# DanEngelbrecht/longtail

Measured on AMD Instinct MI355X. Metric: ingest GB/s (chunk+hash+compress), higher is better.
Workload: dtype u8/u32

## Files before the change

### longtail_amd/csrc/k_blake3.hip

```cpp
#include "lthip_internal.h"

#include <stdlib.h>

namespace
{

enum
{
    F_CHUNK_START = 1,
    F_CHUNK_END = 2,
    F_PARENT = 4,
    F_ROOT = 8
};

#define B3_IV0 0x6A09E667u
#define B3_IV1 0xBB67AE85u
#define B3_IV2 0x3C6EF372u
#define B3_IV3 0xA54FF53Au
#define B3_IV4 0x510E527Fu
#define B3_IV5 0x9B05688Cu
#define B3_IV6 0x1F83D9ABu
#define B3_IV7 0x5BE0CD19u

__device__ __forceinline__ uint32_t rotr32(uint32_t x, uint32_t r) { return __builtin_amdgcn_alignbit(x, x, r); }

__device__ __forceinline__ void b3_g(uint32_t& a, uint32_t& b, uint32_t& c, uint32_t& d, uint32_t mx, uint32_t my)
{
    a = a + b + mx;
    d = rotr32(d ^ a, 16);
    c = c + d;
    b = rotr32(b ^ c, 12);
    a = a + b + my;
    d = rotr32(d ^ a, 8);
    c = c + d;
    b = rotr32(b ^ c, 7);
}

#define B3_ROUND(m0, m1, m2, m3, m4, m5, m6, m7, m8, m9, m10, m11, m12, m13, m14, m15) \
    b3_g(s0, s4, s8, s12, m0, m1);                                                      \
    b3_g(s1, s5, s9, s13, m2, m3);                                                      \
    b3_g(s2, s6, s10, s14, m4, m5);                                                     \
    b3_g(s3, s7, s11, s15, m6, m7);                                                     \
    b3_g(s0, s5, s10, s15, m8, m9);                                                     \
    b3_g(s1, s6, s11, s12, m10, m11);                                                   \
    b3_g(s2, s7, s8, s13, m12, m13);                                                    \
    b3_g(s3, s4, s9, s14, m14, m15);

__device__ __forceinline__ void b3_compress(uint32_t (&cv)[8], const uint32_t (&m)[16], uint32_t counter_lo,
                                            uint32_t block_len, uint32_t flags)
{
    uint32_t s0 = cv[0], s1 = cv[1], s2 = cv[2], s3 = cv[3], s4 = cv[4], s5 = cv[5], s6 = cv[6], s7 = cv[7];
    uint32_t s8 = B3_IV0, s9 = B3_IV1, s10 = B3_IV2, s11 = B3_IV3;
    uint32_t s12 = counter_lo, s13 = 0u, s14 = block_len, s15 = flags;
    B3_ROUND(m[0], m[1], m[2], m[3], m[4], m[5], m[6], m[7], m[8], m[9], m[10], m[11], m[12], m[13], m[14], m[15])
    B3_ROUND(m[2], m[6], m[3], m[10], m[7], m[0], m[4], m[13], m[1], m[11], m[12], m[5], m[9], m[14], m[15], m[8])
    B3_ROUND(m[3], m[4], m[10], m[12], m[13], m[2], m[7], m[14], m[6], m[5], m[9], m[0], m[11], m[15], m[8], m[1])
    B3_ROUND(m[10], m[7], m[12], m[9], m[14], m[3], m[13], m[15], m[4], m[0], m[11], m[2], m[5], m[8], m[1], m[6])
    B3_ROUND(m[12], m[13], m[9], m[11], m[15], m[10], m[14], m[8], m[7], m[2], m[5], m[3], m[0], m[1], m[6], m[4])
    B3_ROUND(m[9], m[14], m[11], m[5], m[8], m[12], m[15], m[1], m[13], m[3], m[0], m[10], m[2], m[6], m[4], m[7])
    B3_ROUND(m[11], m[15], m[5], m[0], m[1], m[9], m[8], m[6], m[14], m[10], m[2], m[12], m[3], m[4], m[7], m[13])
    cv[0] = s0 ^ s8;
    cv[1] = s1 ^ s9;
    cv[2] = s2 ^ s10;
    cv[3] = s3 ^ s11;
    cv[4] = s4 ^ s12;
    cv[5] = s5 ^ s13;
    cv[6] = s6 ^ s14;
    cv[7] = s7 ^ s15;
}

typedef uint32_t u32x4_a4 __attribute__((ext_vector_type(4), aligned(4)));

__device__ __forceinline__ uint32_t leaves_of(uint32_t len) { return len ? (len + 1023u) >> 10 : 1u; }

__global__ void k_leaf_counts(const uint32_t* __restrict__ lens, uint64_t bound, const uint32_t* __restrict__ n_dev,
                              uint32_t* __restrict__ counts)
{
    uint64_t i = (uint64_t)blockIdx.x * blockDim.x + threadIdx.x;
    uint64_t n = n_dev ? (*n_dev < bound ? *n_dev : bound) : bound;
    if (i < n)
        counts[i] = leaves_of(lens[i]);
}

constexpr uint32_t b3s_blocks(uint32_t n, uint32_t B) { return (n + B - 1u) / B; }
constexpr uint32_t b3s_block_leaves(uint32_t n, uint32_t b, uint32_t B) { return n - b * B < B ? n - b * B : B; }
constexpr bool b3s_reg_merge(uint32_t m, uint32_t k, uint32_t st) { return k + st < m; }
constexpr bool b3s_root(uint32_t n, uint32_t K, uint32_t st) { return K == 0u && 2u * st >= n; }
constexpr bool b3s_to_lds(uint32_t n, uint32_t B) { return b3s_blocks(n, B) > 1u; }
constexpr bool b3s_lds_merge(uint32_t nb, uint32_t k, uint32_t st) { return (k & (2u * st - 1u)) == 0u && k + st < nb; }
constexpr bool b3s_lds_root(uint32_t nb, uint32_t st) { return 2u * st >= nb; }
constexpr uint32_t b3s_max_nodes(uint32_t S, uint32_t B) { return 2u * S / (B + 1u); }
constexpr uint32_t b3s_range_bytes(uint32_t n, uint32_t B) { return 6u + (b3s_to_lds(n, B) ? 32u * b3s_blocks(n, B) : 0u); }
constexpr uint32_t b3s_max_bytes(uint32_t S, uint32_t B) { return (6u * (B + 1u) > 70u ? 6u * (B + 1u) : 70u) * S / (B + 1u) + 6u + 16u; }

constexpr uint32_t PJ = 2;
constexpr uint32_t PB = 1u << PJ;
constexpr int PW = 2048;
constexpr int PW_MAXN = 256;
constexpr int PW_THREADS = 512;
constexpr int PW_WAVES = 8;
constexpr uint32_t PW_NODES = b3s_max_nodes(PW + PW_MAXN - 1, PB) + 1u;
constexpr uint32_t PW_MEM16 = (b3s_max_bytes(PW + PW_MAXN - 1, PB) + 15u) / 16u;
constexpr uint32_t PW_LEVELS = 8u - PJ;
static_assert(PW <= 4096 && (PW & (PW - 1)) == 0 && PW_THREADS % 64 == 0 && PW_MAXN >> PJ <= 255, "window tables are 16 bits, list entries 16 + 8 + 8");


__device__ __forceinline__ void b3_load_interior(uint32_t (&w)[17], const uint32_t* __restrict__ src)
{
    const u32x4_a4 v0 = *reinterpret_cast<const u32x4_a4*>(src);
    const u32x4_a4 v1 = *reinterpret_cast<const u32x4_a4*>(src + 4);
    const u32x4_a4 v2 = *reinterpret_cast<const u32x4_a4*>(src + 8);
    const u32x4_a4 v3 = *reinterpret_cast<const u32x4_a4*>(src + 12);
    w[0] = v0.x; w[1] = v0.y; w[2] = v0.z; w[3] = v0.w;
    w[4] = v1.x; w[5] = v1.y; w[6] = v1.z; w[7] = v1.w;
    w[8] = v2.x; w[9] = v2.y; w[10] = v2.z; w[11] = v2.w;
    w[12] = v3.x; w[13] = v3.y; w[14] = v3.z; w[15] = v3.w;
    w[16] = src[16];
}

__device__ __forceinline__ void b3_load_last(uint32_t (&w)[17], const uint32_t* __restrict__ src, uint32_t nd)
{
#pragma unroll
    for (int i = 0; i < 17; ++i)
        w[i] = (uint32_t)i < nd ? src[i] : 0u;
}

__device__ __forceinline__ void b3_interior_block(uint32_t (&cv)[8], uint32_t (&w)[17], uint32_t sh, uint32_t k, uint32_t flags)
{
#pragma unroll
    for (int i = 0; i < 16; ++i)
        asm("v_alignbit_b32 %0, %1, %0, %2" : "+v"(w[i]) : "v"(w[i + 1]), "v"(sh));
    uint32_t m[16];
#pragma unroll
    for (int i = 0; i < 16; ++i)
        m[i] = w[i];
    b3_compress(cv, m, k, 64u, flags);
}

__device__ __forceinline__ void b3_last_block(uint32_t (&cv)[8], const uint32_t (&w)[17], uint32_t sh, uint32_t k, uint32_t bl, uint32_t flags)
{
    uint32_t m[16];
#pragma unroll
    for (int i = 0; i < 16; ++i)
    {
        uint32_t v = __builtin_amdgcn_alignbit(w[i + 1], w[i], sh);
        const int rem = (int)bl - 4 * i;
        if (rem <= 0)
            v = 0u;
        else if (rem < 4)
            v &= (1u << (8 * rem)) - 1u;
        m[i] = v;
    }
    b3_compress(cv, m, k, bl, flags);
}

__device__ __forceinline__ void b3_pin(uint32_t (&cv)[8])
{
    asm volatile("" : "+v"(cv[0]), "+v"(cv[1]), "+v"(cv[2]), "+v"(cv[3]), "+v"(cv[4]), "+v"(cv[5]), "+v"(cv[6]), "+v"(cv[7])::"memory");
}

template <bool PIPE>
__global__ __launch_bounds__(256, 8) void k_blake3_leaves(const uint8_t* __restrict__ data,
                                                       const uint64_t* __restrict__ offsets,
                                                       const uint32_t* __restrict__ lens,
                                                       const uint32_t* __restrict__ leaf_prefix,
                                                       uint64_t count_bound, const uint32_t* __restrict__ n_dev,
                                                       uint32_t* __restrict__ cvs, uint32_t* __restrict__ win_first)
{
    const uint32_t count = (uint32_t)(n_dev ? (*n_dev < count_bound ? *n_dev : count_bound) : count_bound);
    const uint32_t total = leaf_prefix[count];
    const uint64_t g64 = (uint64_t)blockIdx.x * blockDim.x + threadIdx.x;
    if (g64 >= total)
        return;
    const uint32_t g = (uint32_t)g64;
    uint32_t lo = 0, hi = count;
    while (hi - lo > 1)
    {
        const uint32_t mid = lo + ((hi - lo) >> 1);
        if (leaf_prefix[mid] <= g)
            lo = mid;
        else
            hi = mid;
    }
    const uint32_t c = lo;
    const uint32_t first = leaf_prefix[c];
    const uint32_t k = g - first;
    if (win_first && (g & (uint32_t)(PW - 1)) == 0u)
        win_first[g / (uint32_t)PW] = k == 0u ? c : c + 1u;
    const uint32_t rlen = lens[c];
    const uint32_t nleaf = leaves_of(rlen);
    const uint32_t llen = rlen - (k << 10) < 1024u ? rlen - (k << 10) : 1024u;
    const uint8_t* p = data + offsets[c] + ((uint64_t)k << 10);
    const uint32_t root = nleaf == 1u ? (uint32_t)F_ROOT : 0u;

    const uint32_t mis = (uint32_t)((uintptr_t)p & 3u);
    const uint32_t sh = mis * 8u;
    const uint32_t* q = reinterpret_cast<const uint32_t*>(p - mis);

    uint32_t cv[8] = {B3_IV0, B3_IV1, B3_IV2, B3_IV3, B3_IV4, B3_IV5, B3_IV6, B3_IV7};
    const uint32_t nblocks = llen ? (llen + 63u) >> 6 : 1u;

    if constexpr (PIPE)
    {
        const uint32_t last = nblocks - 1u;
        const uint32_t bl = llen - last * 64u;
        const uint32_t nd = bl ? (mis + bl + 3u) >> 2 : 0u;
        uint32_t wa[17], wb[17];
        uint32_t b = 0;
        bool first_half = last > 1u && ((last - 1u) & 1u) == 0u;
        if (last > 1u && !first_half)
            b3_load_interior(wb, q);
        else if (last)
            b3_load_interior(wa, q);
        if (last > 1u)
        {
#pragma unroll 1
            for (;;)
            {
                if (first_half)
                {
                    b3_load_interior(wb, q + (b + 1u) * 16u);
                    b3_pin(cv);
                    b3_interior_block(cv, wa, sh, k, b == 0 ? (uint32_t)F_CHUNK_START : 0u);
                    b3_pin(cv);
                    ++b;
                }
                first_half = true;
                b3_load_interior(wa, q + (b + 1u) * 16u);
                b3_pin(cv);
                b3_interior_block(cv, wb, sh, k, b == 0 ? (uint32_t)F_CHUNK_START : 0u);
                b3_pin(cv);
                ++b;
                if (b + 1u >= last)
                    break;
            }
        }
        if (last)
        {
            b3_load_last(wb, q + last * 16u, nd);
            b3_pin(cv);
            b3_interior_block(cv, wa, sh, k, b == 0 ? (uint32_t)F_CHUNK_START : 0u);
            b3_pin(cv);
        }
        else
            b3_load_last(wb, q, nd);
        b3_last_block(cv, wb, sh, k, bl, (uint32_t)F_CHUNK_END | root | (last == 0 ? (uint32_t)F_CHUNK_START : 0u));
    }
    else
    {
        for (uint32_t b = 0; b + 1 < nblocks; ++b)
        {
            const uint32_t* src = q + b * 16u;
            uint32_t w[17];
            const u32x4_a4 v0 = *reinterpret_cast<const u32x4_a4*>(src);
            const u32x4_a4 v1 = *reinterpret_cast<const u32x4_a4*>(src + 4);
            const u32x4_a4 v2 = *reinterpret_cast<const u32x4_a4*>(src + 8);
            const u32x4_a4 v3 = *reinterpret_cast<const u32x4_a4*>(src + 12);
            w[0] = v0.x; w[1] = v0.y; w[2] = v0.z; w[3] = v0.w;
            w[4] = v1.x; w[5] = v1.y; w[6] = v1.z; w[7] = v1.w;
            w[8] = v2.x; w[9] = v2.y; w[10] = v2.z; w[11] = v2.w;
            w[12] = v3.x; w[13] = v3.y; w[14] = v3.z; w[15] = v3.w;
            w[16] = mis ? src[16] : 0u;
            uint32_t m[16];
#pragma unroll
            for (int i = 0; i < 16; ++i)
                m[i] = __builtin_amdgcn_alignbit(w[i + 1], w[i], sh);
            b3_compress(cv, m, k, 64u, b == 0 ? (uint32_t)F_CHUNK_START : 0u);
        }
        const uint32_t b = nblocks - 1u;
        const uint32_t bl = llen - b * 64u;
        uint32_t w[17];
        b3_load_last(w, q + b * 16u, bl ? (mis + bl + 3u) >> 2 : 0u);
        b3_last_block(cv, w, sh, k, bl, (uint32_t)F_CHUNK_END | root | (b == 0 ? (uint32_t)F_CHUNK_START : 0u));
    }
    uint4* out = reinterpret_cast<uint4*>(cvs + (uint64_t)g * 8u);
    out[0] = make_uint4(cv[0], cv[1], cv[2], cv[3]);
    out[1] = make_uint4(cv[4], cv[5], cv[6], cv[7]);
}

__device__ __forceinline__ void b3_parent(uint32_t* __restrict__ left, const uint32_t* __restrict__ right, uint32_t flags)
{
    uint32_t m[16];
    const uint4 a0 = reinterpret_cast<const uint4*>(left)[0], a1 = reinterpret_cast<const uint4*>(left)[1];
    const uint4 b0 = reinterpret_cast<const uint4*>(right)[0], b1 = reinterpret_cast<const uint4*>(right)[1];
    m[0] = a0.x; m[1] = a0.y; m[2] = a0.z; m[3] = a0.w; m[4] = a1.x; m[5] = a1.y; m[6] = a1.z; m[7] = a1.w;
    m[8] = b0.x; m[9] = b0.y; m[10] = b0.z; m[11] = b0.w; m[12] = b1.x; m[13] = b1.y; m[14] = b1.z; m[15] = b1.w;
    uint32_t cv[8] = {B3_IV0, B3_IV1, B3_IV2, B3_IV3, B3_IV4, B3_IV5, B3_IV6, B3_IV7};
    b3_compress(cv, m, 0u, 64u, flags);
    reinterpret_cast<uint4*>(left)[0] = make_uint4(cv[0], cv[1], cv[2], cv[3]);
    reinterpret_cast<uint4*>(left)[1] = make_uint4(cv[4], cv[5], cv[6], cv[7]);
}

#ifdef LTHIP_ABLATIONS
#include "ablations/k_blake3_parents_small.inc"
#endif

constexpr uint32_t B3_ONE_PITCH = 1024u + 4u;
__global__ __launch_bounds__(64) void k_blake3_one(const uint8_t* __restrict__ in, uint32_t len, uint64_t* __restrict__ out)
{
    extern __shared__ __attribute__((aligned(16))) uint32_t s_one[];
    uint32_t* s_cv = s_one;
    uint32_t* s_in = s_one + 64 * 8;
    const uint32_t lane = threadIdx.x;
    const uint32_t nleaf = leaves_of(len);
    {
        const uint32_t nvec = (((uintptr_t)in & 15u) == 0u) ? len >> 4 : 0u;
        const uint4* in4 = reinterpret_cast<const uint4*>(in);
        for (uint32_t v0 = 0; v0 < nvec; v0 += 64u * 8u)
        {
            uint4 q[8];
#pragma unroll
            for (int u = 0; u < 8; ++u)
            {
                const uint32_t v = v0 + (uint32_t)u * 64u + lane;
                q[u] = v < nvec ? in4[v] : make_uint4(0, 0, 0, 0);
            }
#pragma unroll
            for (int u = 0; u < 8; ++u)
            {
                const uint32_t v = v0 + (uint32_t)u * 64u + lane;
                if (v < nvec)
                {
                    uint32_t* d = s_in + (v >> 6) * (B3_ONE_PITCH / 4u) + (v & 63u) * 4u;
                    d[0] = q[u].x;
                    d[1] = q[u].y;
                    d[2] = q[u].z;
                    d[3] = q[u].w;
                }
            }
        }
        for (uint32_t j = (nvec << 4) + lane; j < len; j += 64u)
            reinterpret_cast<uint8_t*>(s_in)[(j >> 10) * B3_ONE_PITCH + (j & 1023u)] = in[j];
    }
    __syncthreads();
    if (lane < nleaf)
    {
        const uint32_t llen = len - (lane << 10) < 1024u ? len - (lane << 10) : 1024u;
        const uint32_t* pw = s_in + lane * (B3_ONE_PITCH / 4u);
        const uint8_t* p = reinterpret_cast<const uint8_t*>(pw);
        const uint32_t nblocks = llen ? (llen + 63u) >> 6 : 1u;
        uint32_t cv[8] = {B3_IV0, B3_IV1, B3_IV2, B3_IV3, B3_IV4, B3_IV5, B3_IV6, B3_IV7};
        for (uint32_t b = 0; b < nblocks; ++b)
        {
            const uint32_t bl = llen - b * 64u < 64u ? llen - b * 64u : 64u;
            uint32_t m[16];
            if (bl == 64u)
            {
#pragma unroll
                for (int i = 0; i < 16; ++i)
                    m[i] = pw[b * 16u + (uint32_t)i];
            }
            else
            {
#pragma unroll
                for (int i = 0; i < 16; ++i)
                    m[i] = 0u;
                for (uint32_t j = 0; j < bl; ++j)
                    m[j >> 2] |= (uint32_t)p[b * 64u + j] << (8u * (j & 3u));
            }
            uint32_t fl = b == 0 ? (uint32_t)F_CHUNK_START : 0u;
            if (b + 1 == nblocks)
                fl |= (uint32_t)F_CHUNK_END | (nleaf == 1u ? (uint32_t)F_ROOT : 0u);
            b3_compress(cv, m, lane, bl, fl);
        }
#pragma unroll
        for (int i = 0; i < 8; ++i)
            s_cv[lane * 8 + i] = cv[i];
    }
    __syncthreads();
    for (uint32_t stride = 1; stride < nleaf; stride <<= 1)
    {
        const uint32_t last = (stride << 1) >= nleaf;
        const uint32_t k = lane * (stride << 1);
        if (k + stride < nleaf)
            b3_parent(s_cv + k * 8u, s_cv + (k + stride) * 8u, (uint32_t)F_PARENT | (last ? (uint32_t)F_ROOT : 0u));
        __syncthreads();
    }
    if (lane == 0)
        *out = (uint64_t)s_cv[0] | ((uint64_t)s_cv[1] << 32);
}

constexpr int B3S_LEAVES = 1024;

__global__ __launch_bounds__(B3S_LEAVES) void k_blake3_stream_batch(const uint8_t* __restrict__ data, uint32_t leaf0,
                                                                      uint32_t* __restrict__ stack, uint32_t depth_in, uint32_t merges)
{
    __shared__ uint32_t s_cv[B3S_LEAVES * 8];
    const uint32_t t = threadIdx.x;
    {
        const uint32_t* p = reinterpret_cast<const uint32_t*>(data) + (size_t)t * 256u;
        uint32_t cv[8] = {B3_IV0, B3_IV1, B3_IV2, B3_IV3, B3_IV4, B3_IV5, B3_IV6, B3_IV7};
        for (uint32_t b = 0; b < 16u; ++b)
        {
            uint32_t m[16];
            const uint4* q = reinterpret_cast<const uint4*>(p + b * 16u);
            const uint4 v0 = q[0], v1 = q[1], v2 = q[2], v3 = q[3];
            m[0] = v0.x; m[1] = v0.y; m[2] = v0.z; m[3] = v0.w; m[4] = v1.x; m[5] = v1.y; m[6] = v1.z; m[7] = v1.w;
            m[8] = v2.x; m[9] = v2.y; m[10] = v2.z; m[11] = v2.w; m[12] = v3.x; m[13] = v3.y; m[14] = v3.z; m[15] = v3.w;
            b3_compress(cv, m, leaf0 + t, 64u, (b == 0 ? (uint32_t)F_CHUNK_START : 0u) | (b == 15u ? (uint32_t)F_CHUNK_END : 0u));
        }
#pragma unroll
        for (int i = 0; i < 8; ++i)
            s_cv[t * 8 + i] = cv[i];
    }
    __syncthreads();
    for (uint32_t stride = 1; stride < (uint32_t)B3S_LEAVES; stride <<= 1)
    {
        if ((t & (2u * stride - 1u)) == 0u)
            b3_parent(s_cv + t * 8u, s_cv + (t + stride) * 8u, (uint32_t)F_PARENT);
        __syncthreads();
    }
    if (t == 0)
    {
        uint32_t depth = depth_in;
        for (int i = 0; i < 8; ++i)
            stack[depth * 8u + i] = s_cv[i];
        ++depth;
        for (uint32_t m = 0; m < merges; ++m)
        {
            b3_parent(stack + (depth - 2u) * 8u, stack + (depth - 1u) * 8u, (uint32_t)F_PARENT);
            --depth;
        }
    }
}

__global__ __launch_bounds__(B3S_LEAVES) void k_blake3_stream_final(const uint8_t* __restrict__ tail, uint32_t tail_len, uint32_t leaf0,
                                                                      const uint32_t* __restrict__ stack, uint32_t depth_in,
                                                                      uint64_t* __restrict__ out)
{
    __shared__ uint32_t s_cv[B3S_LEAVES * 8];
    __shared__ uint32_t s_stack[64 * 8];
    const uint32_t t = threadIdx.x;
    const uint32_t nleaf = tail_len ? (tail_len + 1023u) >> 10 : (leaf0 == 0u ? 1u : 0u);
    const bool single = leaf0 == 0u && nleaf == 1u;
    if (t < nleaf)
    {
        const uint32_t llen = tail_len - (t << 10) < 1024u ? tail_len - (t << 10) : 1024u;
        const uint8_t* p = tail + ((size_t)t << 10);
        const uint32_t nblocks = llen ? (llen + 63u) >> 6 : 1u;
        uint32_t cv[8] = {B3_IV0, B3_IV1, B3_IV2, B3_IV3, B3_IV4, B3_IV5, B3_IV6, B3_IV7};
        for (uint32_t b = 0; b < nblocks; ++b)
        {
            const uint32_t bl = llen - b * 64u < 64u ? llen - b * 64u : 64u;
            uint32_t m[16];
#pragma unroll
            for (int i = 0; i < 16; ++i)
                m[i] = 0u;
            for (uint32_t j = 0; j < bl; ++j)
                m[j >> 2] |= (uint32_t)p[b * 64u + j] << (8u * (j & 3u));
            uint32_t fl = b == 0 ? (uint32_t)F_CHUNK_START : 0u;
            if (b + 1 == nblocks)
                fl |= (uint32_t)F_CHUNK_END | (single ? (uint32_t)F_ROOT : 0u);
            b3_compress(cv, m, leaf0 + t, bl, fl);
        }
#pragma unroll
        for (int i = 0; i < 8; ++i)
            s_cv[t * 8 + i] = cv[i];
    }
    for (uint32_t i = t; i < depth_in * 8u; i += (uint32_t)B3S_LEAVES)
        s_stack[i] = stack[i];
    __syncthreads();
    if (t != 0)
        return;
    if (single)
    {
        *out = (uint64_t)s_cv[0] | ((uint64_t)s_cv[1] << 32);
        return;
    }
    uint32_t depth = depth_in;
    for (uint32_t j = 0; j + 1 < nleaf; ++j)
    {
        for (int i = 0; i < 8; ++i)
            s_stack[depth * 8u + i] = s_cv[j * 8u + i];
        ++depth;
        uint32_t cnt = leaf0 + j + 1u;
        while ((cnt & 1u) == 0u)
        {
            b3_parent(s_stack + (depth - 2u) * 8u, s_stack + (depth - 1u) * 8u, (uint32_t)F_PARENT);
            --depth;
            cnt >>= 1;
        }
    }
    uint32_t* cur = s_cv + (nleaf - 1u) * 8u;
    while (depth > 0u)
    {
        uint32_t* left = s_stack + (depth - 1u) * 8u;
        b3_parent(left, cur, (uint32_t)F_PARENT | (depth == 1u ? (uint32_t)F_ROOT : 0u));
        cur = left;
        --depth;
    }
    *out = (uint64_t)cur[0] | ((uint64_t)cur[1] << 32);
}

__device__ __forceinline__ void b3_merge_regs(uint32_t (&left)[8], const uint32_t (&right)[8], uint32_t flags)
{
    const uint32_t m[16] = {left[0], left[1], left[2], left[3], left[4], left[5], left[6], left[7],
                            right[0], right[1], right[2], right[3], right[4], right[5], right[6], right[7]};
    uint32_t cv[8] = {B3_IV0, B3_IV1, B3_IV2, B3_IV3, B3_IV4, B3_IV5, B3_IV6, B3_IV7};
    b3_compress(cv, m, 0u, 64u, flags);
#pragma unroll
    for (int i = 0; i < 8; ++i)
        left[i] = cv[i];
}

__device__ __forceinline__ void pw_append(bool is, uint32_t entry, uint32_t* list, uint32_t* cnt, int lane)
{
    const uint64_t mask = __builtin_amdgcn_ballot_w64(is);
    if (mask == 0)
        return;
    uint32_t base = 0;
    if (lane == 0)
        base = atomicAdd(cnt, (uint32_t)__builtin_popcountll(mask));
    base = __builtin_amdgcn_readfirstlane(base);
    if (is)
        list[base + (uint32_t)__builtin_popcountll(mask & ((1ull << lane) - 1ull))] = entry;
}

__global__ __launch_bounds__(PW_THREADS, PW_WAVES) void k_blake3_parents_window(const uint32_t* __restrict__ leaf_prefix, uint64_t count_bound,
                                                                         const uint32_t* __restrict__ n_dev, const uint32_t* __restrict__ cvs,
                                                                         const uint32_t* __restrict__ win_first, uint64_t* __restrict__ hashes)
{
    __shared__ uint4 s_mem[PW_MEM16];
    __shared__ uint32_t s_list[2][PW_NODES / 2 + 1];
    __shared__ uint32_t s_cnt[PW_LEVELS + 1];
    __shared__ uint32_t s_wsum[PW_THREADS / 64];
    const uint32_t count = (uint32_t)(n_dev ? (*n_dev < count_bound ? *n_dev : count_bound) : count_bound);
    const uint32_t total = leaf_prefix[count];
    const uint64_t w0 = (uint64_t)blockIdx.x * PW;
    if (w0 >= total)
        return;
    const uint32_t tid = threadIdx.x;
    const int lane = (int)(tid & 63u);
    const uint32_t c_lo = win_first[blockIdx.x];
    const uint32_t c_hi = w0 + PW >= total ? count : win_first[blockIdx.x + 1u];
    const uint32_t nch = c_hi - c_lo;
    if (nch == 0)
        return;
    const uint32_t wbase = leaf_prefix[c_lo];
    if (nch > (uint32_t)PW || leaf_prefix[c_hi] - wbase > (uint32_t)(PW + PW_MAXN - 1))
        return;
    if (tid <= PW_LEVELS)
        s_cnt[tid] = 0;
    uint16_t* s_leaf = reinterpret_cast<uint16_t*>(s_mem);
    uint16_t* s_blk = s_leaf + (nch + 1u);
    uint16_t* s_node = s_blk + (nch + 1u);
    uint4* s_cv = s_mem + (6u * (nch + 1u) + 15u) / 16u;

    constexpr uint32_t R = (PW + PW_THREADS - 1) / PW_THREADS;
    {
        const uint32_t j0 = tid * R;
        uint32_t lp[R + 1], sum = 0;
#pragma unroll
        for (uint32_t i = 0; i <= R; ++i)
            lp[i] = leaf_prefix[c_lo + (j0 + i < nch ? j0 + i : nch)] - wbase;
#pragma unroll
        for (uint32_t i = 0; i < R; ++i)
        {
            const uint32_t n = lp[i + 1] - lp[i], nb = b3s_blocks(n, PB);
            sum += nb | (b3s_to_lds(n, PB) ? nb << 16 : 0u);
        }
        uint32_t incl = sum;
#pragma unroll
        for (int d = 1; d < 64; d <<= 1)
        {
            const uint32_t up = __shfl_up(incl, d, 64);
            if (lane >= d)
                incl += up;
        }
        if (lane == 63)
            s_wsum[tid >> 6] = incl;
        __syncthreads();
        uint32_t run = incl - sum;
        for (uint32_t w = 0; w < (tid >> 6); ++w)
            run += s_wsum[w];
#pragma unroll
        for (uint32_t i = 0; i <= R; ++i)
        {
            const uint32_t j = j0 + i;
            if (j <= nch && (i < R || j == nch))
            {
                s_leaf[j] = (uint16_t)lp[i];
                s_blk[j] = (uint16_t)(run & 0xFFFFu);
                s_node[j] = (uint16_t)(run >> 16);
            }
            if (i < R)
            {
                const uint32_t n = lp[i + 1] - lp[i], nb = b3s_blocks(n, PB);
                run += nb | (b3s_to_lds(n, PB) ? nb << 16 : 0u);
            }
        }
    }
    __syncthreads();

    if ((6u * (nch + 1u) + 15u) / 16u + 2u * s_node[nch] > PW_MEM16)
        return;

    const uint32_t nblk = s_blk[nch];
    const uint4* cvs4 = reinterpret_cast<const uint4*>(cvs) + (uint64_t)wbase * 2u;
    for (uint32_t b0 = 0; b0 < nblk; b0 += PW_THREADS)
    {
        const uint32_t blk = b0 + tid;
        bool left = false;
        uint32_t entry = 0;
        if (blk < nblk)
        {
            uint32_t lo = 0, hi = nch;
            while (hi - lo > 1)
            {
                const uint32_t mid = lo + ((hi - lo) >> 1);
                if (s_blk[mid] <= blk)
                    lo = mid;
                else
                    hi = mid;
            }
            const uint32_t j = lo, b = blk - s_blk[j];
            const uint32_t p = s_leaf[j], n = s_leaf[j + 1] - p, nb = b3s_blocks(n, PB);
            const uint32_t m = b3s_block_leaves(n, b, PB);
            const uint4* g = cvs4 + (p + b * PB) * 2u;
            uint32_t cv[PB][8];
#pragma unroll
            for (uint32_t i = 0; i < PB; ++i)
            {
                const uint32_t ii = i < m ? i : m - 1u;
                const uint4 x = g[2u * ii], y = g[2u * ii + 1u];
                cv[i][0] = x.x; cv[i][1] = x.y; cv[i][2] = x.z; cv[i][3] = x.w;
                cv[i][4] = y.x; cv[i][5] = y.y; cv[i][6] = y.z; cv[i][7] = y.w;
            }
#pragma unroll
            for (uint32_t st = 1; st < PB; st <<= 1)
            {
#pragma unroll
                for (uint32_t k = 0; k + st < PB; k += 2u * st)
                    if (b3s_reg_merge(m, k, st))
                        b3_merge_regs(cv[k], cv[k + st], (uint32_t)F_PARENT | (b3s_root(n, b * PB + k, st) ? (uint32_t)F_ROOT : 0u));
            }
            if (!b3s_to_lds(n, PB))
                hashes[c_lo + j] = (uint64_t)cv[0][0] | ((uint64_t)cv[0][1] << 32);
            else
            {
                const uint32_t node = (uint32_t)s_node[j] + b;
                s_cv[2u * node] = make_uint4(cv[0][0], cv[0][1], cv[0][2], cv[0][3]);
                s_cv[2u * node + 1u] = make_uint4(cv[0][4], cv[0][5], cv[0][6], cv[0][7]);
                left = b3s_lds_merge(nb, b, 1u);
                entry = node | (b << 16) | (nb << 24);
            }
        }
        pw_append(left, entry, s_list[0], &s_cnt[0], lane);
    }

    uint32_t rot = blockIdx.x;
    for (uint32_t lvl = 0, st = 1;; ++lvl, st <<= 1, ++rot)
    {
        __syncthreads();
        const uint32_t nm = lvl < PW_LEVELS ? s_cnt[lvl] : 0u;
        if (nm == 0)
            break;
        const uint32_t* cur = s_list[lvl & 1u];
        uint32_t* nxt = s_list[(lvl + 1u) & 1u];
        for (uint32_t m0 = 0; m0 < nm; m0 += PW_THREADS)
        {
            const uint32_t mi = m0 + (tid + 64u * rot) % (uint32_t)PW_THREADS;
            bool keep = false;
            uint32_t entry = 0;
            if (mi < nm)
            {
                entry = cur[mi];
                const uint32_t node = entry & 0xFFFFu, k = (entry >> 16) & 0xFFu, nb = entry >> 24;
                const uint4 a0 = s_cv[2u * node], a1 = s_cv[2u * node + 1u];
                const uint4 b0 = s_cv[2u * (node + st)], b1 = s_cv[2u * (node + st) + 1u];
                uint32_t m[16] = {a0.x, a0.y, a0.z, a0.w, a1.x, a1.y, a1.z, a1.w, b0.x, b0.y, b0.z, b0.w, b1.x, b1.y, b1.z, b1.w};
                uint32_t cv[8] = {B3_IV0, B3_IV1, B3_IV2, B3_IV3, B3_IV4, B3_IV5, B3_IV6, B3_IV7};
                b3_compress(cv, m, 0u, 64u, (uint32_t)F_PARENT | (b3s_lds_root(nb, st) ? (uint32_t)F_ROOT : 0u));
                s_cv[2u * node] = make_uint4(cv[0], cv[1], cv[2], cv[3]);
                s_cv[2u * node + 1u] = make_uint4(cv[4], cv[5], cv[6], cv[7]);
                keep = b3s_lds_merge(nb, k, 2u * st);
            }
            pw_append(keep, entry, nxt, &s_cnt[lvl + 1u], lane);
        }
    }
    for (uint32_t j = tid; j < nch; j += PW_THREADS)
        if (b3s_to_lds((uint32_t)s_leaf[j + 1] - s_leaf[j], PB))
        {
            const uint4 r = s_cv[2u * s_node[j]];
            hashes[c_lo + j] = (uint64_t)r.x | ((uint64_t)r.y << 32);
        }
}

__global__ __launch_bounds__(256) void k_blake3_parents_level(const uint32_t* __restrict__ leaf_prefix, uint32_t count,
                                                              uint32_t stride, uint32_t* __restrict__ cvs)
{
    const uint32_t total = leaf_prefix[count];
    const uint64_t g64 = (uint64_t)blockIdx.x * blockDim.x + threadIdx.x;
    if (g64 >= total)
        return;
    const uint32_t g = (uint32_t)g64;
    uint32_t lo = 0, hi = count;
    while (hi - lo > 1)
    {
        const uint32_t mid = lo + ((hi - lo) >> 1);
        if (leaf_prefix[mid] <= g)
            lo = mid;
        else
            hi = mid;
    }
    const uint32_t slot0 = leaf_prefix[lo];
    const uint32_t n = leaf_prefix[lo + 1] - slot0;
    const uint32_t k = g - slot0;
    if ((k & ((stride << 1) - 1u)) != 0u || k + stride >= n)
        return;
    const uint32_t last = (stride << 1) >= n;
    b3_parent(cvs + (uint64_t)g * 8u, cvs + (uint64_t)(g + stride) * 8u, (uint32_t)F_PARENT | (last ? (uint32_t)F_ROOT : 0u));
}

__global__ void k_blake3_emit(const uint32_t* __restrict__ leaf_prefix, uint32_t count, const uint32_t* __restrict__ cvs,
                              uint64_t* __restrict__ hashes)
{
    const uint64_t c = (uint64_t)blockIdx.x * blockDim.x + threadIdx.x;
    if (c >= count)
        return;
    const uint32_t* base = cvs + (uint64_t)leaf_prefix[c] * 8u;
    hashes[c] = (uint64_t)base[0] | ((uint64_t)base[1] << 32);
}

}

int lthip_launch_blake3(lthip_ctx* ctx, const uint8_t* d_data, const uint64_t* d_offsets, const uint32_t* d_lens,
                        const uint32_t* d_count, uint64_t count_bound, uint64_t leaf_bound, uint64_t max_len,
                        uint64_t* d_hashes)
{
    if (count_bound == 0)
        return 0;
    void *lc, *lp, *cv;
    int err;
    if ((err = lthip_scratch(ctx, S_LEAF_COUNT, (count_bound + 1) * 4, &lc)))
        return err;
    if ((err = lthip_scratch(ctx, S_LEAF_PREFIX, (count_bound + 1) * 4, &lp)))
        return err;
    {
        LaunchTimer t(ctx, LTHIP_K_COMPACT);
        hipLaunchKernelGGL(k_leaf_counts, dim3((uint32_t)div_up_u64(count_bound, 256)), dim3(256), 0, ctx->stream, d_lens,
                           count_bound, d_count, (uint32_t*)lc);
        LTHIP_LAUNCH_CHECK(ctx);
    }
    if ((err = lthip_exclusive_scan_u32(ctx, (const uint32_t*)lc, (uint32_t*)lp, count_bound, d_count, LTHIP_K_COMPACT)))
        return err;

    const bool small_trees = max_len != 0 && max_len <= 256u * 1024u;
    uint32_t host_count = 0;
    if (leaf_bound == 0 || !small_trees)
    {
        if (d_count)
        {
            LTHIP_CHECK(ctx, hipMemcpyAsync(&host_count, d_count, 4, hipMemcpyDeviceToHost, ctx->stream));
            LTHIP_CHECK(ctx, lthip_stream_wait(ctx));
            if (host_count > count_bound)
                host_count = (uint32_t)count_bound;
        }
        else
            host_count = (uint32_t)count_bound;
        uint32_t total = 0;
        LTHIP_CHECK(ctx, hipMemcpyAsync(&total, (const uint32_t*)lp + host_count, 4, hipMemcpyDeviceToHost, ctx->stream));
        LTHIP_CHECK(ctx, lthip_stream_wait(ctx));
        leaf_bound = total;
        if (host_count == 0)
            return 0;
    }
    if (leaf_bound == 0)
        return 0;
    if (leaf_bound > 0xFFFFFFF0ull)
        return lthip_fail(ctx, EINVAL, "blake3", "too many leaves in one batch");
    if ((err = lthip_scratch(ctx, S_CV, leaf_bound * 32, &cv)))
        return err;
    void* wf = nullptr;
    if (small_trees && (err = lthip_scratch(ctx, S_B3_WINDOWS, (leaf_bound / PW + 2) * 4, &wf)))
        return err;
    {
        LaunchTimer t(ctx, LTHIP_K_B3_LEAF);
        LTHIP_ABLATION_ENV(env_pad, "LTHIP_B3_PAD_LDS");
        const int pad_lds = env_pad.get() > 0 ? env_pad.get() : 0;
#ifdef LTHIP_ABLATIONS
        LTHIP_ABLATION_ENV(env_pf, "LTHIP_B3_PREFETCH");
        if (env_pf.get() == 0)
            hipLaunchKernelGGL(k_blake3_leaves<false>, dim3((uint32_t)div_up_u64(leaf_bound, 256)), dim3(256), (size_t)pad_lds, ctx->stream,
                               d_data, d_offsets, d_lens, (const uint32_t*)lp, count_bound, d_count, (uint32_t*)cv, (uint32_t*)wf);
        else
#endif
            hipLaunchKernelGGL(k_blake3_leaves<true>, dim3((uint32_t)div_up_u64(leaf_bound, 256)), dim3(256), (size_t)pad_lds, ctx->stream,
                               d_data, d_offsets, d_lens, (const uint32_t*)lp, count_bound, d_count, (uint32_t*)cv, (uint32_t*)wf);
        LTHIP_LAUNCH_CHECK(ctx);
    }
    if (small_trees)
    {
        LaunchTimer t(ctx, LTHIP_K_B3_PARENT);
#ifdef LTHIP_ABLATIONS
        LTHIP_ABLATION_ENV(env_serial, "LTHIP_B3_SERIAL_PARENTS");
        if (env_serial.get() >= 0)
            hipLaunchKernelGGL(k_blake3_parents_small, dim3((uint32_t)div_up_u64(count_bound, 256)), dim3(256), 0, ctx->stream,
                               d_lens, (const uint32_t*)lp, count_bound, d_count, (uint32_t*)cv, d_hashes);
        else
#endif
            hipLaunchKernelGGL(k_blake3_parents_window, dim3((uint32_t)div_up_u64(leaf_bound, PW)), dim3(PW_THREADS), 0, ctx->stream,
                               (const uint32_t*)lp, count_bound, d_count, (const uint32_t*)cv, (const uint32_t*)wf, d_hashes);
        LTHIP_LAUNCH_CHECK(ctx);
    }
    else
    {
        LaunchTimer t(ctx, LTHIP_K_B3_PARENT);
        uint64_t max_leaves = max_len ? div_up_u64(max_len, 1024) : (1ull << 22);
        for (uint64_t stride = 1; stride < max_leaves; stride <<= 1)
            hipLaunchKernelGGL(k_blake3_parents_level, dim3((uint32_t)div_up_u64(leaf_bound, 256)), dim3(256), 0,
                               ctx->stream, (const uint32_t*)lp, host_count, (uint32_t)stride, (uint32_t*)cv);
        hipLaunchKernelGGL(k_blake3_emit, dim3((uint32_t)div_up_u64(host_count, 256)), dim3(256), 0, ctx->stream,
                           (const uint32_t*)lp, host_count, (const uint32_t*)cv, d_hashes);
        LTHIP_LAUNCH_CHECK(ctx);
    }
    return 0;
}

int lthip_launch_blake3_one(lthip_ctx* ctx, const void* in, uint32_t len, uint64_t* out)
{
    if (len > 65536u)
        return lthip_fail(ctx, EINVAL, "blake3_one", "input above 64 KiB");
    LaunchTimer t(ctx, LTHIP_K_B3_LEAF);
    const size_t lds = 64 * 8 * 4 + (size_t)(len ? (len + 1023u) >> 10 : 1u) * B3_ONE_PITCH;
    if (lds > 64u * 1024u)
    {
        static bool granted[64] = {};
        if (ctx->device < 0 || ctx->device >= 64 || !granted[ctx->device])
        {
            LTHIP_CHECK(ctx, hipFuncSetAttribute(reinterpret_cast<const void*>(&k_blake3_one), hipFuncAttributeMaxDynamicSharedMemorySize, 80 * 1024));
            if (ctx->device >= 0 && ctx->device < 64)
                granted[ctx->device] = true;
        }
    }
    hipLaunchKernelGGL(k_blake3_one, dim3(1), dim3(64), lds, ctx->stream, (const uint8_t*)in, len, out);
    LTHIP_LAUNCH_CHECK(ctx);
    return 0;
}

int lthip_launch_blake3_stream_batch(lthip_ctx* ctx, const void* d_data, uint32_t leaf0, uint32_t* d_stack, uint32_t depth_in, uint32_t merges)
{
    LaunchTimer t(ctx, LTHIP_K_B3_LEAF);
    hipLaunchKernelGGL(k_blake3_stream_batch, dim3(1), dim3(B3S_LEAVES), 0, ctx->stream, (const uint8_t*)d_data, leaf0, d_stack, depth_in, merges);
    LTHIP_LAUNCH_CHECK(ctx);
    return 0;
}

int lthip_launch_blake3_stream_final(lthip_ctx* ctx, const void* d_tail, uint32_t tail_len, uint32_t leaf0, const uint32_t* d_stack,
                                     uint32_t depth, uint64_t* d_out)
{
    LaunchTimer t(ctx, LTHIP_K_B3_PARENT);
    hipLaunchKernelGGL(k_blake3_stream_final, dim3(1), dim3(B3S_LEAVES), 0, ctx->stream, (const uint8_t*)d_tail, tail_len, leaf0, d_stack, depth,
                       d_out);
    LTHIP_LAUNCH_CHECK(ctx);
    return 0;
}
```

### longtail_amd/csrc/k_buzhash.hip

```cpp
#include "lthip_internal.h"

#include <stdlib.h>
#include <type_traits>

namespace
{

__constant__ uint32_t c_buztab[256] = {
#include "buzhash_table.inc"
};

constexpr int RUN = 64;
constexpr int TILE = 256 * RUN;
constexpr int ROW_DW = 17;
constexpr int TAB_REP = 64;

__device__ __forceinline__ uint32_t lds_load_u32(uint32_t byte_addr)
{
#if defined(__HIP_DEVICE_COMPILE__)
    return *(const __attribute__((address_space(3))) uint32_t*)byte_addr;
#else
    (void)byte_addr;
    return 0u;
#endif
}

__device__ __forceinline__ uint32_t lds_load_u8(uint32_t byte_addr)
{
#if defined(__HIP_DEVICE_COMPILE__)
    return *(const __attribute__((address_space(3))) uint8_t*)byte_addr;
#else
    (void)byte_addr;
    return 0u;
#endif
}

__device__ __forceinline__ uint4 lds_load_u128(uint32_t byte_addr)
{
#if defined(__HIP_DEVICE_COMPILE__)
    typedef uint32_t v4 __attribute__((ext_vector_type(4)));
    const v4 q = *(const __attribute__((address_space(3))) v4*)byte_addr;
    return make_uint4(q.x, q.y, q.z, q.w);
#else
    (void)byte_addr;
    return make_uint4(0, 0, 0, 0);
#endif
}

__device__ __forceinline__ uint32_t rotl32(uint32_t x, uint32_t r) { return __builtin_amdgcn_alignbit(x, x, (32u - r) & 31u); }
__device__ __forceinline__ uint32_t rotr32(uint32_t x, uint32_t r) { return __builtin_amdgcn_alignbit(x, x, r & 31u); }

__global__ void k_tile_table(const PartDev* __restrict__ parts, uint32_t nparts, uint32_t* __restrict__ tile_part,
                             uint64_t ntiles)
{
    uint64_t t = (uint64_t)blockIdx.x * blockDim.x + threadIdx.x;
    if (t >= ntiles)
        return;
    uint32_t lo = 0, hi = nparts;
    while (hi - lo > 1)
    {
        uint32_t mid = lo + (hi - lo) / 2;
        if ((uint64_t)parts[mid].tile_base <= t)
            lo = mid;
        else
            hi = mid;
    }
    tile_part[t] = lo;
}

constexpr int WROWS = 64 + 1;
constexpr int WTILE = 64 * RUN;

#ifdef LTHIP_ABLATIONS
#include "ablations/k_buzhash_roll.inc"
#endif

#ifndef K1_MAD64
#define K1_MAD64 0
#endif
constexpr int HALO_DW = 64;

struct PrefixConsts
{
    uint32_t lane4;
    uint32_t hj;
    uint32_t halo_byte;
    uint32_t thr;
    uint32_t exact_add;
};

template <int MODE>
__device__ __forceinline__ uint64_t prefix_tile(const uint32_t (&win)[16], uint32_t hb, const PrefixConsts& pc, const DivTest& dv,
                                                int lane, uint32_t* __restrict__ halo)
{
    {
        uint32_t x = lds_load_u32((hb << 8) | pc.lane4);
        x = rotr32(x, pc.hj);
        if (lane >= 47)
            x = 0u;
        x ^= (uint32_t)__builtin_amdgcn_update_dpp(0, (int)x, 0x111, 0xf, 0xf, false);
        x ^= (uint32_t)__builtin_amdgcn_update_dpp(0, (int)x, 0x112, 0xf, 0xf, false);
        x ^= (uint32_t)__builtin_amdgcn_update_dpp(0, (int)x, 0x114, 0xf, 0xf, false);
        x ^= (uint32_t)__builtin_amdgcn_update_dpp(0, (int)x, 0x118, 0xf, 0xf, false);
        x ^= (uint32_t)__builtin_amdgcn_update_dpp(0, (int)x, 0x142, 0xa, 0xf, false);
        x ^= (uint32_t)__builtin_amdgcn_update_dpp(0, (int)x, 0x143, 0xc, 0xf, false);
        halo[pc.hj] = x;
    }

    uint32_t S[65];
#define LT_LOOKUP(j) S[j] = lds_load_u32(__builtin_amdgcn_perm(win[(j) >> 2], pc.lane4, 0x0c0c0400u | ((uint32_t)((j) & 3) << 8)))
#pragma unroll
    for (int j = 63; j >= 0; --j)
        LT_LOOKUP(j);
#undef LT_LOOKUP
    __builtin_amdgcn_sched_barrier(0);
    S[64] = 0u;
#pragma unroll
    for (int j = 63; j >= 0; --j)
        S[j] = S[j + 1] ^ ((j & 31) ? rotr32(S[j], (uint32_t)(j & 31)) : S[j]);
    __builtin_amdgcn_wave_barrier();

    uint32_t mlo = 0, mhi = 0;
    uint32_t inv_v;
    asm volatile("v_mov_b32 %0, %1" : "=v"(inv_v) : "s"(dv.inv));
#if K1_MAD64
    const uint64_t inv64 = (uint64_t)inv_v;
#endif
    typedef uint32_t u32x4 __attribute__((ext_vector_type(4)));
    u32x4 Q[16];
    auto halo_quad = [&](auto QI) __attribute__((always_inline))
    {
        constexpr int q = decltype(QI)::value;
        if constexpr (q >= 4 && q <= 15)
        {
            u32x4 v = {S[4 * q], S[4 * q + 1], S[4 * q + 2], S[4 * q + 3]};
            uint64_t save;
            asm volatile("s_mov_b64 %[sv], exec\n\ts_mov_b64 exec, %[msk]\n\t"
                         "ds_read_b128 %[r], %[ad] offset:%[o]\n\t"
                         "s_mov_b64 exec, %[sv]"
                         : [sv] "=&s"(save), [r] "+v"(v)
                         : [ad] "v"(pc.halo_byte), [msk] "s"(0x8000000000000000ull), [o] "i"(16 * q)
                         : "memory");
            Q[q] = v;
        }
    };
    auto halo_wait = [&](auto QI) __attribute__((always_inline))
    {
        constexpr int q = decltype(QI)::value;
        if constexpr (q >= 4 && q <= 15)
        {
            u32x4 v = Q[q];
            if constexpr (q >= 6)
                asm volatile("s_waitcnt lgkmcnt(2)" : "+v"(v));
            else if constexpr (q == 5)
                asm volatile("s_waitcnt lgkmcnt(1)" : "+v"(v));
            else
                asm volatile("s_waitcnt lgkmcnt(0)" : "+v"(v));
            S[4 * q] = v.x;
            S[4 * q + 1] = v.y;
            S[4 * q + 2] = v.z;
            S[4 * q + 3] = v.w;
        }
    };
    auto group = [&](auto G) __attribute__((always_inline))
    {
        constexpr int g = decltype(G)::value;
        uint32_t y[8];
#pragma unroll
        for (int half = 1; half >= 0; --half)
        {
            if (half == 1)
                halo_wait(std::integral_constant<int, 2 * g + 1 + 4>{});
            else
                halo_wait(std::integral_constant<int, 2 * g + 4>{});
#pragma unroll
            for (int ii = 3; ii >= 0; --ii)
            {
                const int i = 4 * half + ii;
                const int k = 8 * g + i;
                uint32_t w;
                if (k >= 47)
                    w = S[k - 47] ^ S[k + 1];
                else
                    w = (S[0] ^ S[k + 1]) ^ (uint32_t)__builtin_amdgcn_update_dpp(0, (int)S[(k + 17) & 63], 0x13C, 0xf, 0xf, false);
                const uint32_t h = (k & 31) ? rotl32(w, (uint32_t)(k & 31)) : w;
                if (MODE == 1)
                    y[i] = ~h & (dv.d - 1u);
                else
                {
#if K1_MAD64
                    uint64_t t, carry;
                    asm("v_mad_u64_u32 %0, %1, %2, %3, %4" : "=v"(t), "=s"(carry) : "v"(h), "s"(dv.inv), "v"(inv64));
                    y[i] = (uint32_t)t;
#else
                    y[i] = h * dv.inv + inv_v;
#endif
                }
            }
            if (half == 1)
                halo_quad(std::integral_constant<int, 2 * g + 2>{});
            else
                halo_quad(std::integral_constant<int, 2 * g + 1>{});
        }
        const uint32_t m = min(min(min(y[0], y[1]), y[2]), min(min(min(y[3], y[4]), y[5]), min(y[6], y[7])));
        if (__builtin_amdgcn_ballot_w64(m <= pc.thr) != 0ull)
        {
            asm volatile("");
#pragma unroll
            for (int i = 0; i < 8; ++i)
            {
                const int k = 8 * g + i;
                if (__builtin_amdgcn_ballot_w64(y[i] <= pc.thr) != 0ull)
                {
                    asm volatile("");
                    const bool hit = MODE == 1 ? y[i] == 0u : rotr32(y[i] + pc.exact_add, dv.k2) <= dv.qlim;
                    uint32_t hbit;
                    asm volatile("v_cndmask_b32_e64 %0, 0, 1, %1" : "=v"(hbit) : "s"(__builtin_amdgcn_ballot_w64(hit)));
                    if (k < 32)
                        mlo |= hbit << k;
                    else
                        mhi |= hbit << (k - 32);
                }
            }
        }
    };
    group(std::integral_constant<int, 7>{});
    group(std::integral_constant<int, 6>{});
    group(std::integral_constant<int, 5>{});
    group(std::integral_constant<int, 4>{});
    group(std::integral_constant<int, 3>{});
    group(std::integral_constant<int, 2>{});
    group(std::integral_constant<int, 1>{});
    group(std::integral_constant<int, 0>{});
    return ((uint64_t)mhi << 32) | mlo;
}

__device__ __forceinline__ uint64_t prefix_legal(uint64_t m, uint64_t q0, uint64_t size)
{
    if (q0 >= size)
        return 0ull;
    if (q0 < 47)
        m &= ~0ull << (47 - q0);
    const uint64_t remain = size - q0;
    if (remain < 64)
        m &= (1ull << remain) - 1ull;
    return m;
}

__device__ __forceinline__ void prefix_table_init(uint32_t* tab, int tid, int nthreads)
{
    for (int v = tid; v < 256; v += nthreads)
    {
        const uint32_t tv = c_buztab[v];
        uint4 q = make_uint4(tv, tv, tv, tv);
        uint4* dst = reinterpret_cast<uint4*>(tab + v * TAB_REP);
#pragma unroll
        for (int j = 0; j < TAB_REP / 4; ++j)
            dst[j] = q;
    }
    __syncthreads();
    if ((uint32_t)(uintptr_t)(const __attribute__((address_space(3))) uint32_t*)tab != 0u)
        __builtin_trap();
}

#ifdef LTHIP_ABLATIONS
#include "ablations/k_buzhash_prefix_regs.inc"
#endif

constexpr int DMA_BUF_B = WROWS * 64;

struct TileDma
{
    const uint8_t* data;
    uint32_t* buf;
    int lane;
    uint32_t buf_byte;
    uint32_t buf_mid;
    uint32_t src_off;
    uint32_t own_row;
    uint32_t own_f;

    __device__ __forceinline__ TileDma(const uint8_t* d, uint32_t* b, int ln) : data(d), buf(b), lane(ln)
    {
        buf_byte = __builtin_amdgcn_readfirstlane((uint32_t)(uintptr_t)(const __attribute__((address_space(3))) uint32_t*)buf);
        buf_mid = buf_byte + 2048u;
        const uint32_t src_vec = 4u * ((uint32_t)lane >> 2) + (((uint32_t)lane & 3u) ^ (((uint32_t)lane >> 4) & 3u));
        src_off = 16u * src_vec;
        own_f = (((uint32_t)lane + 1u) >> 2) & 3u;
        own_row = buf_byte + 64u * ((uint32_t)lane + 1u);
    }

    template <int MODE>
    __device__ __forceinline__ PrefixConsts consts(const DivTest& dv) const
    {
        PrefixConsts pc;
        pc.lane4 = (uint32_t)lane * 4u;
        pc.hj = 63u - (uint32_t)lane;
        pc.halo_byte = buf_byte + DMA_BUF_B;
        pc.thr = MODE == 1 ? 0u : 0xFFFFFFFFu / (dv.d >> dv.k2);
        pc.exact_add = dv.addc - dv.inv;
        return pc;
    }

    template <int u>
    __device__ __forceinline__ void piece(const uint8_t* mid_src) const
    {
        asm volatile("s_mov_b32 m0, %[l]\n\ts_nop 0\n\t"
                     "global_load_lds_dwordx4 %[v], %[b] offset:%[o]"
                     :
                     : [v] "v"(src_off), [l] "s"(buf_mid), [b] "s"(mid_src), [o] "i"(1024 * u - 2048)
                     : "memory");
    }

    template <int u>
    __device__ __forceinline__ void edge(const PartDev& p, uint64_t sp, const uint8_t* mid_src) const
    {
        const int64_t base = (int64_t)sp - 64 + 1024 * u;
        const int64_t left = (int64_t)p.size - base;
        const int32_t left_hi = (int32_t)(left >> 32);
        const uint32_t before = base < 0 ? (uint32_t)-base : 0u;
        const uint32_t room = left_hi < 0 ? 0u : left_hi > 0 || (uint32_t)left > 1024u ? 1024u : (uint32_t)left;
        const uint32_t room16 = room & ~15u;
        const bool lane_on = (u < 4 || lane < 4) && src_off >= before;
        const bool whole = lane_on && src_off < room16;
        const bool part = lane_on && src_off == room16 && room != room16;
        if (whole)
            piece<u>(mid_src);
        if (part)
        {
            const uint8_t* src = mid_src + (1024 * u - 2048);
            uint32_t w[4] = {0, 0, 0, 0};
            const uint32_t n = room - src_off;
            for (uint32_t bb = 0; bb < n; ++bb)
                w[bb >> 2] |= (uint32_t)src[src_off + bb] << (8 * (bb & 3));
            uint32_t* d = buf + 256 * u + 4 * lane;
            d[0] = w[0];
            d[1] = w[1];
            d[2] = w[2];
            d[3] = w[3];
        }
    }

    __device__ __forceinline__ void issue(const PartDev& p, uint64_t sp) const
    {
        const uint8_t* mid_src = data + p.off + sp - 64 + 2048;
        if (sp >= 64 && sp + (uint64_t)WTILE <= p.size)
        {
            asm volatile("s_mov_b32 m0, %[l]\n\ts_nop 0\n\t"
                         "global_load_lds_dwordx4 %[v], %[b] offset:-2048\n\t"
                         "global_load_lds_dwordx4 %[v], %[b] offset:-1024\n\t"
                         "global_load_lds_dwordx4 %[v], %[b] offset:0\n\t"
                         "global_load_lds_dwordx4 %[v], %[b] offset:1024"
                         :
                         : [v] "v"(src_off), [l] "s"(buf_mid), [b] "s"(mid_src)
                         : "memory");
            if (lane < 4)
                piece<4>(mid_src);
        }
        else
        {
            edge<0>(p, sp, mid_src);
            edge<1>(p, sp, mid_src);
            edge<2>(p, sp, mid_src);
            edge<3>(p, sp, mid_src);
            edge<4>(p, sp, mid_src);
        }
    }

    __device__ __forceinline__ void take(uint32_t (&win)[16], uint32_t& hb, const PrefixConsts& pc) const
    {
        asm volatile("s_waitcnt vmcnt(0)" ::: "memory");
#pragma unroll
        for (int c = 0; c < 4; ++c)
        {
            const uint4 q = lds_load_u128(own_row + 16u * ((uint32_t)c ^ own_f));
            win[4 * c + 0] = q.x;
            win[4 * c + 1] = q.y;
            win[4 * c + 2] = q.z;
            win[4 * c + 3] = q.w;
        }
        hb = lds_load_u8(buf_byte + pc.hj);
        asm volatile("s_waitcnt lgkmcnt(0)" ::: "memory");
    }
};

__device__ __forceinline__ uint64_t* run_words(uint64_t* __restrict__ bm0, uint64_t first)
{
    uint64_t* w = bm0 + first;
    asm("" : "+s"(w));
    return w;
}

template <int MODE, int WAVES>
__global__ __launch_bounds__(64 * WAVES, 1) void k_buzhash_prefix_dma(const uint8_t* __restrict__ data,
                                                                       const PartDev* __restrict__ parts,
                                                                       const uint32_t* __restrict__ tile_part,
                                                                       uint32_t ntiles, DivTest dv,
                                                                       uint64_t* __restrict__ bm0,
                                                                       uint64_t* __restrict__ bm1)
{
    extern __shared__ __attribute__((aligned(16))) uint32_t smem[];
    const int tid = threadIdx.x;
    const int lane = tid & 63;
    const int wave = __builtin_amdgcn_readfirstlane(tid >> 6);
    uint32_t* buf = smem + 256 * TAB_REP + wave * ((DMA_BUF_B >> 2) + HALO_DW);
    uint32_t* halo = buf + (DMA_BUF_B >> 2);
    prefix_table_init(smem, tid, 64 * WAVES);

    const TileDma dma(data, buf, lane);
    const PrefixConsts pc = dma.consts<MODE>(dv);

    const uint64_t nwt = (uint64_t)ntiles * 4u;
    const uint64_t wstride = (uint64_t)gridDim.x * (uint64_t)WAVES;
    uint64_t wt = (uint64_t)blockIdx.x * (uint64_t)WAVES + (uint64_t)wave;
    if (wt >= nwt)
        return;

    PartDev pd = parts[tile_part[wt >> 2]];
    uint64_t span = ((wt >> 2) - pd.tile_base) * (uint64_t)TILE + (wt & 3u) * (uint64_t)WTILE;
    dma.issue(pd, span);

    uint64_t pend_m = 0, pend_summary = 0, pend_i0 = 0, pend_i1 = 0;
    bool pend = false;
    for (;;)
    {
        uint32_t win[16], hb;
        dma.take(win, hb, pc);

        if (pend)
        {
            if (pend_m != 0ull)
                run_words(bm0, pend_i0)[(uint32_t)lane] = pend_m;
            if (lane == 0)
                bm1[pend_i1] = pend_summary;
        }

        const uint64_t next = wt + wstride;
        PartDev npd = pd;
        uint64_t next_span = 0;
        const bool more = (int64_t)(next - nwt) < 0;
        if (more)
        {
            npd = parts[tile_part[next >> 2]];
            next_span = ((next >> 2) - npd.tile_base) * (uint64_t)TILE + (next & 3u) * (uint64_t)WTILE;
            dma.issue(npd, next_span);
        }

        pend_m = prefix_legal(prefix_tile<MODE>(win, hb, pc, dv, lane, halo), span + (uint64_t)lane * RUN, pd.size);
        pend_summary = __builtin_amdgcn_ballot_w64(pend_m != 0ull);
        pend_i0 = pd.bm0_base + (span >> 6);
        pend_i1 = pd.bm1_base + (span >> 12);
        pend = true;

        if (!more)
            break;
        wt = next;
        pd = npd;
        span = next_span;
    }
    if (pend_m != 0ull)
        run_words(bm0, pend_i0)[(uint32_t)lane] = pend_m;
    if (lane == 0)
        bm1[pend_i1] = pend_summary;
}

__device__ __forceinline__ uint64_t bcast64(uint64_t v, int src_lane)
{
    uint32_t lo = __builtin_amdgcn_readlane((uint32_t)v, src_lane);
    uint32_t hi = __builtin_amdgcn_readlane((uint32_t)(v >> 32), src_lane);
    return ((uint64_t)hi << 32) | lo;
}

__global__ __launch_bounds__(64) void k_select_cuts(const PartDev* __restrict__ parts, uint32_t nparts,
                                                    const uint64_t* __restrict__ bm0, const uint64_t* __restrict__ bm1,
                                                    uint32_t min_chunk, uint32_t max_chunk, uint2* __restrict__ region,
                                                    uint32_t* __restrict__ part_count)
{
    const uint32_t p = blockIdx.x;
    if (p >= nparts)
        return;
    const int lane = threadIdx.x;
    const PartDev pd = parts[p];
    const uint64_t size = pd.size;
    const uint64_t* b0 = bm0 + pd.bm0_base;
    const uint64_t* b1 = bm1 + pd.bm1_base;
    uint2* out = region + pd.region_base;

    uint64_t s = 0;
    uint32_t n = 0;
    while (s < size)
    {
        const uint64_t left = size - s;
        uint64_t len;
        if (left <= min_chunk)
            len = left;
        else
        {
            const uint64_t end = left > max_chunk ? max_chunk : left;
            len = end;
            const uint64_t qlo = s + min_chunk;
            const uint64_t qhi = s + end - 1;
            if (qlo <= qhi)
            {
                const uint64_t rlo = qlo >> 6, rhi = qhi >> 6;
                const uint64_t wlo = rlo >> 6, whi = rhi >> 6;
                bool found = false;
                for (uint64_t w0 = wlo; w0 <= whi && !found; w0 += 64)
                {
                    const uint64_t w = w0 + (uint64_t)lane;
                    uint64_t word = 0;
                    if (w <= whi)
                    {
                        word = b1[w];
                        if (w == wlo)
                            word &= ~0ull << (rlo & 63);
                        if (w == whi && (rhi & 63) != 63)
                            word &= (1ull << ((rhi & 63) + 1)) - 1ull;
                    }
                    for (;;)
                    {
                        const uint64_t any = __builtin_amdgcn_ballot_w64(word != 0ull);
                        if (any == 0ull)
                            break;
                        const int f = __builtin_ctzll(any);
                        const uint64_t fw = bcast64(word, f);
                        const int bit = __builtin_ctzll(fw);
                        const uint64_t r = ((w0 + (uint64_t)f) << 6) + (uint64_t)bit;
                        uint64_t m = b0[r];
                        if (r == rlo)
                            m &= ~0ull << (qlo & 63);
                        if (r == rhi && (qhi & 63) != 63)
                            m &= (1ull << ((qhi & 63) + 1)) - 1ull;
                        if (m != 0ull)
                        {
                            const uint64_t q = (r << 6) + (uint64_t)__builtin_ctzll(m);
                            len = q - s + 1;
                            found = true;
                            break;
                        }
                        if (lane == f)
                            word &= word - 1ull;
                    }
                }
            }
        }
        if (lane == 0)
            out[n] = make_uint2((uint32_t)s, (uint32_t)len);
        ++n;
        s += len;
    }
    if (lane == 0)
        part_count[p] = n;
}

#ifdef LTHIP_ABLATIONS
__device__ unsigned long long g_walk_tiles;
#endif

template <int MODE, int WAVES, bool GUESS>
__global__ __launch_bounds__(64 * WAVES, 1) void k_buzhash_walk(const uint8_t* __restrict__ data, const PartDev* __restrict__ parts,
                                                                 uint32_t nparts, DivTest dv, uint32_t min_chunk, uint32_t max_chunk,
                                                                 uint2* __restrict__ region, uint32_t* __restrict__ part_count,
                                                                 uint32_t* __restrict__ ticket)
{
    extern __shared__ __attribute__((aligned(16))) uint32_t smem[];
    const int tid = threadIdx.x;
    const int lane = tid & 63;
    const int wave = __builtin_amdgcn_readfirstlane(tid >> 6);
    uint32_t* buf = smem + 256 * TAB_REP + wave * ((DMA_BUF_B >> 2) + HALO_DW);
    uint32_t* halo = buf + (DMA_BUF_B >> 2);
    prefix_table_init(smem, tid, 64 * WAVES);

    const TileDma dma(data, buf, lane);
    const PrefixConsts pc = dma.consts<MODE>(dv);
    const int lane_base = lane * RUN;

    auto jump = [](uint64_t q) __attribute__((always_inline)) { return q >= 64 ? ((q - 64) & ~(uint64_t)15) + 64 : (uint64_t)0; };

    bool inflight = false;
    uint64_t inflight_tb = 0;
#ifdef LTHIP_ABLATIONS
    uint32_t tiles = 0;
#endif
    for (;;)
    {
        __builtin_amdgcn_wave_barrier();
        uint32_t t = atomicAdd(ticket, lane == 0 ? 1u : 0u);
        t = __builtin_amdgcn_readfirstlane(t);
        if (t >= nparts)
            break;
        const PartDev pd = parts[t];
        const uint64_t size = pd.size;
        uint2* out = region + pd.region_base;
        uint64_t s = 0, qlo = 0, qhi = 0;
        uint32_t n = 0, end = 0;

        auto next_chunk = [&]() __attribute__((always_inline)) -> bool
        {
            for (;;)
            {
                if (s >= size)
                    return false;
                const uint64_t left = size - s;
                const uint32_t len = left <= min_chunk ? (uint32_t)left : left > max_chunk ? max_chunk : (uint32_t)left;
                if (left > min_chunk && len > min_chunk)
                {
                    end = len;
                    qlo = s + min_chunk;
                    qhi = s + end - 1;
                    return true;
                }
                if (lane == 0)
                    out[n] = make_uint2((uint32_t)s, len);
                ++n;
                s += len;
            }
        };

        if (next_chunk())
        {
            uint64_t tb = jump(qlo);
            auto ends_here = [&]() __attribute__((always_inline)) { return (uint32_t)(qhi - tb) < (uint32_t)WTILE; };
            for (bool walking = true; walking;)
            {
                if (!(inflight && inflight_tb == tb))
                {
                    if (inflight)
                        asm volatile("s_waitcnt vmcnt(0)" ::: "memory");
                    dma.issue(pd, tb);
                }
                inflight = false;
                uint32_t win[16], hb;
                dma.take(win, hb, pc);
                if (GUESS)
                {
                    uint64_t g = tb + (uint64_t)WTILE;
                    bool aim = true;
                    if (ends_here())
                    {
                        const uint64_t s2 = s + end;
                        aim = size - s2 > min_chunk && max_chunk > min_chunk;
                        g = jump(s2 + min_chunk);
                    }
                    if (aim)
                    {
                        dma.issue(pd, g);
                        inflight = true;
                        inflight_tb = g;
                    }
                }
                const uint64_t raw = prefix_tile<MODE>(win, hb, pc, dv, lane, halo);
#ifdef LTHIP_ABLATIONS
                ++tiles;
#endif
                for (;;)
                {
                    const int lo = (int)(qlo > tb ? qlo - tb : 0) - lane_base;
                    const int hi = (int)(ends_here() ? (uint32_t)(qhi - tb) : (uint32_t)WTILE - 1u) - lane_base;
                    uint64_t m = raw;
                    if (lo > 0)
                        m = lo > 63 ? 0ull : m & (~0ull << lo);
                    if (hi < 63)
                        m = hi < 0 ? 0ull : m & ((2ull << hi) - 1ull);
                    const uint64_t any = __builtin_amdgcn_ballot_w64(m != 0ull);
                    uint32_t len;
                    if (any != 0ull)
                    {
                        const int f = __builtin_ctzll(any);
                        const uint64_t q = tb + (uint64_t)(f * RUN + __builtin_ctzll(bcast64(m, f)));
                        len = (uint32_t)(q - s) + 1u;
                    }
                    else if (ends_here())
                        len = end;
                    else
                    {
                        tb += (uint64_t)WTILE;
                        break;
                    }
                    if (lane == 0)
                        out[n] = make_uint2((uint32_t)s, len);
                    ++n;
                    s += len;
                    if (!next_chunk())
                    {
                        walking = false;
                        break;
                    }
                    if ((uint32_t)(qlo - tb) < (uint32_t)WTILE)
                        continue;
                    tb = jump(qlo);
                    break;
                }
            }
        }
        if (inflight)
        {
            asm volatile("s_waitcnt vmcnt(0)" ::: "memory");
            inflight = false;
        }
        if (lane == 0)
            part_count[t] = n;
    }
#ifdef LTHIP_ABLATIONS
    if (lane == 0 && tiles)
        atomicAdd(&g_walk_tiles, (unsigned long long)tiles);
#endif
}

constexpr int SCAN_THREADS = 256;
constexpr int SCAN_ITEMS = 8;
constexpr int SCAN_BLOCK = SCAN_THREADS * SCAN_ITEMS;

__device__ __forceinline__ uint32_t block_exclusive_scan(uint32_t v, uint32_t* total, uint32_t* sh )
{
    const int lane = threadIdx.x & 63, wave = threadIdx.x >> 6;
    uint32_t x = v;
#pragma unroll
    for (int o = 1; o < 64; o <<= 1)
    {
        uint32_t y = __shfl_up(x, o, 64);
        if (lane >= o)
            x += y;
    }
    if (lane == 63)
        sh[wave] = x;
    __syncthreads();
    uint32_t base = 0, tot = 0;
#pragma unroll
    for (int w = 0; w < SCAN_THREADS / 64; ++w)
    {
        uint32_t t = sh[w];
        if (w < wave)
            base += t;
        tot += t;
    }
    __syncthreads();
    *total = tot;
    return base + x - v;
}

__global__ __launch_bounds__(SCAN_THREADS) void k_scan_sums(const uint32_t* __restrict__ in, uint64_t n,
                                                            const uint32_t* __restrict__ n_dev,
                                                            uint32_t* __restrict__ sums)
{
    __shared__ uint32_t sh[8];
    if (n_dev)
        n = *n_dev < n ? *n_dev : n;
    const uint64_t base = (uint64_t)blockIdx.x * SCAN_BLOCK;
    uint32_t acc = 0;
#pragma unroll
    for (int i = 0; i < SCAN_ITEMS; ++i)
    {
        uint64_t idx = base + (uint64_t)i * SCAN_THREADS + threadIdx.x;
        if (idx < n)
            acc += in[idx];
    }
    uint32_t tot;
    block_exclusive_scan(acc, &tot, sh);
    if (threadIdx.x == 0)
        sums[blockIdx.x] = tot;
}

__global__ __launch_bounds__(SCAN_THREADS) void k_scan_spine(uint32_t* __restrict__ sums, uint32_t nblocks)
{
    __shared__ uint32_t sh[8];
    uint32_t carry = 0;
    for (uint32_t b0 = 0; b0 < nblocks; b0 += SCAN_THREADS)
    {
        uint32_t i = b0 + threadIdx.x;
        uint32_t v = i < nblocks ? sums[i] : 0;
        uint32_t tot;
        uint32_t ex = block_exclusive_scan(v, &tot, sh);
        if (i < nblocks)
            sums[i] = carry + ex;
        carry += tot;
    }
    if (threadIdx.x == 0)
        sums[nblocks] = carry;
}

__global__ __launch_bounds__(SCAN_THREADS) void k_scan_apply(const uint32_t* __restrict__ in, uint64_t n,
                                                             const uint32_t* __restrict__ n_dev,
                                                             const uint32_t* __restrict__ sums, uint32_t nblocks,
                                                             uint32_t* __restrict__ out)
{
    __shared__ uint32_t sh[8];
    if (n_dev)
        n = *n_dev < n ? *n_dev : n;
    const uint64_t base = (uint64_t)blockIdx.x * SCAN_BLOCK + (uint64_t)threadIdx.x * SCAN_ITEMS;
    uint32_t v[SCAN_ITEMS];
    uint32_t acc = 0;
#pragma unroll
    for (int i = 0; i < SCAN_ITEMS; ++i)
    {
        uint64_t idx = base + i;
        v[i] = idx < n ? in[idx] : 0;
        acc += v[i];
    }
    uint32_t tot;
    uint32_t ex = block_exclusive_scan(acc, &tot, sh) + sums[blockIdx.x];
#pragma unroll
    for (int i = 0; i < SCAN_ITEMS; ++i)
    {
        uint64_t idx = base + i;
        if (idx < n)
            out[idx] = ex;
        ex += v[i];
    }
    if (blockIdx.x == 0 && threadIdx.x == 0)
        out[n] = sums[nblocks];
}

__global__ __launch_bounds__(64) void k_compact_chunks(const PartDev* __restrict__ parts, uint32_t nparts,
                                                       const uint2* __restrict__ region,
                                                       const uint32_t* __restrict__ part_first,
                                                       uint64_t* __restrict__ chunk_offsets,
                                                       uint32_t* __restrict__ chunk_lens)
{
    const uint32_t p = blockIdx.x;
    if (p >= nparts)
        return;
    const PartDev pd = parts[p];
    const uint32_t first = part_first[p];
    const uint32_t n = part_first[p + 1] - first;
    const uint2* in = region + pd.region_base;
    for (uint32_t i = threadIdx.x; i < n; i += 64)
    {
        uint2 e = in[i];
        chunk_offsets[first + i] = pd.off + (uint64_t)e.x;
        chunk_lens[first + i] = e.y;
    }
}

__global__ __launch_bounds__(64) void k_chunk_from_buffer(const uint8_t* __restrict__ buf, uint32_t n, uint32_t min_chunk,
                                                          DivTest dv, uint64_t* __restrict__ out_len)
{
    const int lane = threadIdx.x;
    uint32_t h0 = 0;
    for (uint32_t i = 0; i < 48; ++i)
        h0 ^= rotl32(c_buztab[buf[i]], (47u - i) & 31u);
    uint32_t result = n;
    const uint32_t kmax = n - min_chunk;
    for (uint32_t k0 = 1; k0 <= kmax; k0 += 64)
    {
        const uint32_t k = k0 + (uint32_t)lane;
        bool hit = false;
        if (k <= kmax)
        {
            uint32_t h;
            if (k < 48)
            {
                h = rotl32(h0, k & 31u);
                for (uint32_t i = 1; i <= k; ++i)
                    h ^= rotl32(rotl32(c_buztab[buf[i - 1]], 16) ^ c_buztab[buf[min_chunk + i - 1]], (k - i) & 31u);
            }
            else
            {
                const uint32_t p = min_chunk + k;
                h = 0;
                for (uint32_t j = 0; j < 48; ++j)
                    h ^= rotl32(c_buztab[buf[p - 1 - j]], j & 31u);
            }
            hit = dv.pow2 ? (h & (dv.d - 1u)) == dv.d - 1u : rotr32(h * dv.inv + dv.addc, dv.k2) <= dv.qlim;
        }
        const uint64_t any = __builtin_amdgcn_ballot_w64(hit);
        if (any)
        {
            result = min_chunk + k0 + (uint32_t)__builtin_ctzll(any);
            break;
        }
    }
    if (lane == 0)
        *out_len = result;
}

}

int lthip_launch_from_buffer(lthip_ctx* ctx, const uint8_t* d_data, uint32_t n, uint32_t min_chunk, const DivTest& dv,
                             uint64_t* d_out)
{
    LaunchTimer t(ctx, LTHIP_K_OTHER);
    hipLaunchKernelGGL(k_chunk_from_buffer, dim3(1), dim3(64), 0, ctx->stream, d_data, n, min_chunk, dv, d_out);
    LTHIP_LAUNCH_CHECK(ctx);
    return 0;
}

int lthip_launch_tile_table(lthip_ctx* ctx, lthip_plan* plan)
{
    if (plan->ntiles == 0)
        return 0;
    LaunchTimer t(ctx, LTHIP_K_OTHER);
    const uint32_t blocks = (uint32_t)div_up_u64(plan->ntiles, 256);
    hipLaunchKernelGGL(k_tile_table, dim3(blocks), dim3(256), 0, ctx->stream, plan->d_parts, plan->nparts,
                       plan->d_tile_part, plan->ntiles);
    LTHIP_LAUNCH_CHECK(ctx);
    return 0;
}

#ifdef LTHIP_ABLATIONS
constexpr bool K1_HAS_REG_FLAVOUR = true;
#else
constexpr bool K1_HAS_REG_FLAVOUR = false;
#endif

template <int WAVES, bool DMA>
static int launch_buzhash_prefix(lthip_ctx* ctx, const lthip_plan* plan, const uint8_t* d_data, uint64_t* bm0, uint64_t* bm1)
{
    static_assert(DMA || K1_HAS_REG_FLAVOUR, "the register-staged flavour is compiled by the ablation build only");
    constexpr size_t per_wave = DMA ? (DMA_BUF_B >> 2) + HALO_DW : WROWS * ROW_DW + HALO_DW;
    static_assert(sizeof(uint32_t) * (256 * TAB_REP + WAVES * per_wave) <= 160 * 1024, "LDS budget: one workgroup per CU");
    const size_t lds = sizeof(uint32_t) * (256 * TAB_REP + WAVES * per_wave);
#ifdef LTHIP_ABLATIONS
    auto k0 = DMA ? &k_buzhash_prefix_dma<0, WAVES> : &k_buzhash_prefix<0, WAVES>;
    auto k1 = DMA ? &k_buzhash_prefix_dma<1, WAVES> : &k_buzhash_prefix<1, WAVES>;
#else
    auto k0 = &k_buzhash_prefix_dma<0, WAVES>;
    auto k1 = &k_buzhash_prefix_dma<1, WAVES>;
#endif
    static bool granted[64] = {};
    if (ctx->device < 0 || ctx->device >= 64 || !granted[ctx->device])
    {
        LTHIP_CHECK(ctx, hipFuncSetAttribute(reinterpret_cast<const void*>(k0), hipFuncAttributeMaxDynamicSharedMemorySize, (int)lds));
        LTHIP_CHECK(ctx, hipFuncSetAttribute(reinterpret_cast<const void*>(k1), hipFuncAttributeMaxDynamicSharedMemorySize, (int)lds));
        if (ctx->device >= 0 && ctx->device < 64)
            granted[ctx->device] = true;
    }
    int ncu = 256;
    (void)hipDeviceGetAttribute(&ncu, hipDeviceAttributeMultiprocessorCount, ctx->device);
    uint32_t grid = (uint32_t)ncu;
    if ((uint64_t)grid * WAVES > plan->ntiles * 4u)
        grid = (uint32_t)div_up_u64(plan->ntiles * 4u, WAVES);
    LaunchTimer t(ctx, LTHIP_K_BUZHASH);
    hipLaunchKernelGGL(plan->div.pow2 ? k1 : k0, dim3(grid), dim3(64 * WAVES), lds, ctx->stream, d_data, plan->d_parts,
                       plan->d_tile_part, (uint32_t)plan->ntiles, plan->div, bm0, bm1);
    LTHIP_LAUNCH_CHECK(ctx);
    return 0;
}

#ifdef LTHIP_ABLATIONS
static int k1_flavour()
{
    static std::atomic<int> f{-1};
    static std::atomic<uint32_t> seen{0};
    const uint32_t gen = g_lthip_env_gen;
    if (seen.load(std::memory_order_acquire) != gen)
    {
        const char* e = getenv("LTHIP_K1");
        f.store(!e ? 0 : !strcmp(e, "roll") ? 4 : !strcmp(e, "prefix12") ? 3 : !strcmp(e, "prefix16") ? 2 : !strcmp(e, "dma12") ? 1 : 0,
                std::memory_order_relaxed);
        seen.store(gen, std::memory_order_release);
    }
    return f.load(std::memory_order_relaxed);
}

static int launch_buzhash_roll(lthip_ctx* ctx, const lthip_plan* plan, const uint8_t* d_data, uint64_t* bm0, uint64_t* bm1)
{
    static_assert(sizeof(uint32_t) * (256 * TAB_REP + K1_WAVES * WROWS * ROW_DW) <= 160 * 1024, "LDS budget: one workgroup per CU");
    const size_t lds = sizeof(uint32_t) * (256 * TAB_REP + K1_WAVES * WROWS * ROW_DW);
    if (!ctx->k1_lds_enabled)
    {
        LTHIP_CHECK(ctx, hipFuncSetAttribute(reinterpret_cast<const void*>(&k_buzhash_candidates<0>), hipFuncAttributeMaxDynamicSharedMemorySize, (int)lds));
        LTHIP_CHECK(ctx, hipFuncSetAttribute(reinterpret_cast<const void*>(&k_buzhash_candidates<1>), hipFuncAttributeMaxDynamicSharedMemorySize, (int)lds));
        ctx->k1_lds_enabled = true;
    }
    int ncu = 256;
    (void)hipDeviceGetAttribute(&ncu, hipDeviceAttributeMultiprocessorCount, ctx->device);
    uint32_t grid = (uint32_t)ncu;
    if ((uint64_t)grid * K1_WAVES > plan->ntiles * 4u)
        grid = (uint32_t)div_up_u64(plan->ntiles * 4u, K1_WAVES);
    LaunchTimer t(ctx, LTHIP_K_BUZHASH);
    if (plan->div.pow2)
        hipLaunchKernelGGL(k_buzhash_candidates<1>, dim3(grid), dim3(K1_THREADS), lds, ctx->stream, d_data, plan->d_parts,
                           plan->d_tile_part, (uint32_t)plan->ntiles, plan->div, bm0, bm1);
    else
        hipLaunchKernelGGL(k_buzhash_candidates<0>, dim3(grid), dim3(K1_THREADS), lds, ctx->stream, d_data, plan->d_parts,
                           plan->d_tile_part, (uint32_t)plan->ntiles, plan->div, bm0, bm1);
    LTHIP_LAUNCH_CHECK(ctx);
    return 0;
}
#endif

int lthip_launch_buzhash(lthip_ctx* ctx, const lthip_plan* plan, const uint8_t* d_data, uint64_t* bm0, uint64_t* bm1)
{
    if (plan->ntiles == 0)
        return 0;
#ifdef LTHIP_ABLATIONS
    const int flavour = k1_flavour();
    if (flavour == 1)
        return launch_buzhash_prefix<12, true>(ctx, plan, d_data, bm0, bm1);
    if (flavour == 2)
        return launch_buzhash_prefix<16, false>(ctx, plan, d_data, bm0, bm1);
    if (flavour == 3)
        return launch_buzhash_prefix<12, false>(ctx, plan, d_data, bm0, bm1);
    if (flavour == 4)
        return launch_buzhash_roll(ctx, plan, d_data, bm0, bm1);
#endif
    return launch_buzhash_prefix<16, true>(ctx, plan, d_data, bm0, bm1);
}

uint32_t lthip_k1_resident_waves(int device)
{
    static std::atomic<uint32_t> cached[64] = {};
    if (device >= 0 && device < 64 && cached[device].load(std::memory_order_relaxed))
        return cached[device].load(std::memory_order_relaxed);
    int ncu = 256;
    (void)hipDeviceGetAttribute(&ncu, hipDeviceAttributeMultiprocessorCount, device);
    const uint32_t w = (uint32_t)(ncu > 0 ? ncu : 256) * 16u;
    if (device >= 0 && device < 64)
        cached[device].store(w, std::memory_order_relaxed);
    return w;
}

#ifndef K1_WALK_GUESS
#define K1_WALK_GUESS 1
#endif

template <bool GUESS>
static int launch_buzhash_walk(lthip_ctx* ctx, const lthip_plan* plan, const uint8_t* d_data, uint2* region, uint32_t* part_count)
{
    constexpr int WAVES = 16;
    const size_t lds = sizeof(uint32_t) * (256 * TAB_REP + WAVES * ((DMA_BUF_B >> 2) + HALO_DW));
    auto k0 = &k_buzhash_walk<0, WAVES, GUESS>;
    auto k1 = &k_buzhash_walk<1, WAVES, GUESS>;
    static bool granted[64] = {};
    if (ctx->device < 0 || ctx->device >= 64 || !granted[ctx->device])
    {
        LTHIP_CHECK(ctx, hipFuncSetAttribute(reinterpret_cast<const void*>(k0), hipFuncAttributeMaxDynamicSharedMemorySize, (int)lds));
        LTHIP_CHECK(ctx, hipFuncSetAttribute(reinterpret_cast<const void*>(k1), hipFuncAttributeMaxDynamicSharedMemorySize, (int)lds));
        if (ctx->device >= 0 && ctx->device < 64)
            granted[ctx->device] = true;
    }
    void* ticket;
    int err = lthip_scratch(ctx, S_WALK_TICKET, 64, &ticket);
    if (err)
        return err;
    uint32_t grid = lthip_k1_resident_waves(ctx->device) / WAVES;
    if ((uint64_t)grid * WAVES > plan->nparts)
        grid = (uint32_t)div_up_u64(plan->nparts, WAVES);
    LaunchTimer t(ctx, LTHIP_K_BUZHASH);
    LTHIP_CHECK(ctx, hipMemsetAsync(ticket, 0, 4, ctx->stream));
    hipLaunchKernelGGL(plan->div.pow2 ? k1 : k0, dim3(grid), dim3(64 * WAVES), lds, ctx->stream, d_data, plan->d_parts, plan->nparts,
                       plan->div, plan->min_chunk, plan->max_chunk, region, part_count, (uint32_t*)ticket);
    LTHIP_LAUNCH_CHECK(ctx);
    return 0;
}

int lthip_launch_buzhash_walk(lthip_ctx* ctx, const lthip_plan* plan, const uint8_t* d_data, uint2* region, uint32_t* part_count)
{
    if (plan->nparts == 0)
        return 0;
#ifdef LTHIP_ABLATIONS
    LTHIP_ABLATION_ENV(env_guess, "LTHIP_K1_WALK_GUESS");
    if (env_guess.get() >= 0 && (env_guess.get() != 0) != (K1_WALK_GUESS != 0))
        return launch_buzhash_walk<!K1_WALK_GUESS>(ctx, plan, d_data, region, part_count);
#endif
    return launch_buzhash_walk<K1_WALK_GUESS != 0>(ctx, plan, d_data, region, part_count);
}

extern "C" int lthip_debug_walk_tiles(uint64_t* out_tiles)
{
#ifdef LTHIP_ABLATIONS
    if (!out_tiles)
        return EINVAL;
    unsigned long long v = 0, zero = 0;
    if (hipDeviceSynchronize() != hipSuccess || hipMemcpyFromSymbol(&v, HIP_SYMBOL(g_walk_tiles), sizeof v) != hipSuccess ||
        hipMemcpyToSymbol(HIP_SYMBOL(g_walk_tiles), &zero, sizeof zero) != hipSuccess)
        return EIO;
    *out_tiles = v;
    return 0;
#else
    (void)out_tiles;
    return ENOTSUP;
#endif
}

int lthip_launch_select(lthip_ctx* ctx, const lthip_plan* plan, const uint64_t* bm0, const uint64_t* bm1, uint2* region,
                        uint32_t* part_count)
{
    LaunchTimer t(ctx, LTHIP_K_SELECT);
    hipLaunchKernelGGL(k_select_cuts, dim3(plan->nparts), dim3(64), 0, ctx->stream, plan->d_parts, plan->nparts, bm0, bm1,
                       plan->min_chunk, plan->max_chunk, region, part_count);
    LTHIP_LAUNCH_CHECK(ctx);
    return 0;
}

int lthip_exclusive_scan_u32(lthip_ctx* ctx, const uint32_t* d_in, uint32_t* d_out, uint64_t n_bound,
                             const uint32_t* d_n, int kid)
{
    const uint64_t nblocks64 = n_bound ? div_up_u64(n_bound, SCAN_BLOCK) : 1;
    if (nblocks64 > 0x7FFFFFFFull)
        return lthip_fail(ctx, EINVAL, "scan", "too many elements");
    const uint32_t nblocks = (uint32_t)nblocks64;
    void* tmp;
    int err = lthip_scratch(ctx, S_SCAN_TMP, ((size_t)nblocks + 1) * 4, &tmp);
    if (err)
        return err;
    uint32_t* sums = (uint32_t*)tmp;
    LaunchTimer t(ctx, kid);
    hipLaunchKernelGGL(k_scan_sums, dim3(nblocks), dim3(SCAN_THREADS), 0, ctx->stream, d_in, n_bound, d_n, sums);
    hipLaunchKernelGGL(k_scan_spine, dim3(1), dim3(SCAN_THREADS), 0, ctx->stream, sums, nblocks);
    hipLaunchKernelGGL(k_scan_apply, dim3(nblocks), dim3(SCAN_THREADS), 0, ctx->stream, d_in, n_bound, d_n, sums, nblocks,
                       d_out);
    LTHIP_LAUNCH_CHECK(ctx);
    return 0;
}

int lthip_launch_compact(lthip_ctx* ctx, const lthip_plan* plan, const uint2* region, const uint32_t* part_count,
                         uint32_t* d_part_first, uint64_t* d_chunk_offsets, uint32_t* d_chunk_lens)
{
    int err = lthip_exclusive_scan_u32(ctx, part_count, d_part_first, plan->nparts, nullptr, LTHIP_K_COMPACT);
    if (err || plan->nparts == 0)
        return err;
    LaunchTimer t(ctx, LTHIP_K_COMPACT);
    hipLaunchKernelGGL(k_compact_chunks, dim3(plan->nparts), dim3(64), 0, ctx->stream, plan->d_parts, plan->nparts, region,
                       (const uint32_t*)d_part_first, d_chunk_offsets, d_chunk_lens);
    LTHIP_LAUNCH_CHECK(ctx);
    return 0;
}
```

### longtail_amd/csrc/lthip_ctx.hip

```cpp
#include "lthip_internal.h"
#include "store_index_ops.h"

#include <stdlib.h>

#include <new>

int lthip_fail(lthip_ctx* ctx, int code, const char* what, const char* detail)
{
    if (ctx)
        snprintf(ctx->err, sizeof ctx->err, "%s: %s", what ? what : "?", detail ? detail : "");
    return code;
}

int lthip_scratch(lthip_ctx* ctx, int slot, size_t bytes, void** out)
{
    if (bytes == 0)
        bytes = 256;
    if (ctx->scratch_cap[slot] < bytes)
    {
        if (ctx->scratch[slot])
        {
            LTHIP_CHECK(ctx, lthip_stream_wait(ctx));
            LTHIP_CHECK(ctx, hipFree(ctx->scratch[slot]));
            ctx->scratch[slot] = nullptr;
            ctx->scratch_cap[slot] = 0;
        }
        size_t cap = bytes + bytes / 8 + 4096;
        LTHIP_CHECK(ctx, lthip_hip_malloc(&ctx->scratch[slot], cap));
        ctx->scratch_cap[slot] = cap;
    }
    *out = ctx->scratch[slot];
    return 0;
}

volatile uint32_t g_lthip_env_gen = 1;
extern "C" void lthip_debug_reload_env(void) { g_lthip_env_gen = g_lthip_env_gen + 1u; }

#ifdef LTHIP_ABLATIONS
namespace
{
std::atomic<int64_t> g_alloc_calls{0};
std::atomic<int64_t> g_fail_first{INT64_MAX};
std::atomic<int64_t> g_fail_last{INT64_MAX};
std::atomic<int64_t> g_alloc_failed{0};
bool inject_failure()
{
    const int64_t n = g_alloc_calls.fetch_add(1, std::memory_order_relaxed) + 1;
    if (n < g_fail_first.load(std::memory_order_relaxed) || n > g_fail_last.load(std::memory_order_relaxed))
        return false;
    g_alloc_failed.fetch_add(1, std::memory_order_relaxed);
    return true;
}
}
hipError_t lthip_hip_malloc(void** p, size_t bytes)
{
    if (inject_failure())
    {
        *p = nullptr;
        return hipErrorOutOfMemory;
    }
    return hipMalloc(p, bytes);
}
hipError_t lthip_hip_host_malloc(void** p, size_t bytes, unsigned flags)
{
    if (inject_failure())
    {
        *p = nullptr;
        return hipErrorOutOfMemory;
    }
    return hipHostMalloc(p, bytes, flags);
}
extern "C" int lthip_debug_fail_alloc(int64_t after, int64_t count)
{
    if (after < 0 || count <= 0)
    {
        g_fail_first = INT64_MAX;
        g_fail_last = INT64_MAX;
        return 0;
    }
    const int64_t now = g_alloc_calls.load();
    g_fail_last = INT64_MAX;
    g_fail_first = now + after + 1;
    g_fail_last = count > INT64_MAX - (now + after) ? INT64_MAX : now + after + count;
    return 0;
}
extern "C" int64_t lthip_debug_alloc_calls(int64_t* out_failed)
{
    if (out_failed)
        *out_failed = g_alloc_failed.load();
    return g_alloc_calls.load();
}
#else
extern "C" int lthip_debug_fail_alloc(int64_t, int64_t) { return ENOTSUP; }
extern "C" int64_t lthip_debug_alloc_calls(int64_t* out_failed)
{
    if (out_failed)
        *out_failed = 0;
    return -1;
}
#endif

extern "C" int lthip_device_count(void)
{
    int n = 0;
    if (hipGetDeviceCount(&n) != hipSuccess)
        return 0;
    return n;
}

extern "C" int lthip_ctx_create(int device, void* hip_stream, lthip_ctx** out_ctx)
{
    if (!out_ctx)
        return EINVAL;
    *out_ctx = nullptr;
    int n = 0;
    if (hipGetDeviceCount(&n) != hipSuccess || n <= 0)
        return ENODEV;
    if (device < 0 || device >= n)
        return EINVAL;
    if (hipSetDevice(device) != hipSuccess)
        return EIO;
    lthip_ctx* ctx = new (std::nothrow) lthip_ctx();
    if (!ctx)
        return ENOMEM;
    ctx->device = device;
    ctx->slice_ctx = nullptr;
    ctx->err[0] = 0;
    ctx->timing = false;
    memset(ctx->scratch, 0, sizeof ctx->scratch);
    memset(ctx->stage, 0, sizeof ctx->stage);
    memset(ctx->stage_small, 0, sizeof ctx->stage_small);
    ctx->stage_next = ctx->stage_small_next = 0;
    ctx->k1_lds_enabled = false;
    ctx->z_last_retry = nullptr;
    ctx->z_last_payloads = 0;
    ctx->z_last_foreign_blocks = 0;
    memset(ctx->k5_lds_enabled, 0, sizeof ctx->k5_lds_enabled);
    memset(ctx->scratch_cap, 0, sizeof ctx->scratch_cap);
    memset(ctx->total_ms, 0, sizeof ctx->total_ms);
    memset(ctx->launches, 0, sizeof ctx->launches);
    if (hip_stream != LTHIP_STREAM_PRIVATE)
    {
        ctx->stream = (hipStream_t)hip_stream;
        ctx->own_stream = false;
    }
    else
    {
        if (hipStreamCreateWithFlags(&ctx->stream, hipStreamNonBlocking) != hipSuccess)
        {
            delete ctx;
            return EIO;
        }
        ctx->own_stream = true;
    }
    *out_ctx = ctx;
    return 0;
}

hipError_t lthip_stream_wait(lthip_ctx* ctx) { return hipStreamSynchronize(ctx->stream); }

extern "C" int lthip_set_blocking_waits(int device, int on)
{
    int n = 0;
    if (hipGetDeviceCount(&n) != hipSuccess || device < 0 || device >= n)
        return ENODEV;
    int prev = 0;
    (void)hipGetDevice(&prev);
    if (hipSetDevice(device) != hipSuccess)
        return EIO;
    const hipError_t e = hipSetDeviceFlags(on ? hipDeviceScheduleBlockingSync : hipDeviceScheduleAuto);
    (void)hipSetDevice(prev);
    return e == hipSuccess ? 0 : EIO;
}

extern "C" void lthip_ctx_destroy(lthip_ctx* ctx)
{
    if (!ctx)
        return;
    (void)hipSetDevice(ctx->device);
    (void)hipStreamSynchronize(ctx->stream);
    if (ctx->slice_ctx)
        lthip_ctx_destroy(ctx->slice_ctx);
    for (auto& r : ctx->pending)
    {
        (void)hipEventDestroy(r.a);
        (void)hipEventDestroy(r.b);
    }
    for (auto e : ctx->free_events)
        (void)hipEventDestroy(e);
    for (auto e : ctx->sync_events)
        (void)hipEventDestroy(e);
    if (ctx->stream2)
    {
        (void)hipStreamSynchronize(ctx->stream2);
        (void)hipStreamDestroy(ctx->stream2);
    }
    for (int i = 0; i < S_COUNT; ++i)
        if (ctx->scratch[i])
            (void)hipFree(ctx->scratch[i]);
    for (auto& st : ctx->stage)
    {
        if (st.done)
            (void)hipEventDestroy(st.done);
        if (st.p)
            (void)hipHostFree(st.p);
    }
    for (auto& st : ctx->stage_small)
    {
        if (st.done)
            (void)hipEventDestroy(st.done);
        if (st.p)
            (void)hipHostFree(st.p);
    }
    if (ctx->own_stream)
        (void)hipStreamDestroy(ctx->stream);
    delete ctx;
}

extern "C" int lthip_ctx_sync(lthip_ctx* ctx)
{
    if (!ctx)
        return EINVAL;
    LTHIP_CHECK(ctx, lthip_stream_wait(ctx));
    return 0;
}

extern "C" const char* lthip_ctx_error(const lthip_ctx* ctx) { return ctx ? ctx->err : "no context"; }

extern "C" int lthip_malloc_device(lthip_ctx* ctx, size_t bytes, void** out)
{
    if (!ctx || !out)
        return EINVAL;
    LTHIP_CHECK(ctx, hipSetDevice(ctx->device));
    LTHIP_CHECK(ctx, lthip_hip_malloc(out, bytes ? bytes : 16));
    return 0;
}

extern "C" void lthip_free_device(lthip_ctx* ctx, void* p)
{
    if (!p)
        return;
    if (ctx)
    {
        (void)hipSetDevice(ctx->device);
        (void)lthip_stream_wait(ctx);
    }
    (void)hipFree(p);
}

extern "C" int lthip_malloc_pinned(lthip_ctx* ctx, size_t bytes, void** out)
{
    if (!ctx || !out)
        return EINVAL;
    LTHIP_CHECK(ctx, hipSetDevice(ctx->device));
    LTHIP_CHECK(ctx, lthip_hip_host_malloc(out, bytes ? bytes : 16, hipHostMallocDefault));
    return 0;
}

extern "C" void lthip_free_pinned(lthip_ctx* ctx, void* p)
{
    if (!p)
        return;
    if (ctx)
    {
        (void)hipSetDevice(ctx->device);
        (void)lthip_stream_wait(ctx);
    }
    (void)hipHostFree(p);
}

extern "C" int lthip_copy_h2d(lthip_ctx* ctx, void* d_dst, const void* h_src, size_t bytes)
{
    if (!ctx || (bytes && (!d_dst || !h_src)))
        return EINVAL;
    if (bytes == 0)
        return 0;
    LTHIP_CHECK(ctx, hipSetDevice(ctx->device));
    LTHIP_CHECK(ctx, hipMemcpyAsync(d_dst, h_src, bytes, hipMemcpyHostToDevice, ctx->stream));
    return 0;
}

extern "C" int lthip_copy_d2h(lthip_ctx* ctx, void* h_dst, const void* d_src, size_t bytes)
{
    if (!ctx || (bytes && (!h_dst || !d_src)))
        return EINVAL;
    if (bytes == 0)
        return 0;
    LTHIP_CHECK(ctx, hipSetDevice(ctx->device));
    LTHIP_CHECK(ctx, hipMemcpyAsync(h_dst, d_src, bytes, hipMemcpyDeviceToHost, ctx->stream));
    return 0;
}

static hipEvent_t take_event(lthip_ctx* ctx)
{
    if (!ctx->free_events.empty())
    {
        hipEvent_t e = ctx->free_events.back();
        ctx->free_events.pop_back();
        return e;
    }
    hipEvent_t e = nullptr;
    (void)hipEventCreate(&e);
    return e;
}

LaunchTimer::LaunchTimer(lthip_ctx* c, int kid, hipStream_t s) : ctx(c), on(c->timing), stream(s ? s : c->stream)
{
    if (on)
    {
        rec.kid = kid;
        rec.a = take_event(ctx);
        rec.b = take_event(ctx);
        (void)hipEventRecord(rec.a, stream);
    }
}

int lthip_second_stream(lthip_ctx* ctx, hipStream_t* out)
{
    if (!ctx->stream2)
        LTHIP_CHECK(ctx, hipStreamCreateWithFlags(&ctx->stream2, hipStreamNonBlocking));
    *out = ctx->stream2;
    return 0;
}

int lthip_stage_upload(lthip_ctx* ctx, void* d_dst, const void* h_src, size_t bytes, hipStream_t stream)
{
    if (bytes == 0)
        return 0;
    const bool small = bytes <= LTHIP_STAGE_SMALL;
    LTHIP_ABLATION_ENV(env_slots, "LTHIP_STAGE_SLOTS");
    const size_t nsmall = env_slots.get() > 0 && env_slots.get() < 64 ? (size_t)env_slots.get() : sizeof(ctx->stage_small) / sizeof(ctx->stage_small[0]);
    lthip_ctx::Stage& st = small ? ctx->stage_small[ctx->stage_small_next++ % nsmall]
                                 : ctx->stage[ctx->stage_next++ % (sizeof(ctx->stage) / sizeof(ctx->stage[0]))];
    if (st.used)
        LTHIP_CHECK(ctx, hipEventSynchronize(st.done));
    if (st.cap < bytes)
    {
        if (st.p)
            LTHIP_CHECK(ctx, hipHostFree(st.p));
        st.p = nullptr;
        st.cap = 0;
        const size_t want = small ? LTHIP_STAGE_SMALL : bytes + bytes / 2 + 4096;
        LTHIP_CHECK(ctx, lthip_hip_host_malloc(&st.p, want, hipHostMallocDefault));
        st.cap = want;
    }
    if (!st.done)
        LTHIP_CHECK(ctx, hipEventCreateWithFlags(&st.done, hipEventDisableTiming));
    memcpy(st.p, h_src, bytes);
    LTHIP_CHECK(ctx, hipMemcpyAsync(d_dst, st.p, bytes, hipMemcpyHostToDevice, stream));
    LTHIP_CHECK(ctx, hipEventRecord(st.done, stream));
    st.used = true;
    return 0;
}

hipEvent_t lthip_sync_event(lthip_ctx* ctx)
{
    if (ctx->sync_events.size() < 16)
    {
        hipEvent_t e = nullptr;
        (void)hipEventCreateWithFlags(&e, hipEventDisableTiming);
        ctx->sync_events.push_back(e);
        return e;
    }
    return ctx->sync_events[ctx->sync_next++ % ctx->sync_events.size()];
}

LaunchTimer::~LaunchTimer()
{
    if (on)
    {
        (void)hipEventRecord(rec.b, stream);
        ctx->pending.push_back(rec);
    }
}

static int timing_collect(lthip_ctx* ctx)
{
    if (ctx->pending.empty())
        return 0;
    LTHIP_CHECK(ctx, lthip_stream_wait(ctx));
    for (auto& r : ctx->pending)
    {
        float ms = 0.f;
        if (hipEventElapsedTime(&ms, r.a, r.b) == hipSuccess)
        {
            ctx->total_ms[r.kid] += (double)ms;
            ctx->launches[r.kid] += 1;
        }
        ctx->free_events.push_back(r.a);
        ctx->free_events.push_back(r.b);
    }
    ctx->pending.clear();
    return 0;
}

extern "C" int lthip_timing_enable(lthip_ctx* ctx, int on)
{
    if (!ctx)
        return EINVAL;
    int err = timing_collect(ctx);
    ctx->timing = on != 0;
    if (ctx->slice_ctx)
        (void)lthip_timing_enable(ctx->slice_ctx, on);
    return err;
}

extern "C" int lthip_timing_reset(lthip_ctx* ctx)
{
    if (!ctx)
        return EINVAL;
    int err = timing_collect(ctx);
    memset(ctx->total_ms, 0, sizeof ctx->total_ms);
    memset(ctx->launches, 0, sizeof ctx->launches);
    if (ctx->slice_ctx)
        (void)lthip_timing_reset(ctx->slice_ctx);
    return err;
}

extern "C" int lthip_timing_get(lthip_ctx* ctx, int kernel_id, double* out_total_ms, uint64_t* out_launches)
{
    if (!ctx || kernel_id < 0 || kernel_id >= LTHIP_K_COUNT)
        return EINVAL;
    int err = timing_collect(ctx);
    double ms = ctx->total_ms[kernel_id];
    uint64_t n = ctx->launches[kernel_id];
    if (ctx->slice_ctx)
    {
        double ms2 = 0;
        uint64_t n2 = 0;
        if (lthip_timing_get(ctx->slice_ctx, kernel_id, &ms2, &n2) == 0)
        {
            ms += ms2;
            n += n2;
        }
    }
    if (out_total_ms)
        *out_total_ms = ms;
    if (out_launches)
        *out_launches = n;
    return err;
}

static uint32_t discriminator_from_avg(uint32_t avg)
{
    double a = (double)avg;
    return (uint32_t)(a / (-1.42888852e-7 * a + 1.33237515));
}

static DivTest make_div_test(uint32_t d)
{
    DivTest t;
    memset(&t, 0, sizeof t);
    t.d = d;
    if (d == 0)
        return t;
    uint32_t k2 = 0, dodd = d;
    while ((dodd & 1u) == 0)
    {
        dodd >>= 1;
        ++k2;
    }
    uint32_t inv = dodd;
    for (int i = 0; i < 5; ++i)
        inv *= 2u - dodd * inv;
    t.inv = inv;
    t.k2 = k2;
    t.addc = inv - (1u << k2);
    t.qlim = (uint32_t)(0xFFFFFFFFull / d) - 1u;
    t.pow2 = dodd == 1u;
    return t;
}

extern "C" int lthip_pack_blocks(uint64_t chunk_count, const uint32_t* chunk_lens, uint32_t max_block_size,
                                 uint32_t max_chunks_per_block, uint64_t* block_starts, uint64_t capacity, uint64_t* out_block_count)
{
    if (!out_block_count || (chunk_count && (!chunk_lens || !block_starts)) || max_block_size == 0 || max_chunks_per_block == 0)
        return EINVAL;
    const uint64_t limit = (uint64_t)max_block_size + max_block_size / 10;
    uint64_t i = 0, nb = 0;
    while (i < chunk_count)
    {
        if (nb + 1 >= capacity)
            return ENOMEM;
        block_starts[nb++] = i;
        uint64_t size = chunk_lens[i];
        uint32_t n = 1;
        while (i + 1 < chunk_count && n < max_chunks_per_block && size + chunk_lens[i + 1] <= limit)
        {
            size += chunk_lens[i + 1];
            ++n;
            ++i;
        }
        ++i;
    }
    if (capacity == 0)
        return ENOMEM;
    block_starts[nb] = chunk_count;
    *out_block_count = nb;
    return 0;
}

extern "C" int lthip_pack_blocks_batch(uint64_t chunk_count, const uint32_t* chunk_lens, uint64_t first_chunk,
                                       uint32_t max_block_size, uint32_t max_chunks_per_block, uint64_t max_batch_bytes,
                                       uint64_t arena_bytes, uint32_t bound_div, uint32_t bound_add, uint64_t* block_starts,
                                       uint64_t* block_sizes, uint64_t capacity, uint64_t* out_block_count,
                                       uint64_t* out_next_chunk)
{
    if (!out_block_count || !out_next_chunk || !block_starts || !block_sizes || (chunk_count && !chunk_lens) ||
        max_block_size == 0 || max_chunks_per_block == 0 || bound_div == 0 || capacity < 2 || first_chunk > chunk_count)
        return EINVAL;
    const uint64_t limit = (uint64_t)max_block_size + max_block_size / 10;
    uint64_t i = first_chunk, nb = 0, bytes = 0, arena = 0;
    while (i < chunk_count && nb + 1 < capacity)
    {
        const uint64_t start = i;
        uint64_t size = chunk_lens[i];
        uint32_t n = 1;
        while (i + 1 < chunk_count && n < max_chunks_per_block && size + chunk_lens[i + 1] <= limit)
        {
            size += chunk_lens[i + 1];
            ++n;
            ++i;
        }
        ++i;
        const uint64_t bound = (size + size / bound_div + bound_add + 63u) & ~(uint64_t)63u;
        if (nb && (bytes + size > max_batch_bytes || arena + bound > arena_bytes))
        {
            i = start;
            break;
        }
        block_starts[nb] = start;
        block_sizes[nb] = size;
        ++nb;
        bytes += size;
        arena += bound;
    }
    block_starts[nb] = i;
    *out_block_count = nb;
    *out_next_chunk = i;
    return 0;
}

extern "C" int lthip_store_index_prune(const void* store_index, size_t size, uint32_t keep_count, const uint64_t* keep_block_hashes, void* out,
                                       size_t out_capacity, size_t* out_size)
{
    return lthip_guarded(nullptr, nullptr, [&] { return store_index_ops::prune(store_index, size, keep_count, keep_block_hashes, out, out_capacity, out_size); });
}

extern "C" int lthip_store_index_merge(const void* local, size_t local_size, const void* remote, size_t remote_size, void* out, size_t out_capacity,
                                       size_t* out_size)
{
    return lthip_guarded(nullptr, nullptr, [&] { return store_index_ops::merge(local, local_size, remote, remote_size, out, out_capacity, out_size); });
}

extern "C" int lthip_version_chunk_hashes(const void* version_index, size_t size, uint64_t* out, uint64_t capacity, uint64_t* count)
{
    return store_index_ops::version_chunk_hashes(version_index, size, out, capacity, count);
}

extern "C" int lthip_divtest_eval(uint32_t discriminator, uint32_t hash)
{
    if (discriminator == 0)
        return 0;
    const DivTest t = make_div_test(discriminator);
    if (t.pow2)
        return (hash & (t.d - 1u)) == t.d - 1u;
    const uint32_t m = hash * t.inv + t.addc;
    const uint32_t r = t.k2 ? ((m >> t.k2) | (m << (32u - t.k2))) : m;
    return r <= t.qlim;
}

static uint32_t plan_slice_points(uint32_t part_count, const uint64_t* part_sizes, uint32_t want, uint32_t* first)
{
    if (part_count < 2 || want < 2)
        return 0;
    uint64_t total = 0;
    for (uint32_t p = 0; p < part_count; ++p)
        total += part_sizes[p];
    if (total < LTHIP_SLICE_MIN_BYTES)
        return 0;
    uint32_t S = want > part_count ? part_count : want;
    while (S > 2 && total / S < LTHIP_SLICE_MIN_BYTES / 2)
        --S;
    uint64_t acc = 0;
    uint32_t p = 0;
    first[0] = 0;
    for (uint32_t k = 1; k < S; ++k)
    {
        const uint64_t goal = total / S * k;
        while (p < part_count - (S - k) && acc + part_sizes[p] / 2 < goal)
            acc += part_sizes[p++];
        if (p <= first[k - 1])
        {
            acc += part_sizes[p];
            ++p;
        }
        first[k] = p;
    }
    first[S] = part_count;
    return S;
}

static int plan_layout(lthip_ctx* ctx, const char* what, uint32_t min_chunk, uint32_t part_count, const uint64_t* part_offsets,
                       const uint64_t* part_sizes, PartDev* parts, PlanExtents& x)
{
    memset(&x, 0, sizeof x);
    x.nparts = part_count;
    for (uint32_t p = 0; p < part_count; ++p)
    {
        const uint64_t sz = part_sizes[p];
        if ((part_offsets[p] & 15u) != 0 || sz > 0xFFFFFFFFull)
            return lthip_fail(ctx, EINVAL, what, "part offsets must be 16-byte aligned, sizes < 4 GiB");
        PartDev& pd = parts[p];
        memset(&pd, 0, sizeof pd);
        pd.off = part_offsets[p];
        pd.size = sz;
        pd.bm0_base = x.bm0_words;
        pd.bm1_base = x.bm1_words;
        pd.region_base = x.chunk_cap;
        pd.tile_base = (uint32_t)x.ntiles;
        const uint64_t cap = sz ? sz / min_chunk + 1 : 0;
        pd.region_cap = (uint32_t)cap;
        const uint64_t t = div_up_u64(sz, 16384);
        x.ntiles += t;
        x.bm0_words += t * 256;
        x.bm1_words += t * 4;
        x.chunk_cap += cap;
        x.total_bytes += sz;
        x.leaf_cap += div_up_u64(sz, 1024) + cap;
        x.nonempty_parts += sz != 0;
        x.max_part_bytes = sz > x.max_part_bytes ? sz : x.max_part_bytes;
    }
    return 0;
}

static bool plan_walk_rule(const lthip_plan* plan)
{
    const uint64_t waves = lthip_k1_resident_waves(plan->device);
    return plan->nonempty_parts >= LTHIP_WALK_MIN_PARTS_PER_WAVE * waves &&
           plan->max_part_bytes * LTHIP_WALK_MAX_PART_DIV <= plan->total_bytes / waves;
}

static int plan_create_impl(lthip_ctx* ctx, uint32_t part_count, const uint64_t* part_offsets, const uint64_t* part_sizes,
                            uint32_t min_chunk, uint32_t avg_chunk, uint32_t max_chunk, lthip_plan** out_plan)
{
    if (!ctx || !out_plan || (part_count && (!part_offsets || !part_sizes)))
        return EINVAL;
    *out_plan = nullptr;
    if (min_chunk < 48 || min_chunk > avg_chunk || avg_chunk > max_chunk)
        return lthip_fail(ctx, EINVAL, "lthip_plan_create", "need 48 <= min <= avg <= max");
    uint32_t d = discriminator_from_avg(avg_chunk);
    if (d == 0)
        return lthip_fail(ctx, EINVAL, "lthip_plan_create", "discriminator is zero");
    LTHIP_CHECK(ctx, hipSetDevice(ctx->device));
    std::vector<PartDev> parts(part_count);
    PlanExtents x;
    int err = plan_layout(ctx, "lthip_plan_create", min_chunk, part_count, part_offsets, part_sizes, parts.data(), x);
    if (err)
        return err;
    if (x.ntiles > 0xFFFFFFF0ull)
        return lthip_fail(ctx, EINVAL, "lthip_plan_create", "batch too large");

    lthip_plan* plan = new (std::nothrow) lthip_plan();
    if (!plan)
        return ENOMEM;
    memset(plan, 0, sizeof *plan);
    static_cast<PlanExtents&>(*plan) = x;
    plan->device = ctx->device;
    plan->min_chunk = min_chunk;
    plan->avg_chunk = avg_chunk;
    plan->max_chunk = max_chunk;
    plan->div = make_div_test(d);
    plan->capacity_bytes = x.total_bytes;
    plan->cap_parts = part_count ? part_count : 1;
    plan->cap_tiles = x.ntiles ? x.ntiles : 1;
    plan->walked = plan_walk_rule(plan);

    hipError_t e = lthip_hip_malloc((void**)&plan->d_parts, sizeof(PartDev) * plan->cap_parts);
    if (e == hipSuccess)
        e = lthip_hip_malloc((void**)&plan->d_tile_part, sizeof(uint32_t) * plan->cap_tiles);
    if (e == hipSuccess && part_count)
        e = hipMemcpyAsync(plan->d_parts, parts.data(), sizeof(PartDev) * part_count, hipMemcpyHostToDevice, ctx->stream);
    if (e == hipSuccess)
        e = lthip_stream_wait(ctx);
    if (e != hipSuccess)
    {
        lthip_plan_destroy(ctx, plan);
        return lthip_fail(ctx, e == hipErrorOutOfMemory ? ENOMEM : EIO, "lthip_plan_create", hipGetErrorString(e));
    }
    if ((err = lthip_launch_tile_table(ctx, plan)))
    {
        lthip_plan_destroy(ctx, plan);
        return err;
    }
    *out_plan = plan;
    return 0;
}

static int plan_aim(lthip_ctx* ctx, lthip_plan* plan, const PlanExtents& x, const PartDev* parts)
{
    static_cast<PlanExtents&>(*plan) = x;
    plan->walked = plan_walk_rule(plan);
    const int err = lthip_stage_upload(ctx, plan->d_parts, parts, sizeof(PartDev) * x.nparts, ctx->stream);
    return err ? err : lthip_launch_tile_table(ctx, plan);
}

static bool plan_walks(const lthip_plan* plan);
static void plan_aim_slices(lthip_ctx* ctx, lthip_plan* plan, uint32_t want, const uint64_t* part_offsets, const uint64_t* part_sizes)
{
    plan->sliced = false;
    LTHIP_ABLATION_ENV(env_slices, "LTHIP_SLICES");
    const bool as_one = plan_walks(plan) && env_slices.get() <= 0;
    if (as_one && plan->nslices)
        return;
    uint32_t first[9];
    const uint32_t S = plan_slice_points(plan->nparts, part_sizes, want, first);
    if (S == 0 || (plan->nslices && S != plan->nslices))
        return;
    bool ok = true;
    if (!plan->nslices)
        for (uint32_t k = 0; k < S && ok; ++k)
            ok = plan_create_impl(ctx, first[k + 1] - first[k], part_offsets + first[k], part_sizes + first[k], plan->min_chunk,
                                  plan->avg_chunk, plan->max_chunk, &plan->slice[k]) == 0;
    else
    {
        std::vector<PartDev> parts(plan->nparts);
        PlanExtents x[8];
        for (uint32_t k = 0; k < S && ok; ++k)
        {
            const uint32_t n = first[k + 1] - first[k];
            ok = plan_layout(ctx, "lthip_plan_reaim", plan->min_chunk, n, part_offsets + first[k], part_sizes + first[k], &parts[first[k]],
                             x[k]) == 0 &&
                 n <= plan->slice[k]->cap_parts && x[k].ntiles <= plan->slice[k]->cap_tiles;
        }
        for (uint32_t k = 0; k < S && ok; ++k)
            ok = plan_aim(ctx, plan->slice[k], x[k], &parts[first[k]]) == 0;
    }
    if (!ok)
    {
        if (!plan->nslices)
            for (uint32_t k = 0; k < S; ++k)
            {
                lthip_plan_destroy(ctx, plan->slice[k]);
                plan->slice[k] = nullptr;
            }
        ctx->err[0] = 0;
        return;
    }
    memcpy(plan->slice_first, first, sizeof(uint32_t) * (S + 1));
    plan->nslices = S;
    plan->sliced = !as_one;
}

extern "C" int lthip_plan_create(lthip_ctx* ctx, uint32_t part_count, const uint64_t* part_offsets,
                                 const uint64_t* part_sizes, uint32_t min_chunk, uint32_t avg_chunk, uint32_t max_chunk,
                                 lthip_plan** out_plan)
{
    int err = plan_create_impl(ctx, part_count, part_offsets, part_sizes, min_chunk, avg_chunk, max_chunk, out_plan);
    if (err)
        return err;
    int want = LTHIP_SLICES;
    LTHIP_ABLATION_ENV(env_slices, "LTHIP_SLICES");
    if (env_slices.get() > 0)
        want = env_slices.get() > 8 ? 8 : env_slices.get();
    plan_aim_slices(ctx, *out_plan, (uint32_t)want, part_offsets, part_sizes);
    return 0;
}

extern "C" int lthip_plan_resize_single(lthip_ctx* ctx, lthip_plan* plan, uint64_t size)
{
    if (!ctx || !plan || plan->nparts != 1)
        return EINVAL;
    if (size > plan->capacity_bytes)
        return lthip_fail(ctx, EINVAL, "lthip_plan_resize_single", "size above the capacity the plan was created with");
    LTHIP_CHECK(ctx, hipSetDevice(ctx->device));
    const uint64_t off = 0;
    PartDev pd;
    PlanExtents x;
    const int err = plan_layout(ctx, "lthip_plan_resize_single", plan->min_chunk, 1, &off, &size, &pd, x);
    if (err)
        return err;
    static_cast<PlanExtents&>(*plan) = x;
    return lthip_stage_upload(ctx, plan->d_parts, &pd, sizeof pd, ctx->stream);
}

extern "C" int lthip_plan_reaim(lthip_ctx* ctx, lthip_plan* plan, uint32_t part_count, const uint64_t* part_offsets,
                                const uint64_t* part_sizes)
{
    if (!ctx || !plan || (part_count && (!part_offsets || !part_sizes)))
        return EINVAL;
    if (part_count == 0 || part_count > plan->cap_parts)
        return lthip_fail(ctx, EINVAL, "lthip_plan_reaim", "part count outside 1 .. the count the plan was created with");
    LTHIP_CHECK(ctx, hipSetDevice(ctx->device));
    {
        std::vector<PartDev> parts(part_count);
        PlanExtents x;
        int err = plan_layout(ctx, "lthip_plan_reaim", plan->min_chunk, part_count, part_offsets, part_sizes, parts.data(), x);
        if (err)
            return err;
        if (x.ntiles > plan->cap_tiles)
            return lthip_fail(ctx, EINVAL, "lthip_plan_reaim", "more 16 KiB tiles than the plan was created with");
        if ((err = plan_aim(ctx, plan, x, parts.data())))
            return err;
    }
    if (plan->nslices)
        plan_aim_slices(ctx, plan, plan->nslices, part_offsets, part_sizes);
    return 0;
}

extern "C" void lthip_plan_destroy(lthip_ctx* ctx, lthip_plan* plan)
{
    if (!plan)
        return;
    (void)hipSetDevice(plan->device);
    if (ctx)
        (void)lthip_stream_wait(ctx);
    else
        (void)hipDeviceSynchronize();
    if (plan->d_parts)
        (void)hipFree(plan->d_parts);
    if (plan->d_tile_part)
        (void)hipFree(plan->d_tile_part);
    for (uint32_t k = 0; k < 8; ++k)
        lthip_plan_destroy(ctx, plan->slice[k]);
    delete plan;
}

extern "C" uint64_t lthip_plan_chunk_capacity(const lthip_plan* plan) { return plan ? plan->chunk_cap : 0; }
extern "C" uint32_t lthip_plan_slices(const lthip_plan* plan) { return plan && plan->sliced ? plan->nslices : 1u; }

static bool plan_walks(const lthip_plan* plan)
{
    LTHIP_ABLATION_ENV(env_walk, "LTHIP_K1_WALK");
    if (env_walk.get() >= 0)
        return env_walk.get() != 0 && plan->nparts != 0;
    return plan->walked;
}
extern "C" uint32_t lthip_plan_walked_scans(const lthip_plan* plan)
{
    if (!plan)
        return 0;
    if (!plan->sliced)
        return plan_walks(plan);
    uint32_t n = 0;
    for (uint32_t k = 0; k < plan->nslices; ++k)
        n += plan_walks(plan->slice[k]);
    return n;
}

struct ScanBuffers
{
    uint64_t *bm0, *bm1;
    uint2* region;
    uint32_t* part_count;
};
static int chunk_scan_buffers(lthip_ctx* ctx, const lthip_plan* plan, bool bitmaps, ScanBuffers* b)
{
    b->bm0 = b->bm1 = nullptr;
    int err;
    if (bitmaps && ((err = lthip_scratch(ctx, S_BM0, plan->bm0_words * 8, (void**)&b->bm0)) ||
                    (err = lthip_scratch(ctx, S_BM1, plan->bm1_words * 8, (void**)&b->bm1))))
        return err;
    if ((err = lthip_scratch(ctx, S_REGION, plan->chunk_cap * sizeof(uint2), (void**)&b->region)))
        return err;
    return lthip_scratch(ctx, S_PART_COUNT, ((size_t)plan->nparts + 1) * 4, (void**)&b->part_count);
}

static int chunk_scan(lthip_ctx* ctx, const lthip_plan* plan, const void* d_data, const ScanBuffers& b)
{
    if (!plan->nparts)
        return 0;
    return plan_walks(plan) ? lthip_launch_buzhash_walk(ctx, plan, (const uint8_t*)d_data, b.region, b.part_count)
                            : lthip_launch_buzhash(ctx, plan, (const uint8_t*)d_data, b.bm0, b.bm1);
}

static int chunk_cut_hash(lthip_ctx* ctx, const lthip_plan* plan, const void* d_data, const ScanBuffers& b, uint64_t* d_offsets,
                          uint32_t* d_lens, uint64_t* d_hashes, uint32_t* d_part_first)
{
    int err;
    if (plan->nparts && !plan_walks(plan) && (err = lthip_launch_select(ctx, plan, b.bm0, b.bm1, b.region, b.part_count)))
        return err;
    if ((err = lthip_launch_compact(ctx, plan, b.region, b.part_count, d_part_first, d_offsets, d_lens)))
        return err;
    return d_hashes ? lthip_launch_blake3(ctx, (const uint8_t*)d_data, d_offsets, d_lens, d_part_first + plan->nparts, plan->chunk_cap,
                                          plan->leaf_cap, plan->max_chunk, d_hashes)
                    : 0;
}

__global__ void k_slice_join(const uint64_t* __restrict__ b_off, const uint32_t* __restrict__ b_len, const uint64_t* __restrict__ b_hash,
                             const uint32_t* __restrict__ b_first, uint32_t nparts_b, uint32_t* __restrict__ part_first ,
                             uint64_t* __restrict__ offs, uint32_t* __restrict__ lens, uint64_t* __restrict__ hashes)
{
    const uint32_t base = part_first[0], total_b = b_first[nparts_b];
    const uint64_t i = (uint64_t)blockIdx.x * blockDim.x + threadIdx.x;
    if (i < total_b)
    {
        offs[base + i] = b_off[i];
        lens[base + i] = b_len[i];
        hashes[base + i] = b_hash[i];
    }
    if (i >= 1 && i <= nparts_b)
        part_first[i] = b_first[i] + base;
}

static int chunk_hash_sliced(lthip_ctx* ctx, const lthip_plan* plan, const void* d_data, uint64_t* d_chunk_offsets, uint32_t* d_chunk_lens, uint64_t* d_chunk_hashes, uint32_t* d_part_first,
                             bool* taken)
{
    *taken = false;
    if (!plan->sliced || !d_chunk_hashes)
        return 0;
    if (!ctx->slice_ctx && lthip_ctx_create(ctx->device, LTHIP_STREAM_PRIVATE, &ctx->slice_ctx) != 0)
        return 0;
    lthip_ctx* c2 = ctx->slice_ctx;
    const uint32_t S = plan->nslices;
    uint64_t cap_rest = 0, parts_rest = 0;
    for (uint32_t k = 1; k < S; ++k)
    {
        cap_rest += plan->slice[k]->chunk_cap + 1;
        parts_rest += (uint64_t)plan->slice[k]->nparts + 1;
    }
    void *x_off, *x_len, *x_hash, *x_first;
    ScanBuffers sb;
    const bool bitmaps = lthip_plan_walked_scans(plan) != S;
    if (lthip_scratch(ctx, S_SLICE_OFFS, cap_rest * 8, &x_off) || lthip_scratch(ctx, S_SLICE_LENS, cap_rest * 4, &x_len) ||
        lthip_scratch(ctx, S_SLICE_HASH, cap_rest * 8, &x_hash) || lthip_scratch(ctx, S_SLICE_FIRST, parts_rest * 4, &x_first) ||
        chunk_scan_buffers(ctx, plan, bitmaps, &sb))
    {
        ctx->err[0] = 0;
        return 0;
    }
    *taken = true;
    c2->timing = ctx->timing;

    int err = 0;
    uint64_t co = 0, po = 0;
    uint64_t *offs_k[8], *hash_k[8];
    uint32_t *lens_k[8], *first_k[8];
    for (uint32_t k = 0; k < S && !err; ++k)
    {
        const lthip_plan* pk = plan->slice[k];
        offs_k[k] = k ? (uint64_t*)x_off + co : d_chunk_offsets;
        lens_k[k] = k ? (uint32_t*)x_len + co : d_chunk_lens;
        hash_k[k] = k ? (uint64_t*)x_hash + co : d_chunk_hashes;
        first_k[k] = k ? (uint32_t*)x_first + po : d_part_first;
        co += k ? pk->chunk_cap + 1 : 0;
        po += k ? (uint64_t)pk->nparts + 1 : 0;
        if ((err = chunk_scan(ctx, pk, d_data, sb)))
            break;
        hipEvent_t scanned = lthip_sync_event(ctx);
        hipError_t e = hipEventRecord(scanned, ctx->stream);
        if (e == hipSuccess)
            e = hipStreamWaitEvent(c2->stream, scanned, 0);
        if (e != hipSuccess)
            err = lthip_fail(ctx, EIO, "lthip_chunk_hash (the wait of the second stream for a scan)", hipGetErrorString(e));
        else if ((err = chunk_cut_hash(c2, pk, d_data, sb, offs_k[k], lens_k[k], hash_k[k], first_k[k])))
            (void)lthip_fail(ctx, err, "lthip_chunk_hash (a slice on the second stream)", c2->err);
        if (bitmaps)
        {
            sb.bm0 += pk->bm0_words;
            sb.bm1 += pk->bm1_words;
        }
        sb.region += pk->chunk_cap;
        sb.part_count += pk->nparts;
    }
    hipEvent_t hashed = lthip_sync_event(ctx);
    hipError_t e = hipEventRecord(hashed, c2->stream);
    if (e == hipSuccess)
        e = hipStreamWaitEvent(ctx->stream, hashed, 0);
    if (e != hipSuccess)
    {
        (void)hipStreamSynchronize(c2->stream);
        if (!err)
            err = lthip_fail(ctx, EIO, "lthip_chunk_hash (the join of the second stream)", hipGetErrorString(e));
    }
    if (!err)
    {
        LaunchTimer t(ctx, LTHIP_K_COMPACT);
        for (uint32_t k = 1; k < S; ++k)
        {
            const lthip_plan* pk = plan->slice[k];
            const uint64_t n = pk->chunk_cap > (uint64_t)pk->nparts + 1 ? pk->chunk_cap : (uint64_t)pk->nparts + 1;
            hipLaunchKernelGGL(k_slice_join, dim3((uint32_t)div_up_u64(n, 256)), dim3(256), 0, ctx->stream, (const uint64_t*)offs_k[k], (const uint32_t*)lens_k[k],
                               (const uint64_t*)hash_k[k], (const uint32_t*)first_k[k], pk->nparts, d_part_first + plan->slice_first[k], d_chunk_offsets,
                               d_chunk_lens, d_chunk_hashes);
        }
        if ((e = hipGetLastError()) != hipSuccess)
            err = lthip_fail(ctx, EIO, "kernel launch", hipGetErrorString(e));
    }
    return err;
}

extern "C" int lthip_chunk_hash(lthip_ctx* ctx, const lthip_plan* plan, const void* d_data, uint64_t* d_chunk_offsets,
                                uint32_t* d_chunk_lens, uint64_t* d_chunk_hashes, uint32_t* d_part_first,
                                uint64_t* out_total)
{
    if (!ctx || !plan || !d_chunk_offsets || !d_chunk_lens || !d_part_first || (plan->total_bytes && !d_data))
        return EINVAL;
    LTHIP_CHECK(ctx, hipSetDevice(ctx->device));
    bool sliced;
    int err = chunk_hash_sliced(ctx, plan, d_data, d_chunk_offsets, d_chunk_lens, d_chunk_hashes, d_part_first, &sliced);
    ScanBuffers sb;
    if (!sliced && !(err = chunk_scan_buffers(ctx, plan, !plan_walks(plan), &sb)) && !(err = chunk_scan(ctx, plan, d_data, sb)))
        err = chunk_cut_hash(ctx, plan, d_data, sb, d_chunk_offsets, d_chunk_lens, d_chunk_hashes, d_part_first);
    if (err)
        return err;
    if (out_total)
    {
        uint32_t total = 0;
        LTHIP_CHECK(ctx, hipMemcpyAsync(&total, d_part_first + plan->nparts, 4, hipMemcpyDeviceToHost, ctx->stream));
        LTHIP_CHECK(ctx, lthip_stream_wait(ctx));
        *out_total = total;
    }
    return 0;
}

extern "C" int lthip_chunk_from_buffer(lthip_ctx* ctx, const void* d_data, uint64_t size, uint32_t min_chunk,
                                       uint32_t avg_chunk, uint32_t max_chunk, uint64_t* out_len)
{
    if (!ctx || !d_data || !out_len || size == 0)
        return EINVAL;
    if (min_chunk < 48 || min_chunk > avg_chunk || avg_chunk > max_chunk)
        return lthip_fail(ctx, EINVAL, "lthip_chunk_from_buffer", "need 48 <= min <= avg <= max");
    if (size <= min_chunk)
    {
        *out_len = size;
        return 0;
    }
    const uint32_t d = discriminator_from_avg(avg_chunk);
    if (d == 0)
        return lthip_fail(ctx, EINVAL, "lthip_chunk_from_buffer", "discriminator is zero");
    LTHIP_CHECK(ctx, hipSetDevice(ctx->device));
    void* d_out;
    int err = lthip_scratch(ctx, S_MISC, 64, &d_out);
    if (err)
        return err;
    const uint32_t n = (uint32_t)(size > max_chunk ? max_chunk : size);
    if ((err = lthip_launch_from_buffer(ctx, (const uint8_t*)d_data, n, min_chunk, make_div_test(d), (uint64_t*)d_out)))
        return err;
    uint64_t len = 0;
    LTHIP_CHECK(ctx, hipMemcpyAsync(&len, d_out, 8, hipMemcpyDeviceToHost, ctx->stream));
    LTHIP_CHECK(ctx, lthip_stream_wait(ctx));
    *out_len = len;
    return 0;
}
```

### longtail_amd/csrc/lthip_internal.h

```cpp
#pragma once

#include <hip/hip_runtime.h>

#include <errno.h>
#include <stdint.h>
#include <stdio.h>
#include <stdlib.h>
#include <string.h>

#include <atomic>
#include <new>
#include <vector>

#include "../../include/longtail_hip.h"

struct PartDev
{
    uint64_t off;
    uint64_t size;
    uint64_t bm0_base;
    uint64_t bm1_base;
    uint64_t region_base;
    uint32_t tile_base;
    uint32_t region_cap;
};

struct DivTest
{
    uint32_t d;
    uint32_t inv;
    uint32_t addc;
    uint32_t k2;
    uint32_t qlim;
    uint32_t pow2;
};

struct PlanExtents
{
    uint32_t nparts;
    uint64_t total_bytes;
    uint64_t ntiles;
    uint64_t chunk_cap;
    uint64_t bm0_words;
    uint64_t bm1_words;
    uint64_t leaf_cap;
    uint32_t nonempty_parts;
    uint64_t max_part_bytes;
};

struct lthip_plan : PlanExtents
{
    int device;
    uint32_t min_chunk, avg_chunk, max_chunk;
    DivTest div;
    uint64_t capacity_bytes;
    uint32_t cap_parts;
    uint64_t cap_tiles;
    PartDev* d_parts;
    uint32_t* d_tile_part;
    lthip_plan* slice[8];
    uint32_t slice_first[9];
    uint32_t nslices;
    bool sliced;
    bool walked;
};
constexpr uint32_t LTHIP_WALK_MIN_PARTS_PER_WAVE = 2;
constexpr uint32_t LTHIP_WALK_MAX_PART_DIV = 2;
constexpr uint64_t LTHIP_SLICE_MIN_BYTES = 1ull << 30;
#ifndef LTHIP_SLICES
#define LTHIP_SLICES 2
#endif

enum ScratchSlot
{
    S_BM0 = 0,
    S_BM1,
    S_REGION,
    S_PART_COUNT,
    S_LEAF_COUNT,
    S_LEAF_PREFIX,
    S_SCAN_TMP,
    S_CV,
    S_LZ4_SEGS,
    S_LZ4_META,
    S_LZ4_STREAM,
    S_LZ4_BLOCKS,
    S_TABLES,
    S_TABLES2,
    S_MISC,
    S_Z_LITS,
    S_Z_RECS,
    S_Z_ENC,
    S_Z_WORK,
    S_Z_SUB,
    S_LZ4_WORKLIST,
    S_LZ4_CLASSIFY,
    S_B3_WINDOWS,
    S_Z_FR,
    S_Z_ORG,
    S_Z_PERM,
    S_XCHG,
    S_XCHG2,
    S_SLICE_OFFS,
    S_SLICE_LENS,
    S_SLICE_HASH,
    S_SLICE_FIRST,
    S_LEN_CLASS_ORDER,
    S_WALK_TICKET,
    S_RAW_BLOCKS,
    S_RAW_RUNS,
    S_RAW_TABLES,
    S_CARRY_RUNS,
    S_ARCHIVE_ITEMS,
    S_COUNT
};

struct TimingRec
{
    int kid;
    hipEvent_t a, b;
};

struct lthip_ctx
{
    int device;
    hipStream_t stream;
    bool own_stream;
    lthip_ctx* slice_ctx;
    hipStream_t stream2;
    std::vector<hipEvent_t> sync_events;
    size_t sync_next;
    char err[320];
    struct Stage
    {
        void* p;
        size_t cap;
        hipEvent_t done;
        bool used;
    };
    Stage stage[8], stage_small[64];
    size_t stage_small_next;
    size_t stage_next;
    bool k1_lds_enabled;
    bool k5_lds_enabled[2][2];
    bool k5h_lds_enabled[2];
    void* scratch[S_COUNT];
    size_t scratch_cap[S_COUNT];
    bool timing;
    std::vector<TimingRec> pending;
    std::vector<hipEvent_t> free_events;
    const uint32_t* z_last_retry;
    uint32_t z_last_payloads, z_last_foreign_blocks;
    double total_ms[LTHIP_K_COUNT];
    uint64_t launches[LTHIP_K_COUNT];
};

int lthip_fail(lthip_ctx* ctx, int code, const char* what, const char* detail);
template <class F> int lthip_guarded(lthip_ctx* ctx, const char* who, F&& f)
{
    try
    {
        return f();
    }
    catch (const std::bad_alloc&)
    {
        return lthip_fail(ctx, ENOMEM, who, "host tables");
    }
}
hipError_t lthip_stream_wait(lthip_ctx* ctx);

extern volatile uint32_t g_lthip_env_gen;
struct LthipEnvInt
{
    const char* name;
    std::atomic<int> value{-1};
    std::atomic<uint32_t> seen{0};
    explicit LthipEnvInt(const char* n) : name(n) {}
    int get()
    {
        const uint32_t gen = g_lthip_env_gen;
        if (seen.load(std::memory_order_acquire) != gen)
        {
            const char* e = getenv(name);
            value.store(e ? atoi(e) : -1, std::memory_order_relaxed);
            seen.store(gen, std::memory_order_release);
        }
        return value.load(std::memory_order_relaxed);
    }
};
#ifdef LTHIP_ABLATIONS
#define LTHIP_ABLATION_ENV(var, name) static LthipEnvInt var{name}
#else
struct LthipEnvOff
{
    constexpr int get() const { return -1; }
};
#define LTHIP_ABLATION_ENV(var, name) constexpr LthipEnvOff var{}
#endif
#ifdef LTHIP_ABLATIONS
hipError_t lthip_hip_malloc(void** p, size_t bytes);
hipError_t lthip_hip_host_malloc(void** p, size_t bytes, unsigned flags);
#else
static inline hipError_t lthip_hip_malloc(void** p, size_t bytes) { return hipMalloc(p, bytes); }
static inline hipError_t lthip_hip_host_malloc(void** p, size_t bytes, unsigned flags) { return hipHostMalloc(p, bytes, flags); }
#endif
int lthip_scratch(lthip_ctx* ctx, int slot, size_t bytes, void** out);
lthip_ctx* lthip_store_ctx(const lthip_store* store);
int lthip_second_stream(lthip_ctx* ctx, hipStream_t* out);
hipEvent_t lthip_sync_event(lthip_ctx* ctx);
constexpr uint32_t LTHIP_ZSTD_CHAIN = 8;
uint64_t lthip_codec_batch_bytes();
uint64_t lthip_origin_budget_mib();
constexpr size_t LTHIP_STAGE_SMALL = 64u << 10;
int lthip_stage_upload(lthip_ctx* ctx, void* d_dst, const void* h_src, size_t bytes, hipStream_t stream);

#define LTHIP_CHECK(ctx, expr)                                                          \
    do                                                                                  \
    {                                                                                   \
        hipError_t e__ = (expr);                                                        \
        if (e__ != hipSuccess)                                                          \
            return lthip_fail((ctx), e__ == hipErrorOutOfMemory ? ENOMEM : EIO, #expr, hipGetErrorString(e__)); \
    } while (0)

struct LaunchTimer
{
    lthip_ctx* ctx;
    TimingRec rec;
    bool on;
    hipStream_t stream;
    LaunchTimer(lthip_ctx* c, int kid, hipStream_t s = nullptr);
    ~LaunchTimer();
};

#define LTHIP_LAUNCH_CHECK(ctx)                                                          \
    do                                                                                   \
    {                                                                                    \
        hipError_t e__ = hipGetLastError();                                              \
        if (e__ != hipSuccess)                                                           \
            return lthip_fail((ctx), EIO, "kernel launch", hipGetErrorString(e__));      \
    } while (0)

int lthip_launch_tile_table(lthip_ctx* ctx, lthip_plan* plan);
int lthip_launch_buzhash(lthip_ctx* ctx, const lthip_plan* plan, const uint8_t* d_data, uint64_t* bm0, uint64_t* bm1);
int lthip_launch_buzhash_walk(lthip_ctx* ctx, const lthip_plan* plan, const uint8_t* d_data, uint2* region, uint32_t* part_count);
uint32_t lthip_k1_resident_waves(int device);
int lthip_launch_select(lthip_ctx* ctx, const lthip_plan* plan, const uint64_t* bm0, const uint64_t* bm1, uint2* region,
                        uint32_t* part_count);
int lthip_raw_copy_blocks(lthip_ctx* ctx, uint32_t count, const uint32_t* h_first, const uint32_t* h_count, const uint64_t* h_payload,
                          uint32_t chunk_base, uint32_t chunk_span, const uint32_t* d_lens, const uint64_t* d_src_offsets, const void* d_src,
                          void* d_arena, uint64_t bytes_bound);
int lthip_raw_copy_runs(lthip_ctx* ctx, const uint32_t* d_first_piece, uint32_t slots, const uint64_t* d_run_src, const uint64_t* d_run_dst,
                        const uint64_t* d_run_len, const void* d_src, void* d_dst, uint64_t pieces_bound);
constexpr uint32_t LTHIP_RAW_PIECE_VEC = 2048;
__device__ __forceinline__ uint32_t lthip_raw_pieces(uint64_t dst, uint64_t len)
{
    if (len == 0)
        return 0u;
    uint64_t head = (16u - (dst & 15u)) & 15u;
    if (head > len)
        head = len;
    const uint64_t nvec = (len - head) >> 4;
    return nvec ? (uint32_t)((nvec + LTHIP_RAW_PIECE_VEC - 1) / LTHIP_RAW_PIECE_VEC) : 1u;
}
struct BlockBatchDev
{
    const void* places[3];
    uint32_t nplaces;
    const uint64_t* d_hashes;
    const uint32_t* d_lens;
    uint32_t chunk_base;
    const uint64_t* d_raw_offsets;
    const void* d_raw_src;
    const uint64_t* d_bhash;
    uint32_t* d_comp;
    void* d_arena;
};
struct BlockBatch;
struct BlockImageBufs;
struct Ranges;
int lthip_gather_upload(lthip_ctx* ctx, BlockImageBufs& w, const void* d_src, const Ranges& r, void* d_dst);
int lthip_block_payloads(lthip_ctx* ctx, BlockImageBufs& w, BlockBatch& bt, const BlockBatchDev& dev);
int lthip_block_headers_upload(lthip_ctx* ctx, BlockImageBufs& w, const BlockBatch& bt, bool with_tags);
int lthip_block_headers(lthip_ctx* ctx, const BlockImageBufs& w, const BlockBatch& bt, const BlockBatchDev& dev, const lthip_ingest_config& cfg,
                        bool with_tags);
int lthip_launch_block_headers(lthip_ctx* ctx, int kid, const uint32_t* d_block_first_chunk, uint32_t nblocks, const uint64_t* d_chunk_hashes,
                               const uint32_t* d_chunk_lens, const uint64_t* d_block_hashes, uint32_t hash_identifier, uint32_t tag,
                               const uint32_t* d_block_tags, const uint32_t* d_raw_sizes, uint32_t* d_comp_sizes, const uint64_t* d_image_offsets,
                               void* d_arena, uint32_t raw_mode);
int lthip_launch_compact(lthip_ctx* ctx, const lthip_plan* plan, const uint2* region, const uint32_t* part_count,
                         uint32_t* d_part_first, uint64_t* d_chunk_offsets, uint32_t* d_chunk_lens);
int lthip_exclusive_scan_u32(lthip_ctx* ctx, const uint32_t* d_in, uint32_t* d_out, uint64_t n_bound, const uint32_t* d_n,
                             int kid);
int lthip_launch_blake3(lthip_ctx* ctx, const uint8_t* d_data, const uint64_t* d_offsets, const uint32_t* d_lens,
                        const uint32_t* d_count, uint64_t count_bound, uint64_t leaf_bound, uint64_t max_len,
                        uint64_t* d_hashes);

int lthip_hash_ranges_known(lthip_ctx* ctx, const void* d_data, uint64_t range_count, const uint64_t* d_offsets, const uint32_t* d_lens,
                            uint32_t max_len, uint64_t leaf_total, uint64_t* d_hashes);

int lthip_launch_blake3_stream_batch(lthip_ctx* ctx, const void* d_data, uint32_t leaf0, uint32_t* d_stack, uint32_t depth_in, uint32_t merges);
int lthip_launch_blake3_stream_final(lthip_ctx* ctx, const void* d_tail, uint32_t tail_len, uint32_t leaf0, const uint32_t* d_stack,
                                     uint32_t depth, uint64_t* d_out);
int lthip_launch_blake3_one(lthip_ctx* ctx, const void* in, uint32_t len, uint64_t* out);

struct ChainHash
{
    int (*ranges)(lthip_ctx* ctx, const uint8_t* d_data, const uint64_t* d_offsets, const uint32_t* d_lens, const uint32_t* d_count,
                  uint64_t count_bound, uint64_t* d_hashes);
    int (*one)(lthip_ctx* ctx, const void* in, uint32_t len, uint64_t* out);
    int (*stream)(lthip_ctx* ctx, const void* d_data, uint32_t len, uint32_t* d_state, int first, int final, uint64_t* d_out);
    uint32_t stream_batch;
};
const ChainHash* lthip_chain_blake2s();
const ChainHash* lthip_chain_meow();
int lthip_len_class_order(lthip_ctx* ctx, const uint32_t* d_lens, const uint32_t* d_count, uint64_t count_bound, uint32_t unit_shift,
                          uint32_t long_class, const uint32_t** order, const uint32_t** n_long);

constexpr uint32_t LTHIP_HASH_BLAKE3 = 0x626c6b33u;
constexpr uint32_t LTHIP_HASH_BLAKE2 = 0x626c6b32u;
constexpr uint32_t LTHIP_HASH_MEOW = 0x6d656f77u;
const ChainHash* lthip_chain_hash(uint32_t hash_identifier);
int lthip_hash_ranges_by_id(lthip_ctx* ctx, uint32_t hash_identifier, const void* d_data, uint64_t range_count, const uint64_t* d_offsets,
                            const uint32_t* d_lens, uint32_t max_len, uint64_t leaf_total, uint64_t* d_hashes);

int lthip_launch_from_buffer(lthip_ctx* ctx, const uint8_t* d_data, uint32_t n, uint32_t min_chunk, const DivTest& dv,
                             uint64_t* d_out);

int lthip_launch_lz_sequences(lthip_ctx* ctx, const void* d_src, uint32_t block_count, const uint64_t* src_offsets,
                              const uint32_t* src_sizes, void* d_dst, const uint64_t* dst_offsets, const uint32_t* dst_caps,
                              uint8_t** d_lits, uint64_t** d_recs, void** d_meta, uint32_t* unit_base, uint64_t* total_units, int quality);

struct lthip_occurrence_list
{
    uint32_t hash_identifier;
    uint64_t count;
    const uint64_t* d_hash;
    const uint32_t* d_len;
    const uint64_t* d_dst;
};
int lthip_restore_create_occurrences(lthip_ctx* ctx, const lthip_restore_config* cfg, const lthip_occurrence_list* list, const void* store_index,
                                     size_t si_size, uint64_t out_bytes, const char* who, lthip_restore** out);
uint64_t lthip_restore_outstanding(const lthip_restore* r);

static inline uint64_t div_up_u64(uint64_t a, uint64_t b) { return (a + b - 1) / b; }
```

Measured before the change: 918.9.

## Fuse BLAKE3 leaf hashing into the buzhash chunk walk kernel

The buzhash walk kernel now computes BLAKE3 leaf chaining values while it scans data for chunk boundaries, writing them into per-part run buffers. A new run-slot kernel either maps each chunk to its run slot or moves the CVs into place, and the windowed parent kernel reads CVs through that slot indirection. This is meant to avoid a second pass over the input bytes for leaf hashing, at the cost of extra scratch memory, more register pressure in the walk kernel, and an indirect load in the parent stage.

```diff
diff --git a/longtail_amd/csrc/k_blake3.hip b/longtail_amd/csrc/k_blake3.hip
--- a/longtail_amd/csrc/k_blake3.hip
+++ b/longtail_amd/csrc/k_blake3.hip
@@ -5,73 +5,8 @@
 namespace
 {
 
-enum
-{
-    F_CHUNK_START = 1,
-    F_CHUNK_END = 2,
-    F_PARENT = 4,
-    F_ROOT = 8
-};
-
-#define B3_IV0 0x6A09E667u
-#define B3_IV1 0xBB67AE85u
-#define B3_IV2 0x3C6EF372u
-#define B3_IV3 0xA54FF53Au
-#define B3_IV4 0x510E527Fu
-#define B3_IV5 0x9B05688Cu
-#define B3_IV6 0x1F83D9ABu
-#define B3_IV7 0x5BE0CD19u
-
-__device__ __forceinline__ uint32_t rotr32(uint32_t x, uint32_t r) { return __builtin_amdgcn_alignbit(x, x, r); }
-
-__device__ __forceinline__ void b3_g(uint32_t& a, uint32_t& b, uint32_t& c, uint32_t& d, uint32_t mx, uint32_t my)
-{
-    a = a + b + mx;
-    d = rotr32(d ^ a, 16);
-    c = c + d;
-    b = rotr32(b ^ c, 12);
-    a = a + b + my;
-    d = rotr32(d ^ a, 8);
-    c = c + d;
-    b = rotr32(b ^ c, 7);
-}
-
-#define B3_ROUND(m0, m1, m2, m3, m4, m5, m6, m7, m8, m9, m10, m11, m12, m13, m14, m15) \
-    b3_g(s0, s4, s8, s12, m0, m1);                                                      \
-    b3_g(s1, s5, s9, s13, m2, m3);                                                      \
-    b3_g(s2, s6, s10, s14, m4, m5);                                                     \
-    b3_g(s3, s7, s11, s15, m6, m7);                                                     \
-    b3_g(s0, s5, s10, s15, m8, m9);                                                     \
-    b3_g(s1, s6, s11, s12, m10, m11);                                                   \
-    b3_g(s2, s7, s8, s13, m12, m13);                                                    \
-    b3_g(s3, s4, s9, s14, m14, m15);
-
-__device__ __forceinline__ void b3_compress(uint32_t (&cv)[8], const uint32_t (&m)[16], uint32_t counter_lo,
-                                            uint32_t block_len, uint32_t flags)
-{
-    uint32_t s0 = cv[0], s1 = cv[1], s2 = cv[2], s3 = cv[3], s4 = cv[4], s5 = cv[5], s6 = cv[6], s7 = cv[7];
-    uint32_t s8 = B3_IV0, s9 = B3_IV1, s10 = B3_IV2, s11 = B3_IV3;
-    uint32_t s12 = counter_lo, s13 = 0u, s14 = block_len, s15 = flags;
-    B3_ROUND(m[0], m[1], m[2], m[3], m[4], m[5], m[6], m[7], m[8], m[9], m[10], m[11], m[12], m[13], m[14], m[15])
-    B3_ROUND(m[2], m[6], m[3], m[10], m[7], m[0], m[4], m[13], m[1], m[11], m[12], m[5], m[9], m[14], m[15], m[8])
-    B3_ROUND(m[3], m[4], m[10], m[12], m[13], m[2], m[7], m[14], m[6], m[5], m[9], m[0], m[11], m[15], m[8], m[1])
-    B3_ROUND(m[10], m[7], m[12], m[9], m[14], m[3], m[13], m[15], m[4], m[0], m[11], m[2], m[5], m[8], m[1], m[6])
-    B3_ROUND(m[12], m[13], m[9], m[11], m[15], m[10], m[14], m[8], m[7], m[2], m[5], m[3], m[0], m[1], m[6], m[4])
-    B3_ROUND(m[9], m[14], m[11], m[5], m[8], m[12], m[15], m[1], m[13], m[3], m[0], m[10], m[2], m[6], m[4], m[7])
-    B3_ROUND(m[11], m[15], m[5], m[0], m[1], m[9], m[8], m[6], m[14], m[10], m[2], m[12], m[3], m[4], m[7], m[13])
-    cv[0] = s0 ^ s8;
-    cv[1] = s1 ^ s9;
-    cv[2] = s2 ^ s10;
-    cv[3] = s3 ^ s11;
-    cv[4] = s4 ^ s12;
-    cv[5] = s5 ^ s13;
-    cv[6] = s6 ^ s14;
-    cv[7] = s7 ^ s15;
-}
-
-typedef uint32_t u32x4_a4 __attribute__((ext_vector_type(4), aligned(4)));
-
-__device__ __forceinline__ uint32_t leaves_of(uint32_t len) { return len ? (len + 1023u) >> 10 : 1u; }
+#include "k_blake3_leaf.h"
+
 
 __global__ void k_leaf_counts(const uint32_t* __restrict__ lens, uint64_t bound, const uint32_t* __restrict__ n_dev,
                               uint32_t* __restrict__ counts)
@@ -105,60 +40,6 @@
 static_assert(PW <= 4096 && (PW & (PW - 1)) == 0 && PW_THREADS % 64 == 0 && PW_MAXN >> PJ <= 255, "window tables are 16 bits, list entries 16 + 8 + 8");
 
 
-__device__ __forceinline__ void b3_load_interior(uint32_t (&w)[17], const uint32_t* __restrict__ src)
-{
-    const u32x4_a4 v0 = *reinterpret_cast<const u32x4_a4*>(src);
-    const u32x4_a4 v1 = *reinterpret_cast<const u32x4_a4*>(src + 4);
-    const u32x4_a4 v2 = *reinterpret_cast<const u32x4_a4*>(src + 8);
-    const u32x4_a4 v3 = *reinterpret_cast<const u32x4_a4*>(src + 12);
-    w[0] = v0.x; w[1] = v0.y; w[2] = v0.z; w[3] = v0.w;
-    w[4] = v1.x; w[5] = v1.y; w[6] = v1.z; w[7] = v1.w;
-    w[8] = v2.x; w[9] = v2.y; w[10] = v2.z; w[11] = v2.w;
-    w[12] = v3.x; w[13] = v3.y; w[14] = v3.z; w[15] = v3.w;
-    w[16] = src[16];
-}
-
-__device__ __forceinline__ void b3_load_last(uint32_t (&w)[17], const uint32_t* __restrict__ src, uint32_t nd)
-{
-#pragma unroll
-    for (int i = 0; i < 17; ++i)
-        w[i] = (uint32_t)i < nd ? src[i] : 0u;
-}
-
-__device__ __forceinline__ void b3_interior_block(uint32_t (&cv)[8], uint32_t (&w)[17], uint32_t sh, uint32_t k, uint32_t flags)
-{
-#pragma unroll
-    for (int i = 0; i < 16; ++i)
-        asm("v_alignbit_b32 %0, %1, %0, %2" : "+v"(w[i]) : "v"(w[i + 1]), "v"(sh));
-    uint32_t m[16];
-#pragma unroll
-    for (int i = 0; i < 16; ++i)
-        m[i] = w[i];
-    b3_compress(cv, m, k, 64u, flags);
-}
-
-__device__ __forceinline__ void b3_last_block(uint32_t (&cv)[8], const uint32_t (&w)[17], uint32_t sh, uint32_t k, uint32_t bl, uint32_t flags)
-{
-    uint32_t m[16];
-#pragma unroll
-    for (int i = 0; i < 16; ++i)
-    {
-        uint32_t v = __builtin_amdgcn_alignbit(w[i + 1], w[i], sh);
-        const int rem = (int)bl - 4 * i;
-        if (rem <= 0)
-            v = 0u;
-        else if (rem < 4)
-            v &= (1u << (8 * rem)) - 1u;
-        m[i] = v;
-    }
-    b3_compress(cv, m, k, bl, flags);
-}
-
-__device__ __forceinline__ void b3_pin(uint32_t (&cv)[8])
-{
-    asm volatile("" : "+v"(cv[0]), "+v"(cv[1]), "+v"(cv[2]), "+v"(cv[3]), "+v"(cv[4]), "+v"(cv[5]), "+v"(cv[6]), "+v"(cv[7])::"memory");
-}
-
 template <bool PIPE>
 __global__ __launch_bounds__(256, 8) void k_blake3_leaves(const uint8_t* __restrict__ data,
                                                        const uint64_t* __restrict__ offsets,
@@ -202,49 +83,7 @@
 
     if constexpr (PIPE)
     {
-        const uint32_t last = nblocks - 1u;
-        const uint32_t bl = llen - last * 64u;
-        const uint32_t nd = bl ? (mis + bl + 3u) >> 2 : 0u;
-        uint32_t wa[17], wb[17];
-        uint32_t b = 0;
-        bool first_half = last > 1u && ((last - 1u) & 1u) == 0u;
-        if (last > 1u && !first_half)
-            b3_load_interior(wb, q);
-        else if (last)
-            b3_load_interior(wa, q);
-        if (last > 1u)
-        {
-#pragma unroll 1
-            for (;;)
-            {
-                if (first_half)
-                {
-                    b3_load_interior(wb, q + (b + 1u) * 16u);
-                    b3_pin(cv);
-                    b3_interior_block(cv, wa, sh, k, b == 0 ? (uint32_t)F_CHUNK_START : 0u);
-                    b3_pin(cv);
-                    ++b;
-                }
-                first_half = true;
-                b3_load_interior(wa, q + (b + 1u) * 16u);
-                b3_pin(cv);
-                b3_interior_block(cv, wb, sh, k, b == 0 ? (uint32_t)F_CHUNK_START : 0u);
-                b3_pin(cv);
-                ++b;
-                if (b + 1u >= last)
-                    break;
-            }
-        }
-        if (last)
-        {
-            b3_load_last(wb, q + last * 16u, nd);
-            b3_pin(cv);
-            b3_interior_block(cv, wa, sh, k, b == 0 ? (uint32_t)F_CHUNK_START : 0u);
-            b3_pin(cv);
-        }
-        else
-            b3_load_last(wb, q, nd);
-        b3_last_block(cv, wb, sh, k, bl, (uint32_t)F_CHUNK_END | root | (last == 0 ? (uint32_t)F_CHUNK_START : 0u));
+#include "k_blake3_leaf_body.inc"
     }
     else
     {
@@ -518,7 +357,8 @@
 
 __global__ __launch_bounds__(PW_THREADS, PW_WAVES) void k_blake3_parents_window(const uint32_t* __restrict__ leaf_prefix, uint64_t count_bound,
                                                                          const uint32_t* __restrict__ n_dev, const uint32_t* __restrict__ cvs,
-                                                                         const uint32_t* __restrict__ win_first, uint64_t* __restrict__ hashes)
+                                                                         const uint32_t* __restrict__ win_first, uint64_t* __restrict__ hashes,
+                                                                         const uint32_t* __restrict__ run_slot)
 {
     __shared__ uint4 s_mem[PW_MEM16];
     __shared__ uint32_t s_list[2][PW_NODES / 2 + 1];
@@ -616,7 +456,7 @@
             const uint32_t j = lo, b = blk - s_blk[j];
             const uint32_t p = s_leaf[j], n = s_leaf[j + 1] - p, nb = b3s_blocks(n, PB);
             const uint32_t m = b3s_block_leaves(n, b, PB);
-            const uint4* g = cvs4 + (p + b * PB) * 2u;
+            const uint4* g = run_slot ? reinterpret_cast<const uint4*>(cvs) + ((uint64_t)run_slot[c_lo + j] + b * PB) * 2u : cvs4 + (p + b * PB) * 2u;
             uint32_t cv[PB][8];
 #pragma unroll
             for (uint32_t i = 0; i < PB; ++i)
@@ -722,11 +562,73 @@
     hashes[c] = (uint64_t)base[0] | ((uint64_t)base[1] << 32);
 }
 
-}
+template <bool MOVE>
+__global__ __launch_bounds__(256) void k_blake3_run_slots(const PartDev* __restrict__ parts, uint32_t nparts,
+                                                           const uint32_t* __restrict__ part_first,
+                                                           const uint32_t* __restrict__ leaf_prefix, const uint4* __restrict__ runs,
+                                                           uint4* __restrict__ cvs, uint32_t* __restrict__ run_slot,
+                                                           uint32_t* __restrict__ win_first)
+{
+    const uint32_t p = blockIdx.x;
+    if (p >= nparts)
+        return;
+    const uint32_t c0 = part_first[p], c1 = part_first[p + 1];
+    const uint32_t g0 = leaf_prefix[c0], g1 = leaf_prefix[c1];
+    if constexpr (MOVE)
+    {
+        const uint4* src = runs + lthip_part_run_base(parts[p]) * 2u;
+        uint4* dst = cvs + (uint64_t)g0 * 2u;
+        const uint32_t n = (g1 - g0) * 2u;
+        for (uint32_t i = threadIdx.x; i < n; i += 256u)
+            dst[i] = src[i];
+    }
+    else
+    {
+        const uint32_t base = (uint32_t)lthip_part_run_base(parts[p]) - g0;
+        for (uint32_t c = c0 + threadIdx.x; c < c1; c += 256u)
+            run_slot[c] = base + leaf_prefix[c];
+    }
+    if (!win_first)
+        return;
+    for (uint64_t g = (((uint64_t)g0 + (uint32_t)(PW - 1)) & ~(uint64_t)(PW - 1)) + (uint64_t)threadIdx.x * PW; g < g1; g += 256u * (uint64_t)PW)
+    {
+        uint32_t lo = c0, hi = c1;
+        while (hi - lo > 1)
+        {
+            const uint32_t mid = lo + ((hi - lo) >> 1);
+            if (leaf_prefix[mid] <= g)
+                lo = mid;
+            else
+                hi = mid;
+        }
+        win_first[g / (uint32_t)PW] = leaf_prefix[lo] == g ? lo : lo + 1u;
+    }
+}
+
+#ifndef B3_RUNS_IN_PLACE
+#define B3_RUNS_IN_PLACE 1
+#endif
+
+}
+
+static int launch_blake3(lthip_ctx* ctx, const uint8_t* d_data, const uint64_t* d_offsets, const uint32_t* d_lens, const uint32_t* d_count,
+                         uint64_t count_bound, uint64_t leaf_bound, uint64_t max_len, uint64_t* d_hashes, const lthip_b3_runs* runs);
 
 int lthip_launch_blake3(lthip_ctx* ctx, const uint8_t* d_data, const uint64_t* d_offsets, const uint32_t* d_lens,
                         const uint32_t* d_count, uint64_t count_bound, uint64_t leaf_bound, uint64_t max_len,
                         uint64_t* d_hashes)
+{
+    return launch_blake3(ctx, d_data, d_offsets, d_lens, d_count, count_bound, leaf_bound, max_len, d_hashes, nullptr);
+}
+
+int lthip_launch_blake3_parents(lthip_ctx* ctx, const lthip_b3_runs& runs, const uint32_t* d_lens, const uint32_t* d_count,
+                                uint64_t count_bound, uint64_t leaf_bound, uint64_t max_len, uint64_t* d_hashes)
+{
+    return launch_blake3(ctx, nullptr, nullptr, d_lens, d_count, count_bound, leaf_bound, max_len, d_hashes, &runs);
+}
+
+static int launch_blake3(lthip_ctx* ctx, const uint8_t* d_data, const uint64_t* d_offsets, const uint32_t* d_lens, const uint32_t* d_count,
+                         uint64_t count_bound, uint64_t leaf_bound, uint64_t max_len, uint64_t* d_hashes, const lthip_b3_runs* runs)
 {
     if (count_bound == 0)
         return 0;
@@ -774,6 +676,23 @@
     void* wf = nullptr;
     if (small_trees && (err = lthip_scratch(ctx, S_B3_WINDOWS, (leaf_bound / PW + 2) * 4, &wf)))
         return err;
+    LTHIP_ABLATION_ENV(env_serial, "LTHIP_B3_SERIAL_PARENTS");
+    void* slots = nullptr;
+    if (runs && small_trees && B3_RUNS_IN_PLACE && env_serial.get() < 0 &&
+        (err = lthip_scratch(ctx, S_CV_SLOTS, (count_bound + 1) * 4, &slots)))
+        return err;
+    if (runs)
+    {
+        LaunchTimer t(ctx, LTHIP_K_B3_LEAF);
+        if (slots)
+            hipLaunchKernelGGL(k_blake3_run_slots<false>, dim3(runs->nparts), dim3(256), 0, ctx->stream, runs->d_parts, runs->nparts,
+                               runs->d_part_first, (const uint32_t*)lp, (const uint4*)runs->d_cvs, (uint4*)nullptr, (uint32_t*)slots, (uint32_t*)wf);
+        else
+            hipLaunchKernelGGL(k_blake3_run_slots<true>, dim3(runs->nparts), dim3(256), 0, ctx->stream, runs->d_parts, runs->nparts,
+                               runs->d_part_first, (const uint32_t*)lp, (const uint4*)runs->d_cvs, (uint4*)cv, (uint32_t*)nullptr, (uint32_t*)wf);
+        LTHIP_LAUNCH_CHECK(ctx);
+    }
+    else
     {
         LaunchTimer t(ctx, LTHIP_K_B3_LEAF);
         LTHIP_ABLATION_ENV(env_pad, "LTHIP_B3_PAD_LDS");
@@ -793,14 +712,14 @@
     {
         LaunchTimer t(ctx, LTHIP_K_B3_PARENT);
 #ifdef LTHIP_ABLATIONS
-        LTHIP_ABLATION_ENV(env_serial, "LTHIP_B3_SERIAL_PARENTS");
         if (env_serial.get() >= 0)
             hipLaunchKernelGGL(k_blake3_parents_small, dim3((uint32_t)div_up_u64(count_bound, 256)), dim3(256), 0, ctx->stream,
                                d_lens, (const uint32_t*)lp, count_bound, d_count, (uint32_t*)cv, d_hashes);
         else
 #endif
             hipLaunchKernelGGL(k_blake3_parents_window, dim3((uint32_t)div_up_u64(leaf_bound, PW)), dim3(PW_THREADS), 0, ctx->stream,
-                               (const uint32_t*)lp, count_bound, d_count, (const uint32_t*)cv, (const uint32_t*)wf, d_hashes);
+                               (const uint32_t*)lp, count_bound, d_count, slots ? runs->d_cvs : (const uint32_t*)cv, (const uint32_t*)wf, d_hashes,
+                               (const uint32_t*)slots);
         LTHIP_LAUNCH_CHECK(ctx);
     }
     else
diff --git a/longtail_amd/csrc/k_blake3_leaf.h b/longtail_amd/csrc/k_blake3_leaf.h
--- /dev/null
+++ b/longtail_amd/csrc/k_blake3_leaf.h
@@ -0,0 +1,141 @@
+#pragma once
+
+enum
+{
+    F_CHUNK_START = 1,
+    F_CHUNK_END = 2,
+    F_PARENT = 4,
+    F_ROOT = 8
+};
+
+#define B3_IV0 0x6A09E667u
+#define B3_IV1 0xBB67AE85u
+#define B3_IV2 0x3C6EF372u
+#define B3_IV3 0xA54FF53Au
+#define B3_IV4 0x510E527Fu
+#define B3_IV5 0x9B05688Cu
+#define B3_IV6 0x1F83D9ABu
+#define B3_IV7 0x5BE0CD19u
+
+__device__ __forceinline__ uint32_t b3_rotr32(uint32_t x, uint32_t r) { return __builtin_amdgcn_alignbit(x, x, r); }
+
+__device__ __forceinline__ void b3_g(uint32_t& a, uint32_t& b, uint32_t& c, uint32_t& d, uint32_t mx, uint32_t my)
+{
+    a = a + b + mx;
+    d = b3_rotr32(d ^ a, 16);
+    c = c + d;
+    b = b3_rotr32(b ^ c, 12);
+    a = a + b + my;
+    d = b3_rotr32(d ^ a, 8);
+    c = c + d;
+    b = b3_rotr32(b ^ c, 7);
+}
+
+#define B3_ROUND(m0, m1, m2, m3, m4, m5, m6, m7, m8, m9, m10, m11, m12, m13, m14, m15) \
+    b3_g(s0, s4, s8, s12, m0, m1);                                                      \
+    b3_g(s1, s5, s9, s13, m2, m3);                                                      \
+    b3_g(s2, s6, s10, s14, m4, m5);                                                     \
+    b3_g(s3, s7, s11, s15, m6, m7);                                                     \
+    b3_g(s0, s5, s10, s15, m8, m9);                                                     \
+    b3_g(s1, s6, s11, s12, m10, m11);                                                   \
+    b3_g(s2, s7, s8, s13, m12, m13);                                                    \
+    b3_g(s3, s4, s9, s14, m14, m15);
+
+__device__ __forceinline__ void b3_compress(uint32_t (&cv)[8], const uint32_t (&m)[16], uint32_t counter_lo,
+                                            uint32_t block_len, uint32_t flags)
+{
+    uint32_t s0 = cv[0], s1 = cv[1], s2 = cv[2], s3 = cv[3], s4 = cv[4], s5 = cv[5], s6 = cv[6], s7 = cv[7];
+    uint32_t s8 = B3_IV0, s9 = B3_IV1, s10 = B3_IV2, s11 = B3_IV3;
+    uint32_t s12 = counter_lo, s13 = 0u, s14 = block_len, s15 = flags;
+    B3_ROUND(m[0], m[1], m[2], m[3], m[4], m[5], m[6], m[7], m[8], m[9], m[10], m[11], m[12], m[13], m[14], m[15])
+    B3_ROUND(m[2], m[6], m[3], m[10], m[7], m[0], m[4], m[13], m[1], m[11], m[12], m[5], m[9], m[14], m[15], m[8])
+    B3_ROUND(m[3], m[4], m[10], m[12], m[13], m[2], m[7], m[14], m[6], m[5], m[9], m[0], m[11], m[15], m[8], m[1])
+    B3_ROUND(m[10], m[7], m[12], m[9], m[14], m[3], m[13], m[15], m[4], m[0], m[11], m[2], m[5], m[8], m[1], m[6])
+    B3_ROUND(m[12], m[13], m[9], m[11], m[15], m[10], m[14], m[8], m[7], m[2], m[5], m[3], m[0], m[1], m[6], m[4])
+    B3_ROUND(m[9], m[14], m[11], m[5], m[8], m[12], m[15], m[1], m[13], m[3], m[0], m[10], m[2], m[6], m[4], m[7])
+    B3_ROUND(m[11], m[15], m[5], m[0], m[1], m[9], m[8], m[6], m[14], m[10], m[2], m[12], m[3], m[4], m[7], m[13])
+    cv[0] = s0 ^ s8;
+    cv[1] = s1 ^ s9;
+    cv[2] = s2 ^ s10;
+    cv[3] = s3 ^ s11;
+    cv[4] = s4 ^ s12;
+    cv[5] = s5 ^ s13;
+    cv[6] = s6 ^ s14;
+    cv[7] = s7 ^ s15;
+}
+
+typedef uint32_t u32x4_a4 __attribute__((ext_vector_type(4), aligned(4)));
+
+__device__ __forceinline__ uint32_t leaves_of(uint32_t len) { return len ? (len + 1023u) >> 10 : 1u; }
+
+__device__ __forceinline__ void b3_load_interior(uint32_t (&w)[17], const uint32_t* __restrict__ src)
+{
+    const u32x4_a4 v0 = *reinterpret_cast<const u32x4_a4*>(src);
+    const u32x4_a4 v1 = *reinterpret_cast<const u32x4_a4*>(src + 4);
+    const u32x4_a4 v2 = *reinterpret_cast<const u32x4_a4*>(src + 8);
+    const u32x4_a4 v3 = *reinterpret_cast<const u32x4_a4*>(src + 12);
+    w[0] = v0.x; w[1] = v0.y; w[2] = v0.z; w[3] = v0.w;
+    w[4] = v1.x; w[5] = v1.y; w[6] = v1.z; w[7] = v1.w;
+    w[8] = v2.x; w[9] = v2.y; w[10] = v2.z; w[11] = v2.w;
+    w[12] = v3.x; w[13] = v3.y; w[14] = v3.z; w[15] = v3.w;
+    w[16] = src[16];
+}
+
+__device__ __forceinline__ void b3_load_last(uint32_t (&w)[17], const uint32_t* __restrict__ src, uint32_t nd)
+{
+#pragma unroll
+    for (int i = 0; i < 17; ++i)
+        w[i] = (uint32_t)i < nd ? src[i] : 0u;
+}
+
+__device__ __forceinline__ void b3_interior_block(uint32_t (&cv)[8], uint32_t (&w)[17], uint32_t sh, uint32_t k, uint32_t flags)
+{
+#pragma unroll
+    for (int i = 0; i < 16; ++i)
+        asm("v_alignbit_b32 %0, %1, %0, %2" : "+v"(w[i]) : "v"(w[i + 1]), "v"(sh));
+    uint32_t m[16];
+#pragma unroll
+    for (int i = 0; i < 16; ++i)
+        m[i] = w[i];
+    b3_compress(cv, m, k, 64u, flags);
+}
+
+__device__ __forceinline__ void b3_last_block(uint32_t (&cv)[8], const uint32_t (&w)[17], uint32_t sh, uint32_t k, uint32_t bl, uint32_t flags)
+{
+    uint32_t m[16];
+#pragma unroll
+    for (int i = 0; i < 16; ++i)
+    {
+        uint32_t v = __builtin_amdgcn_alignbit(w[i + 1], w[i], sh);
+        const int rem = (int)bl - 4 * i;
+        if (rem <= 0)
+            v = 0u;
+        else if (rem < 4)
+            v &= (1u << (8 * rem)) - 1u;
+        m[i] = v;
+    }
+    b3_compress(cv, m, k, bl, flags);
+}
+
+__device__ __forceinline__ void b3_pin(uint32_t (&cv)[8])
+{
+    asm volatile("" : "+v"(cv[0]), "+v"(cv[1]), "+v"(cv[2]), "+v"(cv[3]), "+v"(cv[4]), "+v"(cv[5]), "+v"(cv[6]), "+v"(cv[7])::"memory");
+}
+
+__device__ __forceinline__ void b3_leaf(uint32_t (&out)[8], const uint8_t* p, uint32_t rlen, uint32_t k)
+{
+    const uint32_t nleaf = leaves_of(rlen);
+    const uint32_t llen = rlen - (k << 10) < 1024u ? rlen - (k << 10) : 1024u;
+    const uint32_t root = nleaf == 1u ? (uint32_t)F_ROOT : 0u;
+    const uint32_t mis = (uint32_t)((uintptr_t)p & 3u);
+    const uint32_t sh = mis * 8u;
+    const uint32_t* q = reinterpret_cast<const uint32_t*>(p - mis);
+    uint32_t cv[8] = {B3_IV0, B3_IV1, B3_IV2, B3_IV3, B3_IV4, B3_IV5, B3_IV6, B3_IV7};
+    const uint32_t nblocks = llen ? (llen + 63u) >> 6 : 1u;
+    {
+#include "k_blake3_leaf_body.inc"
+    }
+#pragma unroll
+    for (int i = 0; i < 8; ++i)
+        out[i] = cv[i];
+}
diff --git a/longtail_amd/csrc/k_blake3_leaf_body.inc b/longtail_amd/csrc/k_blake3_leaf_body.inc
--- /dev/null
+++ b/longtail_amd/csrc/k_blake3_leaf_body.inc
@@ -0,0 +1,43 @@
+const uint32_t last = nblocks - 1u;
+const uint32_t bl = llen - last * 64u;
+const uint32_t nd = bl ? (mis + bl + 3u) >> 2 : 0u;
+uint32_t wa[17], wb[17];
+uint32_t b = 0;
+bool first_half = last > 1u && ((last - 1u) & 1u) == 0u;
+if (last > 1u && !first_half)
+    b3_load_interior(wb, q);
+else if (last)
+    b3_load_interior(wa, q);
+if (last > 1u)
+{
+#pragma unroll 1
+    for (;;)
+    {
+        if (first_half)
+        {
+            b3_load_interior(wb, q + (b + 1u) * 16u);
+            b3_pin(cv);
+            b3_interior_block(cv, wa, sh, k, b == 0 ? (uint32_t)F_CHUNK_START : 0u);
+            b3_pin(cv);
+            ++b;
+        }
+        first_half = true;
+        b3_load_interior(wa, q + (b + 1u) * 16u);
+        b3_pin(cv);
+        b3_interior_block(cv, wb, sh, k, b == 0 ? (uint32_t)F_CHUNK_START : 0u);
+        b3_pin(cv);
+        ++b;
+        if (b + 1u >= last)
+            break;
+    }
+}
+if (last)
+{
+    b3_load_last(wb, q + last * 16u, nd);
+    b3_pin(cv);
+    b3_interior_block(cv, wa, sh, k, b == 0 ? (uint32_t)F_CHUNK_START : 0u);
+    b3_pin(cv);
+}
+else
+    b3_load_last(wb, q, nd);
+b3_last_block(cv, wb, sh, k, bl, (uint32_t)F_CHUNK_END | root | (last == 0 ? (uint32_t)F_CHUNK_START : 0u));
diff --git a/longtail_amd/csrc/k_buzhash.hip b/longtail_amd/csrc/k_buzhash.hip
--- a/longtail_amd/csrc/k_buzhash.hip
+++ b/longtail_amd/csrc/k_buzhash.hip
@@ -9,6 +9,8 @@
 __constant__ uint32_t c_buztab[256] = {
 #include "buzhash_table.inc"
 };
+
+#include "k_blake3_leaf.h"
 
 constexpr int RUN = 64;
 constexpr int TILE = 256 * RUN;
@@ -707,6 +709,242 @@
 #endif
 }
 
+constexpr int PEND_CAP = 64;
+
+template <int MODE, int WAVES, bool GUESS>
+__global__ __launch_bounds__(64 * WAVES, 1) void k_buzhash_hash_walk(const uint8_t* __restrict__ data, const PartDev* __restrict__ parts,
+                                                                      uint32_t nparts, DivTest dv, uint32_t min_chunk, uint32_t max_chunk,
+                                                                      uint2* __restrict__ region, uint32_t* __restrict__ part_count,
+                                                                      uint32_t* __restrict__ ticket, uint32_t* __restrict__ cv_runs)
+{
+    extern __shared__ __attribute__((aligned(16))) uint32_t smem[];
+    const int tid = threadIdx.x;
+    const int lane = tid & 63;
+    const int wave = __builtin_amdgcn_readfirstlane(tid >> 6);
+    uint32_t* buf = smem + 256 * TAB_REP + wave * ((DMA_BUF_B >> 2) + HALO_DW);
+    uint32_t* halo = buf + (DMA_BUF_B >> 2);
+    uint4* pend = reinterpret_cast<uint4*>(smem + 256 * TAB_REP + WAVES * ((DMA_BUF_B >> 2) + HALO_DW)) + wave * PEND_CAP;
+    prefix_table_init(smem, tid, 64 * WAVES);
+
+    const TileDma dma(data, buf, lane);
+    const PrefixConsts pc = dma.consts<MODE>(dv);
+    const int lane_base = lane * RUN;
+
+    auto jump = [](uint64_t q) __attribute__((always_inline)) { return q >= 64 ? ((q - 64) & ~(uint64_t)15) + 64 : (uint64_t)0; };
+
+    bool inflight = false;
+    uint64_t inflight_tb = 0;
+#ifdef LTHIP_ABLATIONS
+    uint32_t tiles = 0;
+#endif
+    uint32_t pn = 0, pl = 0, phead = 0, last_nl = 0;
+    bool have = false, scanning = false, drained = false;
+    PartDev pd = {};
+    uint32_t t = 0, n = 0, end = 0, slot = 0;
+    uint64_t size = 0, s = 0, qlo = 0, qhi = 0, tb = 0;
+    uint2* out = region;
+
+    auto emit = [&](uint32_t len) __attribute__((always_inline))
+    {
+        if (lane == 0)
+        {
+            const uint64_t at = pd.off + s;
+            out[n] = make_uint2((uint32_t)s, len);
+            pend[pn] = make_uint4((uint32_t)at, (uint32_t)(at >> 32), len, slot);
+        }
+        last_nl = leaves_of(len);
+        ++n;
+        ++pn;
+        pl += last_nl;
+        slot += last_nl;
+        s += len;
+    };
+    auto classify = [&](uint32_t& len) __attribute__((always_inline)) -> bool
+    {
+        const uint64_t left = size - s;
+        len = left <= min_chunk ? (uint32_t)left : left > max_chunk ? max_chunk : (uint32_t)left;
+        if (!(left > min_chunk && len > min_chunk))
+            return false;
+        end = len;
+        qlo = s + min_chunk;
+        qhi = s + end - 1;
+        return true;
+    };
+
+    for (;;)
+    {
+        if (pl >= 64u || (drained && pl != 0u))
+        {
+            asm volatile("" ::: "memory");
+            __builtin_amdgcn_wave_barrier();
+            const bool has = (uint32_t)lane < pn;
+            const uint4 e = pend[has ? lane : 0];
+            const uint32_t cnt = has ? leaves_of(e.z) - (lane == 0 ? phead : 0u) : 0u;
+            uint32_t incl = cnt;
+            incl += (uint32_t)__builtin_amdgcn_update_dpp(0, (int)incl, 0x111, 0xf, 0xf, false);
+            incl += (uint32_t)__builtin_amdgcn_update_dpp(0, (int)incl, 0x112, 0xf, 0xf, false);
+            incl += (uint32_t)__builtin_amdgcn_update_dpp(0, (int)incl, 0x114, 0xf, 0xf, false);
+            incl += (uint32_t)__builtin_amdgcn_update_dpp(0, (int)incl, 0x118, 0xf, 0xf, false);
+            incl += (uint32_t)__builtin_amdgcn_update_dpp(0, (int)incl, 0x142, 0xa, 0xf, false);
+            incl += (uint32_t)__builtin_amdgcn_update_dpp(0, (int)incl, 0x143, 0xc, 0xf, false);
+            const uint32_t excl = incl - cnt;
+            if (!has)
+                incl = 0xFFFFFFFFu;
+            const uint32_t take = pl < 64u ? pl : 64u;
+            uint32_t j = 0;
+#pragma unroll
+            for (uint32_t step = 32u; step; step >>= 1)
+                if ((uint32_t)__builtin_amdgcn_ds_bpermute((int)((j + step - 1u) * 4u), (int)incl) <= (uint32_t)lane)
+                    j += step;
+            const bool on = (uint32_t)lane < take;
+            if (!on)
+                j = 0;
+            const uint32_t k = (uint32_t)lane - (uint32_t)__builtin_amdgcn_ds_bpermute((int)(j * 4u), (int)excl) + (j == 0u ? phead : 0u);
+            const uint4 c = pend[j];
+            if (on)
+            {
+                uint32_t cv[8];
+                b3_leaf(cv, data + (((uint64_t)c.y << 32) | c.x) + ((uint64_t)k << 10), c.z, k);
+                uint4* o = reinterpret_cast<uint4*>(cv_runs + (uint64_t)(c.w + k) * 8u);
+                o[0] = make_uint4(cv[0], cv[1], cv[2], cv[3]);
+                o[1] = make_uint4(cv[4], cv[5], cv[6], cv[7]);
+            }
+            pl -= take;
+            if (pl != 0u)
+            {
+                const uint32_t li = pn - 1u;
+                const uint4 l = make_uint4(__builtin_amdgcn_readlane(e.x, li), __builtin_amdgcn_readlane(e.y, li),
+                                           __builtin_amdgcn_readlane(e.z, li), __builtin_amdgcn_readlane(e.w, li));
+                if (lane == 0)
+                    pend[0] = l;
+                phead = last_nl - pl;
+                pn = 1;
+            }
+            else
+                pn = 0, phead = 0;
+            asm volatile("" ::: "memory");
+            __builtin_amdgcn_wave_barrier();
+            continue;
+        }
+        if (drained)
+            break;
+        if (!have)
+        {
+            __builtin_amdgcn_wave_barrier();
+            t = atomicAdd(ticket, lane == 0 ? 1u : 0u);
+            t = __builtin_amdgcn_readfirstlane(t);
+            if (t >= nparts)
+            {
+                drained = true;
+                continue;
+            }
+            pd = parts[t];
+            size = pd.size;
+            out = region + pd.region_base;
+            slot = (uint32_t)lthip_part_run_base(pd);
+            s = 0;
+            n = 0;
+            have = true;
+            scanning = false;
+        }
+        if (!scanning)
+        {
+            if (s >= size)
+            {
+                if (inflight)
+                {
+                    asm volatile("s_waitcnt vmcnt(0)" ::: "memory");
+                    inflight = false;
+                }
+                if (lane == 0)
+                    part_count[t] = n;
+                have = false;
+                continue;
+            }
+            uint32_t len;
+            if (!classify(len))
+            {
+                emit(len);
+                continue;
+            }
+            tb = jump(qlo);
+            scanning = true;
+        }
+
+        auto ends_here = [&]() __attribute__((always_inline)) { return (uint32_t)(qhi - tb) < (uint32_t)WTILE; };
+        if (!(inflight && inflight_tb == tb))
+        {
+            if (inflight)
+                asm volatile("s_waitcnt vmcnt(0)" ::: "memory");
+            dma.issue(pd, tb);
+        }
+        inflight = false;
+        uint32_t win[16], hb;
+        dma.take(win, hb, pc);
+        if (GUESS)
+        {
+            uint64_t g = tb + (uint64_t)WTILE;
+            bool aim = true;
+            if (ends_here())
+            {
+                const uint64_t s2 = s + end;
+                aim = size - s2 > min_chunk && max_chunk > min_chunk;
+                g = jump(s2 + min_chunk);
+            }
+            if (aim)
+            {
+                dma.issue(pd, g);
+                inflight = true;
+                inflight_tb = g;
+            }
+        }
+        const uint64_t raw = prefix_tile<MODE>(win, hb, pc, dv, lane, halo);
+#ifdef LTHIP_ABLATIONS
+        ++tiles;
+#endif
+        for (;;)
+        {
+            const int lo = (int)(qlo > tb ? qlo - tb : 0) - lane_base;
+            const int hi = (int)(ends_here() ? (uint32_t)(qhi - tb) : (uint32_t)WTILE - 1u) - lane_base;
+            uint64_t m = raw;
+            if (lo > 0)
+                m = lo > 63 ? 0ull : m & (~0ull << lo);
+            if (hi < 63)
+                m = hi < 0 ? 0ull : m & ((2ull << hi) - 1ull);
+            const uint64_t any = __builtin_amdgcn_ballot_w64(m != 0ull);
+            uint32_t len;
+            if (any != 0ull)
+            {
+                const int f = __builtin_ctzll(any);
+                const uint64_t q = tb + (uint64_t)(f * RUN + __builtin_ctzll(bcast64(m, f)));
+                len = (uint32_t)(q - s) + 1u;
+            }
+            else if (ends_here())
+                len = end;
+            else
+            {
+                tb += (uint64_t)WTILE;
+                break;
+            }
+            emit(len);
+            uint32_t plain;
+            if (s >= size || !classify(plain))
+            {
+                scanning = false;
+                break;
+            }
+            if ((uint32_t)(qlo - tb) < (uint32_t)WTILE && pl < 64u)
+                continue;
+            tb = jump(qlo);
+            break;
+        }
+    }
+#ifdef LTHIP_ABLATIONS
+    if (lane == 0 && tiles)
+        atomicAdd(&g_walk_tiles, (unsigned long long)tiles);
+#endif
+}
+
 constexpr int SCAN_THREADS = 256;
 constexpr int SCAN_ITEMS = 8;
 constexpr int SCAN_BLOCK = SCAN_THREADS * SCAN_ITEMS;
@@ -1015,18 +1253,26 @@
 #define K1_WALK_GUESS 1
 #endif
 
-template <bool GUESS>
-static int launch_buzhash_walk(lthip_ctx* ctx, const lthip_plan* plan, const uint8_t* d_data, uint2* region, uint32_t* part_count)
+template <bool GUESS, bool HASH>
+static int launch_buzhash_walk(lthip_ctx* ctx, const lthip_plan* plan, const uint8_t* d_data, uint2* region, uint32_t* part_count,
+                               uint32_t* cv_runs)
 {
     constexpr int WAVES = 16;
-    const size_t lds = sizeof(uint32_t) * (256 * TAB_REP + WAVES * ((DMA_BUF_B >> 2) + HALO_DW));
+    constexpr size_t lds = sizeof(uint32_t) * (256 * TAB_REP + WAVES * ((DMA_BUF_B >> 2) + HALO_DW))
+                           + (HASH ? sizeof(uint4) * WAVES * PEND_CAP : 0);
+    static_assert(lds <= 160 * 1024 && (sizeof(uint32_t) * (256 * TAB_REP + WAVES * ((DMA_BUF_B >> 2) + HALO_DW))) % 16 == 0,
+                  "LDS budget: one workgroup per CU; the lists are 16-byte aligned");
     auto k0 = &k_buzhash_walk<0, WAVES, GUESS>;
     auto k1 = &k_buzhash_walk<1, WAVES, GUESS>;
+    auto h0 = &k_buzhash_hash_walk<0, WAVES, GUESS>;
+    auto h1 = &k_buzhash_hash_walk<1, WAVES, GUESS>;
     static bool granted[64] = {};
     if (ctx->device < 0 || ctx->device >= 64 || !granted[ctx->device])
     {
-        LTHIP_CHECK(ctx, hipFuncSetAttribute(reinterpret_cast<const void*>(k0), hipFuncAttributeMaxDynamicSharedMemorySize, (int)lds));
-        LTHIP_CHECK(ctx, hipFuncSetAttribute(reinterpret_cast<const void*>(k1), hipFuncAttributeMaxDynamicSharedMemorySize, (int)lds));
+        LTHIP_CHECK(ctx, hipFuncSetAttribute(HASH ? reinterpret_cast<const void*>(h0) : reinterpret_cast<const void*>(k0),
+                                             hipFuncAttributeMaxDynamicSharedMemorySize, (int)lds));
+        LTHIP_CHECK(ctx, hipFuncSetAttribute(HASH ? reinterpret_cast<const void*>(h1) : reinterpret_cast<const void*>(k1),
+                                             hipFuncAttributeMaxDynamicSharedMemorySize, (int)lds));
         if (ctx->device >= 0 && ctx->device < 64)
             granted[ctx->device] = true;
     }
@@ -1039,22 +1285,29 @@
         grid = (uint32_t)div_up_u64(plan->nparts, WAVES);
     LaunchTimer t(ctx, LTHIP_K_BUZHASH);
     LTHIP_CHECK(ctx, hipMemsetAsync(ticket, 0, 4, ctx->stream));
-    hipLaunchKernelGGL(plan->div.pow2 ? k1 : k0, dim3(grid), dim3(64 * WAVES), lds, ctx->stream, d_data, plan->d_parts, plan->nparts,
-                       plan->div, plan->min_chunk, plan->max_chunk, region, part_count, (uint32_t*)ticket);
+    if (HASH)
+        hipLaunchKernelGGL(plan->div.pow2 ? h1 : h0, dim3(grid), dim3(64 * WAVES), lds, ctx->stream, d_data, plan->d_parts, plan->nparts,
+                           plan->div, plan->min_chunk, plan->max_chunk, region, part_count, (uint32_t*)ticket, cv_runs);
+    else
+        hipLaunchKernelGGL(plan->div.pow2 ? k1 : k0, dim3(grid), dim3(64 * WAVES), lds, ctx->stream, d_data, plan->d_parts, plan->nparts,
+                           plan->div, plan->min_chunk, plan->max_chunk, region, part_count, (uint32_t*)ticket);
     LTHIP_LAUNCH_CHECK(ctx);
     return 0;
 }
 
-int lthip_launch_buzhash_walk(lthip_ctx* ctx, const lthip_plan* plan, const uint8_t* d_data, uint2* region, uint32_t* part_count)
+int lthip_launch_buzhash_walk(lthip_ctx* ctx, const lthip_plan* plan, const uint8_t* d_data, uint2* region, uint32_t* part_count,
+                              uint32_t* cv_runs)
 {
     if (plan->nparts == 0)
         return 0;
 #ifdef LTHIP_ABLATIONS
     LTHIP_ABLATION_ENV(env_guess, "LTHIP_K1_WALK_GUESS");
     if (env_guess.get() >= 0 && (env_guess.get() != 0) != (K1_WALK_GUESS != 0))
-        return launch_buzhash_walk<!K1_WALK_GUESS>(ctx, plan, d_data, region, part_count);
-#endif
-    return launch_buzhash_walk<K1_WALK_GUESS != 0>(ctx, plan, d_data, region, part_count);
+        return cv_runs ? launch_buzhash_walk<!K1_WALK_GUESS, true>(ctx, plan, d_data, region, part_count, cv_runs)
+                       : launch_buzhash_walk<!K1_WALK_GUESS, false>(ctx, plan, d_data, region, part_count, nullptr);
+#endif
+    return cv_runs ? launch_buzhash_walk<K1_WALK_GUESS != 0, true>(ctx, plan, d_data, region, part_count, cv_runs)
+                   : launch_buzhash_walk<K1_WALK_GUESS != 0, false>(ctx, plan, d_data, region, part_count, nullptr);
 }
 
 extern "C" int lthip_debug_walk_tiles(uint64_t* out_tiles)
diff --git a/longtail_amd/csrc/lthip_ctx.hip b/longtail_amd/csrc/lthip_ctx.hip
--- a/longtail_amd/csrc/lthip_ctx.hip
+++ b/longtail_amd/csrc/lthip_ctx.hip
@@ -848,16 +848,34 @@
     return n;
 }
 
+#ifndef LTHIP_WALK_HASH
+#define LTHIP_WALK_HASH 1
+#endif
+static bool plan_walk_hashes(const lthip_plan* plan, bool hashes)
+{
+    LTHIP_ABLATION_ENV(env_fused, "LTHIP_WALK_HASH");
+    const bool on = env_fused.get() >= 0 ? env_fused.get() != 0 : LTHIP_WALK_HASH != 0;
+    return on && hashes && plan_walks(plan) && lthip_plan_run_slots(plan) <= 0xFFFFFFF0ull;
+}
+uint64_t lthip_plan_run_slots(const lthip_plan* plan) { return plan->chunk_cap + 16u * plan->ntiles; }
+
 struct ScanBuffers
 {
     uint64_t *bm0, *bm1;
     uint2* region;
     uint32_t* part_count;
+    uint32_t* cv_runs;
 };
-static int chunk_scan_buffers(lthip_ctx* ctx, const lthip_plan* plan, bool bitmaps, ScanBuffers* b)
+static int chunk_scan_buffers(lthip_ctx* ctx, const lthip_plan* plan, bool bitmaps, bool hashes, ScanBuffers* b)
 {
     b->bm0 = b->bm1 = nullptr;
+    b->cv_runs = nullptr;
     int err;
+    bool runs = !plan->sliced && plan_walk_hashes(plan, hashes);
+    for (uint32_t k = 0; plan->sliced && k < plan->nslices; ++k)
+        runs |= plan_walk_hashes(plan->slice[k], hashes);
+    if (runs && (err = lthip_scratch(ctx, S_CV_RUNS, lthip_plan_run_slots(plan) * 32, (void**)&b->cv_runs)))
+        return err;
     if (bitmaps && ((err = lthip_scratch(ctx, S_BM0, plan->bm0_words * 8, (void**)&b->bm0)) ||
                     (err = lthip_scratch(ctx, S_BM1, plan->bm1_words * 8, (void**)&b->bm1))))
         return err;
@@ -870,7 +888,8 @@
 {
     if (!plan->nparts)
         return 0;
-    return plan_walks(plan) ? lthip_launch_buzhash_walk(ctx, plan, (const uint8_t*)d_data, b.region, b.part_count)
+    return plan_walks(plan) ? lthip_launch_buzhash_walk(ctx, plan, (const uint8_t*)d_data, b.region, b.part_count,
+                                                        plan_walk_hashes(plan, b.cv_runs != nullptr) ? b.cv_runs : nullptr)
                             : lthip_launch_buzhash(ctx, plan, (const uint8_t*)d_data, b.bm0, b.bm1);
 }
 
@@ -882,9 +901,13 @@
         return err;
     if ((err = lthip_launch_compact(ctx, plan, b.region, b.part_count, d_part_first, d_offsets, d_lens)))
         return err;
-    return d_hashes ? lthip_launch_blake3(ctx, (const uint8_t*)d_data, d_offsets, d_lens, d_part_first + plan->nparts, plan->chunk_cap,
-                                          plan->leaf_cap, plan->max_chunk, d_hashes)
-                    : 0;
+    if (!d_hashes)
+        return 0;
+    if (plan_walk_hashes(plan, b.cv_runs != nullptr))
+        return lthip_launch_blake3_parents(ctx, lthip_b3_runs{b.cv_runs, plan->d_parts, plan->nparts, d_part_first}, d_lens,
+                                           d_part_first + plan->nparts, plan->chunk_cap, plan->leaf_cap, plan->max_chunk, d_hashes);
+    return lthip_launch_blake3(ctx, (const uint8_t*)d_data, d_offsets, d_lens, d_part_first + plan->nparts, plan->chunk_cap, plan->leaf_cap,
+                               plan->max_chunk, d_hashes);
 }
 
 __global__ void k_slice_join(const uint64_t* __restrict__ b_off, const uint32_t* __restrict__ b_len, const uint64_t* __restrict__ b_hash,
@@ -924,7 +947,7 @@
     const bool bitmaps = lthip_plan_walked_scans(plan) != S;
     if (lthip_scratch(ctx, S_SLICE_OFFS, cap_rest * 8, &x_off) || lthip_scratch(ctx, S_SLICE_LENS, cap_rest * 4, &x_len) ||
         lthip_scratch(ctx, S_SLICE_HASH, cap_rest * 8, &x_hash) || lthip_scratch(ctx, S_SLICE_FIRST, parts_rest * 4, &x_first) ||
-        chunk_scan_buffers(ctx, plan, bitmaps, &sb))
+        chunk_scan_buffers(ctx, plan, bitmaps, true, &sb))
     {
         ctx->err[0] = 0;
         return 0;
@@ -962,6 +985,8 @@
         }
         sb.region += pk->chunk_cap;
         sb.part_count += pk->nparts;
+        if (sb.cv_runs)
+            sb.cv_runs += lthip_plan_run_slots(pk) * 8;
     }
     hipEvent_t hashed = lthip_sync_event(ctx);
     hipError_t e = hipEventRecord(hashed, c2->stream);
@@ -1000,7 +1025,7 @@
     bool sliced;
     int err = chunk_hash_sliced(ctx, plan, d_data, d_chunk_offsets, d_chunk_lens, d_chunk_hashes, d_part_first, &sliced);
     ScanBuffers sb;
-    if (!sliced && !(err = chunk_scan_buffers(ctx, plan, !plan_walks(plan), &sb)) && !(err = chunk_scan(ctx, plan, d_data, sb)))
+    if (!sliced && !(err = chunk_scan_buffers(ctx, plan, !plan_walks(plan), d_chunk_hashes != nullptr, &sb)) && !(err = chunk_scan(ctx, plan, d_data, sb)))
         err = chunk_cut_hash(ctx, plan, d_data, sb, d_chunk_offsets, d_chunk_lens, d_chunk_hashes, d_part_first);
     if (err)
         return err;
diff --git a/longtail_amd/csrc/lthip_internal.h b/longtail_amd/csrc/lthip_internal.h
--- a/longtail_amd/csrc/lthip_internal.h
+++ b/longtail_amd/csrc/lthip_internal.h
@@ -24,6 +24,8 @@
     uint32_t tile_base;
     uint32_t region_cap;
 };
+
+__host__ __device__ inline uint64_t lthip_part_run_base(const PartDev& p) { return p.region_base + 16ull * p.tile_base; }
 
 struct DivTest
 {
@@ -48,6 +50,8 @@
     uint64_t max_part_bytes;
 };
 
+struct lthip_plan;
+uint64_t lthip_plan_run_slots(const lthip_plan* plan);
 struct lthip_plan : PlanExtents
 {
     int device;
@@ -112,6 +116,8 @@
     S_RAW_TABLES,
     S_CARRY_RUNS,
     S_ARCHIVE_ITEMS,
+    S_CV_RUNS,
+    S_CV_SLOTS,
     S_COUNT
 };
 
@@ -242,7 +248,8 @@
 
 int lthip_launch_tile_table(lthip_ctx* ctx, lthip_plan* plan);
 int lthip_launch_buzhash(lthip_ctx* ctx, const lthip_plan* plan, const uint8_t* d_data, uint64_t* bm0, uint64_t* bm1);
-int lthip_launch_buzhash_walk(lthip_ctx* ctx, const lthip_plan* plan, const uint8_t* d_data, uint2* region, uint32_t* part_count);
+int lthip_launch_buzhash_walk(lthip_ctx* ctx, const lthip_plan* plan, const uint8_t* d_data, uint2* region, uint32_t* part_count,
+                              uint32_t* cv_runs);
 uint32_t lthip_k1_resident_waves(int device);
 int lthip_launch_select(lthip_ctx* ctx, const lthip_plan* plan, const uint64_t* bm0, const uint64_t* bm1, uint2* region,
                         uint32_t* part_count);
@@ -295,6 +302,16 @@
                         const uint32_t* d_count, uint64_t count_bound, uint64_t leaf_bound, uint64_t max_len,
                         uint64_t* d_hashes);
 
+struct lthip_b3_runs
+{
+    const uint32_t* d_cvs;
+    const PartDev* d_parts;
+    uint32_t nparts;
+    const uint32_t* d_part_first;
+};
+int lthip_launch_blake3_parents(lthip_ctx* ctx, const lthip_b3_runs& runs, const uint32_t* d_lens, const uint32_t* d_count,
+                                uint64_t count_bound, uint64_t leaf_bound, uint64_t max_len, uint64_t* d_hashes);
+
 int lthip_hash_ranges_known(lthip_ctx* ctx, const void* d_data, uint64_t range_count, const uint64_t* d_offsets, const uint32_t* d_lens,
                             uint32_t max_len, uint64_t leaf_total, uint64_t* d_hashes);
 
```

Result: faster. 940.4, median of 6 (+2.3%).
